# YOUNESELBOUKNIFY/Ctr_recommendation

Measured on AMD Instinct MI355X. Metric: training samples/sec (FiBiNET d=128, MicroLens-shaped synthetic, full train step), higher is better.
Workload: dtype bf16; 1 GPU; C3: FiBiNET emb_dim=128 + item_emb_d128, batch 8192/GPU, history 20, every GEMM operand bf16 (forward and backward) / fp32 accumulation + fp32 master weights, gradients and Adam; model=MM_FiBiNET, global_batch=8192, seq_len=20, item_rows=1250000, item_rows_per_gpu=1250000, emb_dim=128, parallelism=single, hipgraph=False, launch_mode=program

## Files before the change

ctr_recommendation_amd/_lib.py:

```python
from __future__ import annotations

import contextlib
import ctypes
import os
import struct
import threading
from typing import Optional

import torch

_HERE = os.path.dirname(os.path.abspath(__file__))
LIB_PATH = os.environ.get("FBN_LIB_PATH") or os.path.join(_HERE, "libfibinet_hip.so")

P = ctypes.c_void_p
I = ctypes.c_int
LL = ctypes.c_longlong
F = ctypes.c_float
D = ctypes.c_double
SZ = ctypes.c_size_t
U = ctypes.c_uint

SIGNATURES = {
    "fbn_version": (I, []),
    "fbn_last_error": (ctypes.c_char_p, []),
    "fbn_device_ok": (I, []),
    "fbn_gemm_workspace_size": (SZ, [I, I, I, I]),
    "fbn_gemm": (I, [P, P, P, P, I, I, I, I, I, I, I, I, I, I, I, I, I, I, F, I, I, I, P, P, SZ, P]),
    "fbn_gemm_split": (I, [P, P, P, P, I, I, I, I, I, I, I, I, I, I, I, F, P, P, SZ, P, I, I, P, I, I, P]),
    "fbn_gemm_bf16out": (I, [P, P, P, I, I, I, I, I, I, I, I, P]),
    "fbn_gemm_s3": (I, [P, P, P, I, I, I, I, I, I, I, I, LL, LL, F, P, SZ, P]),
    "fbn_gemm_bn_bwd_part_supported": (I, [I, I, I, I, I, I, I]),
    "fbn_gemm_bn_bwd_part": (I, [P, P, P, I, I, I, I, I, I, I, I, P, P, P, F, P, P]),
    "fbn_bn_tile_stats": (I, [P, I, I, P, P, P]),
    "fbn_bn_tile_moments": (I, [P, I, I, P, P]),
    "fbn_bn_moments_finalize": (I, [P, D, I, P, P, P, P, F, F, I, P]),
    "fbn_bn_tile_finalize": (I, [P, I, I, D, P, P, P, P, F, F, I, P]),
    "fbn_bn_colpart_size": (SZ, [I, I]),
    "fbn_row_chunks": (I, [I]),
    "fbn_bn_bwd_chunks": (I, [I, I]),
    "fbn_bn_bwd_fused": (I, [P, P, P, P, P, F, P, P, P, P, I, I, D, P, P, P, P, P, P, P, P, P]),
    "fbn_bn_bwd_fused_img": (I, [P, P, P, P, P, F, P, P, P, P, I, I, D, P, P, P, P, P, P, P, P, P]),
    "fbn_colsum_partial": (I, [P, I, I, I, P, P]),
    "fbn_sum_jobs": (I, [P, I, P]),
    "fbn_sum_jobs2": (I, [P, I, P, I, P]),
    "fbn_gemm_slabs_size": (SZ, [I, I, I]),
    "fbn_gemm_slabs": (I, [P, P, I, I, I, I, I, I, I, P, SZ, P, I, I, P, I, I, P, P]),
    "fbn_gemm_slabs_split": (I, [I, I, I]),
    "fbn_gemm_slabs_group": (I, [P, I, P]),
    "fbn_gemm_slabs_group_split": (I, [I, I, I]),
    "fbn_fields_fwd": (I, [P, P, P, P, P, P, P, F, P, I, P, LL, P, P, P, P, P, I, P, P, P, P, I, I, P, P, P, P, P, I, I, I, I,
                           P]),
    "fbn_fields_fwd_hot": (I, [P, P, P, P, P, P, P, F, P, I, P, LL, P, P, P, P, I, P, P, P, P, I, I, P, P, P, P, P,
                               I, I, I, P, P, I, P]),
    "fbn_hot_rows": (I, [P, P, I, I, LL, P, P, P, I, I, I, P]),
    "fbn_fields_bwd_partials_size": (I, [I, I, I]),
    "fbn_fields_bwd_grid": (I, [I, I]),
    "fbn_fields_bwd": (I, [P, P, P, P, P, P, P, F, P, P, P, I, I, P, P, P, P, P, P, P, P, P, P, P, P, LL, P, P, I, I,
                           I, I, P]),
    "fbn_fields_bwd_img": (I, [P, P, P, P, P, P, P, F, P, P, P, I, I, P, P, P, P, P, P, P, P, P, P, P, P, LL, P, P, I,
                               I, I, I, P]),
    "fbn_pairs_fwd": (I, [P, P, P, P, I, I, I, I, I, P]),
    "fbn_pairs_bwd": (I, [P, P, P, P, P, P, P, I, I, I, I, P]),
    "fbn_pairs_fwd_img": (I, [P, P, P, P, I, I, I, P]),
    "fbn_pairs_bwd_img": (I, [P, P, P, P, P, I, I, I, P]),
    "fbn_bn_workspace_size": (SZ, [I, I]),
    "fbn_bn_stats_pass": (I, [P, I, I, P, P, P, P]),
    "fbn_bn_mean": (I, [P, D, I, P, P]),
    "fbn_bn_finalize": (I, [P, P, D, I, P, P, P, P, F, F, I, P]),
    "fbn_bn_stats": (I, [P, I, I, P, P, P, P, F, F, I, P, P]),
    "fbn_bn_eval_params": (I, [P, P, P, P, I, F, P]),
    "fbn_bn_act_fwd": (I, [P, P, I, I, P, P, P, P, F, P, U, P, P, P, P]),
    "fbn_bn_act_fwd_img": (I, [P, P, I, I, P, P, P, P, F, P, U, P, P, P, P]),
    "fbn_bn_act_head_fwd": (I, [P, P, I, I, P, P, P, P, F, P, U, P, P, P, P, P, P, P, P, P, F, P, F, P]),
    "fbn_bn_bwd_reduce": (I, [P, P, P, P, F, P, P, I, I, P, P, P]),
    "fbn_bn_bwd_apply": (I, [P, P, P, P, F, P, P, P, P, I, I, P, D, P, P, P, P, P, P, P]),
    "fbn_convert_bf16": (I, [P, I, P]),
    "fbn_bn_bwd": (I, [P, P, P, P, F, P, P, P, P, I, I, P, P, P, P, P, P]),
    "fbn_colsum_workspace_size": (SZ, [I, I]),
    "fbn_colsum": (I, [P, I, I, I, P, F, P, P]),
    "fbn_head_fwd": (I, [P, P, P, I, I, P, P, P, P, P, F, P]),
    "fbn_sigmoid_bwd": (I, [P, P, P, I, P]),
    "fbn_outer": (I, [P, P, P, I, I, P]),
    "fbn_sum": (I, [P, I, P, F, P]),
    "fbn_sumsq": (I, [P, LL, P, I, P, P]),
    "fbn_clip_coef": (I, [P, F, P, P, P]),
    "fbn_adam_dense": (I, [P, P, P, P, LL, P, P, P, F, F, F, P, F, P, P, P]),
    "fbn_sparse_fixup": (I, [P, P, P, I, I, LL, I, P, P, P, P, I, I, P]),
    "fbn_sumsq_sparse": (I, [P, P, P, I, I, I, P, P]),
    "fbn_sparse_fixup_dup": (I, [P, I, P, P, P, I, I, P]),
    "fbn_sumsq_sparse_norms": (I, [P, P, P, P, I, I, I, P, P, P, LL, P]),
    "fbn_sparse_fold_fx": (I, [P, P, I, P, P, I, I, P, P]),
    "fbn_adam_table": (I, [P, P, P, LL, I, P, P, P, P, I, P, P, P, F, F, F, I, P]),
    "fbn_adam_touched": (I, [P, P, P, I, P, P, P, P, I, I, P, P, P, F, F, F, P, P]),
    "fbn_adam_catchup": (I, [P, P, P, LL, I, P, I, P, I, I, P, P, P, F, F, F, P, P, P, LL, I, I, P]),
    "fbn_adam_claim_catchup": (I, [P, P, I, I, LL, P, P, P, P, P, P, P, P, LL, I, I, P, P, P, F, F, F, P, P, P, LL, I,
                                   I, P]),
    "fbn_adam_claim_catchup_conv": (I, [P, P, I, I, LL, P, P, P, P, P, P, P, P, LL, I, I, P, P, P, F, F, F, P, P, P,
                                        LL, I, I, P, I, P]),
    "fbn_adam_flush": (I, [P, P, P, LL, I, P, P, P, F, F, F, P, P, P, LL, I, I, P]),
    "fbn_adam_prefetch_rows": (I, [P, I, I, LL, P, P, P, P, P, I, P, P, P, F, F, F, P, P, P, LL, I, I, P]),
    "fbn_adam_prefetch": (I, [P, P, I, I, LL, P, P, P, P, P, I, P, P, P, F, F, F, P, P, P, LL, I, I, P]),
    "fbn_adam_prefetch_binned_ws_size": (SZ, [LL]),
    "fbn_adam_prefetch_binned": (I, [P, P, I, I, LL, P, P, P, P, P, I, P, P, P, F, F, F, P, P, P, LL, I, I, P, SZ, P]),
    "fbn_adam_selftest": (I, [I, ctypes.c_uint, P, P]),
    "fbn_adam_step_tail": (I, [P, P, P, P, LL, P, F, P, P, P, P, P, I, P, P, P, P, I, I, P, P, F, F, F, P, P, P, P, I,
                               LL, I, P, P, P, P, I, P, P]),
    "fbn_adam_commit": (I, [P, P, P, I, P, P, P, P, I, I, P, P, P, F, F, F, P, P, P, P, I, I, P]),
    "fbn_claim_rows": (I, [P, P, I, I, LL, P, P, P, P, P]),
    "fbn_pack_extras": (I, [P, P, P, P]),
    "fbn_unpack_extras": (I, [P, P, P, P]),
    "fbn_unpack_sumsq": (I, [P, P, P, LL, P, P]),
    "fbn_step_end": (I, [P, P, P, P, P, I, P, P]),
    "fbn_route": (I, [P, P, I, I, LL, LL, I, P, P, P, P, P, P, P]),
# ... 345 lines not shown
```

ctr_recommendation_amd/csrc/fields.hip:

```cpp
#include <cstdlib>
#include "common.h"
#include "fields_common.h"

#ifndef FBN_HCH
#define FBN_HCH 10
#endif

struct FieldArgs {
  const int64_t* item_id;
  const int64_t* item_seq;
  const int64_t* likes;
  const int64_t* views;
  const float* hmm;
  const float* ln_g;
  const float* ln_b;
  const float* cate;
  const float* table;
  const int* pos;
  const float* w1; const float* b1; const float* w2; const float* b2;
  float* X;
  float* Vc;
  short* Vc16;
  void* c;
  float* a_out;
// ... 195 lines not shown
    const f32x4 xs[5] = {c1, c2, rit, x4, x5};
    float z[6];
    z[0] = 0.f;
#pragma unroll
    for (int f = 0; f < 5; ++f) z[f + 1] = group_sum<G>(xs[f][0] + xs[f][1] + xs[f][2] + xs[f][3]) / (float)D;
    float qv[FBN_MAXR], a[6];
    senet_excite<D>(z, p.w1, p.b1, p.w2, p.b2, p.R, qv, a);

    float* Xb = p.X + (size_t)b * 2 * D + 4 * q;
    *reinterpret_cast<f32x4*>(Xb) = rit;
    *reinterpret_cast<f32x4*>(Xb + D) = x5;
    float* Vb = p.Vc ? p.Vc + (size_t)b * 5 * D + 4 * q : nullptr;
    float* cb = (p.c && !p.c16) ? (float*)p.c + (size_t)b * p.ldc + 4 * q : nullptr;
    short* cb16 = (p.c && p.c16) ? (short*)p.c + (size_t)b * p.ldc + 4 * q : nullptr;
#pragma unroll
    for (int f = 0; f < 5; ++f) {
      const f32x4 v = xs[f] * a[f + 1];
      if (p.Vc) *reinterpret_cast<f32x4*>(Vb + f * D) = v;
      const bf16x4 v16 = (bf16x4){f2bf(v[0]), f2bf(v[1]), f2bf(v[2]), f2bf(v[3])};
      if (cb16) *reinterpret_cast<bf16x4*>(cb16 + f * D) = v16;
      else if (cb) *reinterpret_cast<f32x4*>(cb + f * D) = v;
      if (p.Vc16) *reinterpret_cast<bf16x4*>(p.Vc16 + ((size_t)b * 5 + f) * D + 4 * q) = v16;
    }
#pragma unroll
    for (int f = 0; f < 6; ++f)
      if (f % G == q) p.a_out[(size_t)b * 6 + f] = a[f];
    if (q == 0) p.cnt_out[b] = cnt;

    if (MODE == 0 && p.map) {
      for (int t = q; t <= L; t += G) {
        long long r = (t == 0) ? item : p.item_seq[(size_t)b * L + (t - 1)];
        if (r > 0 && r < p.V) map_claim(p.map, p.slot_row, (int)r, b * (L + 1) + t);
      }
    }
  }
}

struct FieldBwdArgs {
  const int64_t* item_id; const int64_t* item_seq; const int64_t* likes; const int64_t* views;
  const float* hmm; const float* ln_g;
  const float* w1; const float* b1; const float* w2;
  const float* X;
  const float* cate;
  const float* ln_b;
  const float* a;
  const float* cnt;
  const float* dV;
  float* dhmm;
  short* dhmm16;
  long long dhmm16_lo;
  float* partials;
  float* gtab; float* gvec;
  double* gnorm;
  const int* pos; void* sendbuf;
  long long V;
  int B, L, R, n_cate;
  float ln_eps;
};

template <int G>
__device__ __forceinline__ f32x4 transpose_cols(const f32x4& v, int lane) {
  const int base = lane - lane % G, q = lane % G;
  f32x4 t;
#pragma unroll
  for (int e = 0; e < 4; ++e) {
    const int src = base + e * (G / 4) + q / 4;
    const float x0 = __shfl(v[0], src, 64), x1 = __shfl(v[1], src, 64);
    const float x2 = __shfl(v[2], src, 64), x3 = __shfl(v[3], src, 64);
    const int c = q & 3;
    t[e] = c == 0 ? x0 : (c == 1 ? x1 : (c == 2 ? x2 : x3));
  }
  return t;
}
template <int G>
__device__ __forceinline__ void atomic_add_row_t(float* row, const f32x4& t, int q) {
  atomicAdd(row + q, t[0]); atomicAdd(row + G + q, t[1]); atomicAdd(row + 2 * G + q, t[2]);
  atomicAdd(row + 3 * G + q, t[3]);
}

template <int D, int MODE, int RMAX>
__global__ void __launch_bounds__(256) fields_bwd_kernel(FieldBwdArgs p) {
  FBN_MAIN_PRIO();
  constexpr int G = D / 4;
  constexpr int SPW = 64 / G;
  constexpr int NPMAX = 13 * RMAX + 6;
  constexpr int SJ = (NPMAX + G - 1) / G;
  extern __shared__ __attribute__((aligned(16))) float sp[];
  const int R = p.R;
  const int NP = 13 * R + 6;
  const int P = NP + 3 * D + p.n_cate * D;
  const int wave = threadIdx.x >> 6;
  float* ws = sp + wave * P;
  float* sv = sp + 4 * P + (wave * SPW + (threadIdx.x & 63) / G) * (12 + 2 * RMAX);
  for (int i = threadIdx.x; i < 4 * P; i += blockDim.x) sp[i] = 0.f;
  __syncthreads();
  float* w_lg = ws + NP;
  float* w_ct = w_lg + 2 * D;
  float* w_hb = w_ct + p.n_cate * D;

  const int lane = threadIdx.x & 63;
  const int q = lane % G, grp = lane / G;
  const int gw = (blockIdx.x * blockDim.x + threadIdx.x) >> 6;
  const int nwaves = (gridDim.x * blockDim.x) >> 6;
  const int L = p.L;
  f32x4 acc_lg = {0.f, 0.f, 0.f, 0.f}, acc_lb = {0.f, 0.f, 0.f, 0.f}, acc_hb = {0.f, 0.f, 0.f, 0.f};
  float acc_se[SJ];
#pragma unroll
  for (int j = 0; j < SJ; ++j) acc_se[j] = 0.f;

  for (int b0 = gw * SPW; b0 < p.B; b0 += nwaves * SPW) {
    const int b = b0 + grp;
    const bool live = b < p.B;
    f32x4 dx0 = {0.f, 0.f, 0.f, 0.f}, dx1 = {0.f, 0.f, 0.f, 0.f};
    long long lk = -1, vw = -1;
    if (live) {
      const float* Xb = p.X + (size_t)b * 2 * D + 4 * q;
      const float* dVb = p.dV + (size_t)b * 5 * D + 4 * q;
      f32x4 x[5], dv[5];
      lk = p.likes[b];
      vw = p.views[b];
      const long long lkc = (lk >= 0 && lk < p.n_cate) ? lk : 0, vwc = (vw >= 0 && vw < p.n_cate) ? vw : 0;
      x[0] = *reinterpret_cast<const f32x4*>(p.cate + lkc * D + 4 * q);
      x[1] = *reinterpret_cast<const f32x4*>(p.cate + vwc * D + 4 * q);
      x[2] = *reinterpret_cast<const f32x4*>(Xb);
      x[4] = *reinterpret_cast<const f32x4*>(Xb + D);
#pragma unroll
      for (int f = 0; f < 5; ++f) dv[f] = *reinterpret_cast<const f32x4*>(dVb + f * D);
      const f32x4 h = *reinterpret_cast<const f32x4*>(p.hmm + (size_t)b * D + 4 * q);
      x[3] = ln_relu<G>(h, p.ln_g, p.ln_b, p.ln_eps, q);
      float a[6];
#pragma unroll
      for (int f = 0; f < 6; ++f) a[f] = p.a[(size_t)b * 6 + f];
      float z[6];
      z[0] = 0.f;
#pragma unroll
      for (int f = 0; f < 5; ++f) z[f + 1] = group_sum<G>(x[f][0] + x[f][1] + x[f][2] + x[f][3]) / (float)D;
      float qv[RMAX], rj[RMAX], dq[RMAX];
#pragma unroll
      for (int j = 0; j < RMAX; ++j) {
        float s = 0.f;
        if (j < R) {
          s = p.b1[j];
#pragma unroll
          for (int f = 0; f < 6; ++f) s += p.w1[j * 6 + f] * z[f];
        }
        qv[j] = s;
        rj[j] = fmaxf(s, 0.f);
      }
      float ds[6];
      ds[0] = 0.f;
#pragma unroll
      for (int f = 0; f < 5; ++f) {
        const float da = group_sum<G>(dv[f][0] * x[f][0] + dv[f][1] * x[f][1] + dv[f][2] * x[f][2] + dv[f][3] * x[f][3]);
        ds[f + 1] = da * (1.f - a[f + 1]) * a[f + 1];
      }
      float dz[6] = {0.f, 0.f, 0.f, 0.f, 0.f, 0.f};
#pragma unroll
// ... 16 lines not shown
        for (int jj = 0; jj < RMAX; ++jj) { sv[12 + jj] = dq[jj]; sv[12 + RMAX + jj] = rj[jj]; }
      }
      __builtin_amdgcn_wave_barrier();
#pragma unroll
      for (int j = 0; j < SJ; ++j) {
        const int k = q + j * G;
        float v = 0.f;
        if (k < 6 * R) v = sv[12 + k / 6] * sv[6 + k % 6];
        else if (k < 7 * R) v = sv[12 + (k - 6 * R)];
        else if (k < 13 * R) v = sv[(k - 7 * R) / R] * sv[12 + RMAX + (k - 7 * R) % R];
        else if (k < NP) v = sv[k - 13 * R];
        acc_se[j] += v;
      }
      __builtin_amdgcn_wave_barrier();
      f32x4 dx[5];
#pragma unroll
      for (int f = 0; f < 5; ++f) dx[f] = dv[f] * a[f + 1] + dz[f + 1] / (float)D;
      dx0 = dx[0];
      dx1 = dx[1];

      {
        const float mean = group_sum<G>(h[0] + h[1] + h[2] + h[3]) / (float)D;
        const f32x4 dh = h - mean;
        const float s2 = group_sum<G>(dh[0] * dh[0] + dh[1] * dh[1] + dh[2] * dh[2] + dh[3] * dh[3]);
        const float rstd = 1.f / sqrtf(s2 / (float)D + p.ln_eps);
        const f32x4 gam = *reinterpret_cast<const f32x4*>(p.ln_g + 4 * q);
        f32x4 gl, xh, gx;
#pragma unroll
        for (int e = 0; e < 4; ++e) {
          gl[e] = x[3][e] > 0.f ? dx[3][e] : 0.f;
          xh[e] = dh[e] * rstd;
          gx[e] = gl[e] * gam[e];
          acc_lg[e] += gl[e] * xh[e];
          acc_lb[e] += gl[e];
        }
        const float m1 = group_sum<G>(gx[0] + gx[1] + gx[2] + gx[3]) / (float)D;
        const float m2 = group_sum<G>(gx[0] * xh[0] + gx[1] * xh[1] + gx[2] * xh[2] + gx[3] * xh[3]) / (float)D;
        f32x4 out;
#pragma unroll
        for (int e = 0; e < 4; ++e) out[e] = rstd * (gx[e] - m1 - xh[e] * m2);
        *reinterpret_cast<f32x4*>(p.dhmm + (size_t)b * D + 4 * q) = out;
        acc_hb += out;
        if (p.dhmm16) {
          const bf16x4 hi = (bf16x4){f2bf(out[0]), f2bf(out[1]), f2bf(out[2]), f2bf(out[3])};
          *reinterpret_cast<bf16x4*>(p.dhmm16 + (size_t)b * D + 4 * q) = hi;
          if (p.dhmm16_lo)
            *reinterpret_cast<bf16x4*>(p.dhmm16 + p.dhmm16_lo + (size_t)b * D + 4 * q) =
                (bf16x4){f2bf(out[0] - bf2f(hi[0])), f2bf(out[1] - bf2f(hi[1])), f2bf(out[2] - bf2f(hi[2])),
                         f2bf(out[3] - bf2f(hi[3]))};
        }
      }
      const f32x4 gh = dx[4] / p.cnt[b];
      if (MODE == 0 && p.gvec) {
        *reinterpret_cast<f32x4*>(p.gvec + (size_t)b * 2 * D + 4 * q) = dx[2];
        *reinterpret_cast<f32x4*>(p.gvec + ((size_t)b * 2 + 1) * D + 4 * q) = gh;
        if (p.gnorm) {
          double si = 0.0, sh = 0.0;
#pragma unroll
          for (int e = 0; e < 4; ++e) {
            si += (double)(dx[2][e] * dx[2][e]);
            sh += (double)(gh[e] * gh[e]);
          }
#pragma unroll
          for (int o = G / 2; o > 0; o >>= 1) {
            si += __shfl_xor(si, o, 64);
            sh += __shfl_xor(sh, o, 64);
          }
          if (q == 0) {
            p.gnorm[(size_t)b * 2] = si;
            p.gnorm[(size_t)b * 2 + 1] = sh;
          }
        }
      } else if (MODE == 0) {
        const f32x4 ti = transpose_cols<G>(dx[2], lane);
        const f32x4 th = transpose_cols<G>(gh, lane);
        const long long item = p.item_id[b];
        if (item > 0 && item < p.V) atomic_add_row_t<G>(p.gtab + item * D, ti, q);
        for (int t = 0; t < L; ++t) {
          const long long s = p.item_seq[(size_t)b * L + t];
          if (s > 0 && s < p.V) atomic_add_row_t<G>(p.gtab + s * D, th, q);
        }
      } else {
        const int* pb = p.pos + (size_t)b * (L + 1);
        auto put = [&](int row, const f32x4& x) {
          if constexpr (MODE == 2) {
            *reinterpret_cast<bf16x4*>(reinterpret_cast<short*>(p.sendbuf) + (size_t)row * D + 4 * q) =
                (bf16x4){f2bf(x[0]), f2bf(x[1]), f2bf(x[2]), f2bf(x[3])};
          } else {
            *reinterpret_cast<f32x4*>(reinterpret_cast<float*>(p.sendbuf) + (size_t)row * D + 4 * q) = x;
          }
        };
        if (pb[0] >= 0) put(pb[0], dx[2]);
        for (int t = 0; t < L; ++t)
          if (pb[t + 1] >= 0) put(pb[t + 1], gh);
      }
    }
#pragma unroll
    for (int gi = 0; gi < SPW; ++gi) {
      if (grp == gi && live) {
        if (lk >= 0 && lk < p.n_cate) {
          f32x4* c = reinterpret_cast<f32x4*>(w_ct + lk * D + 4 * q);
          *c = *c + dx0;
        }
        if (vw >= 0 && vw < p.n_cate) {
          f32x4* c = reinterpret_cast<f32x4*>(w_ct + vw * D + 4 * q);
          *c = *c + dx1;
        }
      }
// ... 143 lines not shown
  if (clear && i == 0) *hot_n = 0;
  if (i >= (long long)B * (L + 1)) return;
  const long long b = i / (L + 1), t = i - b * (L + 1);
  const long long id = t == 0 ? item[b] : seq[b * L + (t - 1)];
  if (id <= 0 || id >= V) return;
  if (clear) {
    cnt[id] = 0;
    return;
  }
  if (atomicAdd(cnt + id, 1) == tau - 1) {
    const int s = atomicAdd(hot_n, 1);
    if (s < H) hot[s] = (int)id;
  }
}

extern "C" int fbn_hot_rows(const int64_t* item, const int64_t* seq, int B, int L, long long V, int* cnt, int* hot,
                            int* hot_n, int H, int tau, int clear, void* stream) {
  const long long n = (long long)B * (L + 1);
  if (n <= 0) return FBN_OK;
  fbn_launch(hot_rows_kernel, dim3((unsigned)((n + 255) / 256)), dim3(256), 0, (hipStream_t)stream, item,
                     L > 0 ? seq : nullptr, B, L, V, cnt, hot, hot_n, H, tau < 1 ? 1 : tau, clear);
  FBN_CHECK_LAUNCH();
  return FBN_OK;
}

static int fields_fwd_impl(const int64_t* item_id, const int64_t* item_seq, const int64_t* likes,
                           const int64_t* views, const float* hmm, const float* ln_g, const float* ln_b,
                           float ln_eps, const float* cate, int n_cate, const float* table, long long V,
                           const int* pos, const float* w1, const float* b1, const float* w2,
                           const float* b2, int R, float* X, float* Vc, short* Vc16, void* c, int ldc, int c_bf16,
                           float* a_out, float* cnt_out, int* err, int* map, int* slot_row, int B, int L,
                           int D, int rows_bf16, const int* hot, const int* hot_n, int H, void* stream) {
  if (B <= 0) return FBN_OK;
  if (L < 0 || L > 32 || R < 1 || R > FBN_MAXR || (ldc & 3)) {
    fbn_set_error("fbn_fields_fwd: need 0 <= L <= 32, 1 <= R <= 8, ldc % 4 == 0");
    return FBN_ERR_ARG;
  }
  FieldArgs a;
  a.item_id = item_id; a.item_seq = L > 0 ? item_seq : nullptr; a.likes = likes; a.views = views;
  a.hmm = hmm; a.ln_g = ln_g; a.ln_b = ln_b; a.cate = cate; a.table = table; a.pos = pos;
  a.w1 = w1; a.b1 = b1; a.w2 = w2; a.b2 = b2;
  a.X = X; a.Vc = Vc; a.Vc16 = Vc16; a.c = c; a.a_out = a_out; a.cnt_out = cnt_out; a.err = err;
  a.map = map; a.slot_row = slot_row;
  a.V = V; a.B = B; a.L = L; a.ldc = ldc; a.R = R; a.n_cate = n_cate; a.ln_eps = ln_eps; a.c16 = c_bf16;
  a.hot = hot; a.hot_n = hot_n; a.H = H;
  if (pos && rows_bf16) return launch_fields_fwd<2>(a, D, (hipStream_t)stream);
  if (pos) return launch_fields_fwd<1>(a, D, (hipStream_t)stream);
  return launch_fields_fwd<0>(a, D, (hipStream_t)stream);
}

extern "C" int fbn_fields_bwd_partials_size(int D, int R, int n_cate) { return 13 * R + 6 + 3 * D + n_cate * D; }
extern "C" int fbn_fields_bwd_grid(int B, int D) { return fields_grid(B, D, FBN_FB_MAXBLK); }

template <int MODE, int RMAX>
static int launch_fields_bwd_r(const FieldBwdArgs& a, int D, hipStream_t st) {
  const int grid = fields_grid(a.B, D, FBN_FB_MAXBLK);
  const size_t lds = (4 * (size_t)(13 * a.R + 6 + 3 * D + a.n_cate * D) + 4 * (64 / (D / 4)) * (12 + 2 * RMAX)) *
                     sizeof(float);
  switch (D) {
    case 16: fbn_launch((fields_bwd_kernel<16, MODE, RMAX>), dim3(grid), dim3(256), lds, st, a); break;
    case 32: fbn_launch((fields_bwd_kernel<32, MODE, RMAX>), dim3(grid), dim3(256), lds, st, a); break;
    case 64: fbn_launch((fields_bwd_kernel<64, MODE, RMAX>), dim3(grid), dim3(256), lds, st, a); break;
    case 128: fbn_launch((fields_bwd_kernel<128, MODE, RMAX>), dim3(grid), dim3(256), lds, st, a); break;
    case 256: fbn_launch((fields_bwd_kernel<256, MODE, RMAX>), dim3(grid), dim3(256), lds, st, a); break;
    default: fbn_set_error("fields: embedding_dim must be one of 16,32,64,128,256"); return FBN_ERR_UNSUPPORTED;
  }
  FBN_CHECK_LAUNCH();
  return FBN_OK;
}

template <int MODE>
static int launch_fields_bwd(const FieldBwdArgs& a, int D, hipStream_t st) {
  return a.R <= 3 ? launch_fields_bwd_r<MODE, 3>(a, D, st) : launch_fields_bwd_r<MODE, FBN_MAXR>(a, D, st);
}

static int fields_bwd_impl(const int64_t* item_id, const int64_t* item_seq, const int64_t* likes,
                           const int64_t* views, const float* hmm, const float* ln_g, const float* ln_b,
                           float ln_eps, const float* w1, const float* b1, const float* w2, int R, int n_cate,
                           const float* cate, const float* X, const float* a, const float* cnt, const float* dV,
                           float* dhmm, short* dhmm16, float* partials, float* const* param_grads, float* gtab,
                           float* gvec, double* gnorm, long long V, const int* pos, void* sendbuf, int send_bf16,
                           int B, int L, int D, void* stream, long long dhmm16_lo);
extern "C" int fbn_fields_bwd(const int64_t* item_id, const int64_t* item_seq, const int64_t* likes,
                              const int64_t* views, const float* hmm, const float* ln_g, const float* ln_b,
                              float ln_eps, const float* w1, const float* b1, const float* w2, int R, int n_cate,
                              const float* cate, const float* X, const float* a, const float* cnt, const float* dV, float* dhmm,
                              short* dhmm16, float* partials, float* const* param_grads, float* gtab, float* gvec,
                              double* gnorm, long long V, const int* pos, void* sendbuf, int send_bf16, int B,
                              int L, int D, void* stream) {
  return fields_bwd_impl(item_id, item_seq, likes, views, hmm, ln_g, ln_b, ln_eps, w1, b1, w2, R, n_cate, cate, X, a,
                         cnt, dV, dhmm, dhmm16, partials, param_grads, gtab, gvec, gnorm, V, pos, sendbuf, send_bf16, B,
                         L, D, stream, 0);
}
extern "C" int fbn_fields_bwd_img(const int64_t* item_id, const int64_t* item_seq, const int64_t* likes,
                                  const int64_t* views, const float* hmm, const float* ln_g, const float* ln_b,
                                  float ln_eps, const float* w1, const float* b1, const float* w2, int R, int n_cate,
                                  const float* cate, const float* X, const float* a, const float* cnt, const float* dV,
                                  float* dhmm, void* dhmm_img, float* partials, float* const* param_grads,
                                  float* gtab, float* gvec, double* gnorm, long long V, const int* pos, void* sendbuf,
                                  int send_bf16, int B, int L, int D, void* stream) {
  if (!dhmm_img) { fbn_set_error("fbn_fields_bwd_img: dhmm_img"); return FBN_ERR_ARG; }
  return fields_bwd_impl(item_id, item_seq, likes, views, hmm, ln_g, ln_b, ln_eps, w1, b1, w2, R, n_cate, cate, X, a,
                         cnt, dV, dhmm, (short*)dhmm_img, partials, param_grads, gtab, gvec, gnorm, V, pos, sendbuf,
                         send_bf16, B, L, D, stream, (long long)B * D);
}
static int fields_bwd_impl(const int64_t* item_id, const int64_t* item_seq, const int64_t* likes,
                           const int64_t* views, const float* hmm, const float* ln_g, const float* ln_b,
                           float ln_eps, const float* w1, const float* b1, const float* w2, int R, int n_cate,
                           const float* cate, const float* X, const float* a, const float* cnt, const float* dV,
                           float* dhmm, short* dhmm16, float* partials, float* const* param_grads, float* gtab,
                           float* gvec, double* gnorm, long long V, const int* pos, void* sendbuf, int send_bf16,
                           int B, int L, int D, void* stream, long long dhmm16_lo) {
  if (B <= 0) return FBN_OK;
  if (L < 0 || L > 32 || R < 1 || R > FBN_MAXR) { fbn_set_error("fbn_fields_bwd: bad L/R"); return FBN_ERR_ARG; }
  FieldBwdArgs p;
  p.item_id = item_id; p.item_seq = L > 0 ? item_seq : nullptr; p.likes = likes; p.views = views;
  p.hmm = hmm; p.ln_g = ln_g; p.ln_b = ln_b; p.w1 = w1; p.b1 = b1; p.w2 = w2; p.cate = cate;
  p.X = X; p.a = a; p.cnt = cnt; p.dV = dV; p.dhmm = dhmm; p.dhmm16 = dhmm16; p.partials = partials;
  p.dhmm16_lo = dhmm16_lo;
  p.gtab = gtab; p.gvec = gvec; p.gnorm = gvec ? gnorm : nullptr; p.pos = pos; p.sendbuf = sendbuf;
  p.V = V; p.B = B; p.L = L; p.R = R; p.n_cate = n_cate; p.ln_eps = ln_eps;
  hipStream_t st = (hipStream_t)stream;
  int rc = !pos ? launch_fields_bwd<0>(p, D, st) : send_bf16 ? launch_fields_bwd<2>(p, D, st)
                                                               : launch_fields_bwd<1>(p, D, st);
  if (rc) return rc;
  if (!param_grads) return FBN_OK;
  const int P = 13 * R + 6 + 3 * D + n_cate * D;
  const int nblk = fields_grid(B, D, FBN_FB_MAXBLK);

  GradOuts o;
  const int sizes[8] = {6 * R, R, 6 * R, 6, D, D, n_cate * D, D};
  o.off[0] = 0;
  for (int j = 0; j < 8; ++j) {
    if (j < 7 && !param_grads[j]) {
      fbn_set_error("fbn_fields_bwd: null parameter-gradient destination");
      return FBN_ERR_ARG;
    }
    o.p[j] = param_grads[j];
    o.off[j + 1] = o.off[j] + sizes[j];
  }
  fbn_launch(reduce_partials_one16, dim3(fbn_cdiv(P, 16)), dim3(1024), 0, st, (const float*)partials, nblk, P, o);
  FBN_CHECK_LAUNCH();
  return FBN_OK;
}
```

ctr_recommendation_amd/csrc/mlp.hip:

```cpp
#include <cstdlib>
#include "common.h"
#include "convert.h"

__device__ constexpr int c_pi[10] = {0, 0, 0, 0, 1, 1, 1, 2, 2, 3};
__device__ constexpr int c_pj[10] = {1, 2, 3, 4, 2, 3, 4, 3, 4, 4};

__device__ __forceinline__ void store4(float* p, const f32x4& v) { *reinterpret_cast<f32x4*>(p) = v; }
__device__ __forceinline__ void store4(short* p, const f32x4& v) {
  *reinterpret_cast<bf16x4*>(p) = (bf16x4){f2bf(v[0]), f2bf(v[1]), f2bf(v[2]), f2bf(v[3])};
}
__device__ __forceinline__ void store_img4(short* p, long long lo_off, const f32x4& v) {
  bf16x4 h, l;
#pragma unroll
  for (int e = 0; e < 4; ++e) {
    h[e] = f2bf(v[e]);
    l[e] = f2bf(v[e] - bf2f(h[e]));
  }
  *reinterpret_cast<bf16x4*>(p) = h;
  *reinterpret_cast<bf16x4*>(p + lo_off) = l;
}
__device__ __forceinline__ void store_lo4(short* p, const f32x4& v) {
  bf16x4 l;
#pragma unroll
  for (int e = 0; e < 4; ++e) l[e] = f2bf(v[e] - bf2f(f2bf(v[e])));
// ... 753 lines not shown
                                                            const float* __restrict__ mean,
                                                            const float* __restrict__ invstd,
                                                            const float* __restrict__ g,
                                                            const float* __restrict__ coef, float* __restrict__ dX,
                                                            short* __restrict__ dX16, int B, int C,
                                                            int rows_per_chunk, float* __restrict__ colpart) {
  FBN_MAIN_PRIO();
  __shared__ f32x4 red[4][64];
  const int q = threadIdx.x & 63, rl = threadIdx.x >> 6;
  const int c = blockIdx.x * 256 + q * 4;
  const int r0 = blockIdx.y * rows_per_chunk, r1 = min(B, r0 + rows_per_chunk);
  f32x4 acc = {0.f, 0.f, 0.f, 0.f};
  if (c < C) {
    const f32x4 mu = *reinterpret_cast<const f32x4*>(mean + c);
    const f32x4 is = *reinterpret_cast<const f32x4*>(invstd + c);
    const f32x4 gg = *reinterpret_cast<const f32x4*>(g + c);
    const f32x4 c0 = *reinterpret_cast<const f32x4*>(coef + c);
    const f32x4 c1 = *reinterpret_cast<const f32x4*>(coef + C + c);
    const f32x4 ww = s.G ? (f32x4){0.f, 0.f, 0.f, 0.f} : *reinterpret_cast<const f32x4*>(s.w + c);
    for (int r = r0 + rl; r < r1; r += 4) {
      const size_t i = (size_t)r * C + c;
      const f32x4 h = bn_act4(s, i);
      const f32x4 x = *reinterpret_cast<const f32x4*>(Xpre + i);
      f32x4 d;
      if (s.G) d = *reinterpret_cast<const f32x4*>(s.G + i);
      else { const float gv = s.gvec[r]; d = (f32x4){gv * ww[0], gv * ww[1], gv * ww[2], gv * ww[3]}; }
      f32x4 v;
#pragma unroll
      for (int e = 0; e < 4; ++e) {
        const float dy = h[e] > 0.f ? d[e] * s.scale : 0.f;
        v[e] = (dy - c0[e] - (x[e] - mu[e]) * c1[e]) * is[e] * gg[e];
      }
      if (dX) *reinterpret_cast<f32x4*>(dX + i) = v;
      if (dX16) {
        if (s.dx16_lo) store_img4(dX16 + i, s.dx16_lo, v);
        else store4(dX16 + i, v);
      }
      acc += v;
    }
  }
  if (!colpart) return;
  red[rl][q] = acc;
  __syncthreads();
  if (rl == 0 && c < C)
    *reinterpret_cast<f32x4*>(colpart + (size_t)blockIdx.y * C + c) = red[0][q] + red[1][q] + red[2][q] + red[3][q];
}

struct SumJob {
  const float* part;
  float* out;
  int nch, C;
  float scale, beta;
  int ld;
  int pad_;
};
struct SlabJob {
  const float* ws;
  float* out;
  int M, N, ldc, nsplit, seg, off0, off1;
  float beta;
};
#define FBN_MAX_SUM_JOBS 16
#define FBN_SUM_WIDE 32
#define FBN_MAX_SLAB_JOBS 8
#define FBN_SLAB_GROUPS 4
struct SumJobs {
  SumJob j[FBN_MAX_SUM_JOBS];
  int col0[FBN_MAX_SUM_JOBS + 1];
  int n;
  SlabJob s[FBN_MAX_SLAB_JOBS];
  int blk0[FBN_MAX_SLAB_JOBS + 1];
  int ns;
};
#define FBN_SLAB_DIRECT 8
__device__ __forceinline__ void slab_direct(const SlabJob& sj, int lb) {
  const size_t total = (size_t)sj.M * sj.N;
  const size_t i4 = (size_t)lb * 256 + threadIdx.x;
  if (i4 >= total / 4) return;
  const float* src = sj.ws + i4 * 4;
  f32x4 x[FBN_SLAB_DIRECT];
#pragma unroll
  for (int z = 0; z < FBN_SLAB_DIRECT; ++z)
    if (z < sj.nsplit) x[z] = *reinterpret_cast<const f32x4*>(src + (size_t)z * total);
  f32x4 t = x[0];
#pragma unroll
  for (int z = 1; z < FBN_SLAB_DIRECT; ++z)
    if (z < sj.nsplit) t += x[z];
  const int m = (int)(i4 * 4 / sj.N), n = (int)(i4 * 4 - (size_t)m * sj.N);
  float* cp = sj.out + (size_t)m * sj.ldc + n + (n < sj.seg ? sj.off0 : sj.off1);
  if (sj.beta != 0.f) t += sj.beta * *reinterpret_cast<const f32x4*>(cp);
  *reinterpret_cast<f32x4*>(cp) = t;
}
__device__ __forceinline__ void slab_block(const SumJobs& J, int gb) {
  __shared__ f32x4 red[FBN_SLAB_GROUPS][64];
  int u = 0;
  while (u + 1 < J.ns && gb >= J.blk0[u + 1]) ++u;
  const SlabJob sj = J.s[u];
  if (sj.nsplit <= FBN_SLAB_DIRECT) {
    slab_direct(sj, gb - J.blk0[u]);
    return;
  }
  const int qd = threadIdx.x & 63, grp = threadIdx.x >> 6;
  const size_t total = (size_t)sj.M * sj.N;
  const size_t i4 = (size_t)(gb - J.blk0[u]) * 64 + qd;
  const bool ok = i4 < total / 4;
  f32x4 acc = {0.f, 0.f, 0.f, 0.f};
  if (ok) {
    const float* src = sj.ws + i4 * 4;
    int z = grp;
    for (; z + 3 * FBN_SLAB_GROUPS < sj.nsplit; z += 4 * FBN_SLAB_GROUPS) {
      const f32x4 a = *reinterpret_cast<const f32x4*>(src + (size_t)z * total);
      const f32x4 b = *reinterpret_cast<const f32x4*>(src + (size_t)(z + FBN_SLAB_GROUPS) * total);
      const f32x4 c = *reinterpret_cast<const f32x4*>(src + (size_t)(z + 2 * FBN_SLAB_GROUPS) * total);
      const f32x4 d = *reinterpret_cast<const f32x4*>(src + (size_t)(z + 3 * FBN_SLAB_GROUPS) * total);
      acc += a; acc += b; acc += c; acc += d;
    }
    for (; z < sj.nsplit; z += FBN_SLAB_GROUPS) acc += *reinterpret_cast<const f32x4*>(src + (size_t)z * total);
  }
  red[grp][qd] = acc;
  __syncthreads();
  if (grp == 0 && ok) {
    f32x4 t = red[0][qd];
#pragma unroll
    for (int k = 1; k < FBN_SLAB_GROUPS; ++k) t += red[k][qd];
    const int m = (int)(i4 * 4 / sj.N), n = (int)(i4 * 4 - (size_t)m * sj.N);
    float* cp = sj.out + (size_t)m * sj.ldc + n + (n < sj.seg ? sj.off0 : sj.off1);
    if (sj.beta != 0.f) t += sj.beta * *reinterpret_cast<const f32x4*>(cp);
    *reinterpret_cast<f32x4*>(cp) = t;
  }
}
__device__ __forceinline__ void sum_wide_block(const SumJob& jb, int c0) {
  __shared__ float red[16][17];
  const int col = threadIdx.x & 15, str = threadIdx.x >> 4, c = c0 + col;
  const size_t ld = jb.ld > 0 ? jb.ld : jb.C;
  float a0 = 0.f, a1 = 0.f;
  if (c < jb.C) {
    int k = str;
    for (; k + 16 < jb.nch; k += 32) {
      a0 += jb.part[(size_t)k * ld + c];
      a1 += jb.part[(size_t)(k + 16) * ld + c];
    }
    for (; k < jb.nch; k += 16) a0 += jb.part[(size_t)k * ld + c];
  }
  red[str][col] = a0 + a1;
  __syncthreads();
  if (str == 0 && c < jb.C) {
    float t = 0.f;
#pragma unroll
    for (int k = 0; k < 16; ++k) t += red[k][col];
    t *= jb.scale;
    jb.out[c] = jb.beta != 0.f ? jb.beta * jb.out[c] + t : t;
  }
}
__global__ void __launch_bounds__(256) sum_jobs_kernel(SumJobs J) {
  __shared__ float red[4];
  const int gc = blockIdx.x;
  if (gc >= J.col0[J.n]) {
    slab_block(J, gc - J.col0[J.n]);
    return;
  }
  int u = 0;
  while (u + 1 < J.n && gc >= J.col0[u + 1]) ++u;
  const SumJob jb = J.j[u];
  if (jb.C >= FBN_SUM_WIDE) {
    sum_wide_block(jb, (gc - J.col0[u]) * 16);
    return;
  }
  const int c = gc - J.col0[u];
  const size_t ld = jb.ld > 0 ? jb.ld : jb.C;
  float a0 = 0.f, a1 = 0.f, a2 = 0.f, a3 = 0.f;
  int k = threadIdx.x;
  for (; k + 768 < jb.nch; k += 1024) {
    a0 += jb.part[(size_t)k * ld + c];
    a1 += jb.part[(size_t)(k + 256) * ld + c];
    a2 += jb.part[(size_t)(k + 512) * ld + c];
    a3 += jb.part[(size_t)(k + 768) * ld + c];
  }
  for (; k < jb.nch; k += 256) a0 += jb.part[(size_t)k * ld + c];
  float v = wave_sum((a0 + a1) + (a2 + a3));
  if ((threadIdx.x & 63) == 0) red[threadIdx.x >> 6] = v;
  __syncthreads();
  if (threadIdx.x == 0) {
    const float t = jb.scale * ((red[0] + red[1]) + (red[2] + red[3]));
    jb.out[c] = jb.beta != 0.f ? jb.beta * jb.out[c] + t : t;
  }
}

__global__ void head_fwd_kernel(const float* __restrict__ H, const float* __restrict__ w, const float* __restrict__ bias,
                                int B, int C, float* __restrict__ logits, float* __restrict__ probs,
                                const float* __restrict__ labels, float* __restrict__ loss_terms,
                                float* __restrict__ gout, float denom) {
  const int lane = threadIdx.x & 63;
  const int row = (blockIdx.x * blockDim.x + threadIdx.x) >> 6;
  if (row >= B) return;
  float s = 0.f;
  for (int c = lane * 4; c < C; c += 256) {
    const f32x4 h = *reinterpret_cast<const f32x4*>(H + (size_t)row * C + c);
    const f32x4 ww = *reinterpret_cast<const f32x4*>(w + c);
    s += h[0] * ww[0] + h[1] * ww[1] + h[2] * ww[2] + h[3] * ww[3];
  }
  head_row(s, row, lane, HeadArgs{w, bias, logits, probs, labels, loss_terms, gout, denom});
}

__global__ void sigmoid_bwd_kernel(const float* gp, const float* probs, float* gout, int B) {
  const int i = blockIdx.x * blockDim.x + threadIdx.x;
  if (i < B) gout[i] = gp[i] * (1.f - probs[i]) * probs[i];
}

__global__ void outer_kernel(const float* g, const float* w, float* out, int B, int C) {
  const size_t total = (size_t)B * C;
  for (size_t i = (size_t)blockIdx.x * blockDim.x + threadIdx.x; i < total; i += (size_t)gridDim.x * blockDim.x)
    out[i] = g[i / C] * w[i % C];
}

__global__ void __launch_bounds__(1024) sum_kernel(const float* x, int n, float* out, float scale) {
  __shared__ float red[16];
  float s0 = 0.f, s1 = 0.f, s2 = 0.f, s3 = 0.f;
  int i = threadIdx.x;
  for (; i + 3 * 1024 < n; i += 4 * 1024) {
    s0 += x[i]; s1 += x[i + 1024]; s2 += x[i + 2048]; s3 += x[i + 3072];
  }
  for (; i < n; i += 1024) s0 += x[i];
  float s = wave_sum((s0 + s1) + (s2 + s3));
  if ((threadIdx.x & 63) == 0) red[threadIdx.x >> 6] = s;
  __syncthreads();
  if (threadIdx.x < 64) {
    float t = threadIdx.x < 16 ? red[threadIdx.x] : 0.f;
    t = wave_sum(t);
    if (threadIdx.x == 0) out[0] = t * scale;
  }
}

static int ew_grid(size_t n) {
  size_t g = (n + 255) / 256;
  return (int)(g < 1 ? 1 : (g > 8192 ? 8192 : g));
}
static int row_chunks(int B) {
// ... 360 lines not shown
  return bn_bwd_fused_impl(G, gvec, w, hact, hact16, scale, Xpre, mean, invstd, gamma, B, C, ntot, dXpre,
                           (short*)dXpre_img, dgamma, dbeta, dw, colpart, part_pre, ws, stream, (long long)B * C);
}
static int bn_bwd_fused_impl(const float* G, const float* gvec, const float* w, const float* hact,
                             const short* hact16, float scale, const float* Xpre, const float* mean,
                             const float* invstd, const float* gamma, int B, int C, double ntot, float* dXpre,
                             short* dXpre16, float* dgamma, float* dbeta, float* dw, float* colpart,
                             const double* part_pre, void* ws, void* stream, long long img_lo) {
  if (B <= 0) return FBN_OK;
  if (C & 3) { fbn_set_error("fbn_bn_bwd_fused: C % 4"); return FBN_ERR_ARG; }
  if (!hact && !(hact16 && G)) {
    fbn_set_error("fbn_bn_bwd_fused: the bf16 activation image stands in only for a matrix source");
    return FBN_ERR_ARG;
  }
  if (!dXpre && !dXpre16) { fbn_set_error("fbn_bn_bwd_fused: no output"); return FBN_ERR_ARG; }
  hipStream_t st = (hipStream_t)stream;
  BnBwdSrc s{G, gvec, w, hact, scale, hact16, img_lo};
  const int nch = bn_bwd_chunks(B, C), rpc = (B + nch - 1) / nch;
  double* part = (double*)ws;
  float* coef = (float*)((double*)ws + (size_t)nch * 3 * C + 3 * (size_t)C);
  if (part_pre)
    part = const_cast<double*>(part_pre);
  else
    fbn_launch(bn_bwd_partial4_kernel, dim3(fbn_cdiv(C, 256), nch), dim3(256), 0, st, s, Xpre, mean, B, C, rpc,
                       part);
  const char* nce = getenv("FBN_BN_REDUCE_NC");
  const int nc = nce ? atoi(nce) : 16;
  if (nc == 4)
    fbn_launch(bn_bwd_reduce_finalize16_kernel<4>, dim3(fbn_cdiv(C, 4)), dim3(256), 0, st, part, nch, C, ntot,
               invstd, coef, dgamma, dbeta, dw);
  else if (nc == 8)
    fbn_launch(bn_bwd_reduce_finalize16_kernel<8>, dim3(fbn_cdiv(C, 8)), dim3(512), 0, st, part, nch, C, ntot,
               invstd, coef, dgamma, dbeta, dw);
  else
    fbn_launch(bn_bwd_reduce_finalize16_kernel<16>, dim3(fbn_cdiv(C, 16)), dim3(1024), 0, st, part, nch, C, ntot,
                       invstd, coef, dgamma, dbeta, dw);
  fbn_launch(bn_bwd_apply4_kernel, dim3(fbn_cdiv(C, 256), nch), dim3(256), 0, st, s, Xpre, mean, invstd, gamma,
                     coef, dXpre, dXpre16, B, C, rpc, colpart);
  FBN_CHECK_LAUNCH();
  return FBN_OK;
}

extern "C" int fbn_colsum_partial(const float* X, int B, int C, int ldx, float* part, void* stream) {
  if (B <= 0) return FBN_OK;
  const int nch = row_chunks(B), rpc = (B + nch - 1) / nch;
  fbn_launch(colsum_partial_kernel, dim3(fbn_cdiv(C, 64), nch), dim3(256), 0, (hipStream_t)stream, X, B, C,
                     ldx, rpc, part);
  FBN_CHECK_LAUNCH();
  return FBN_OK;
}

extern "C" int fbn_row_chunks(int B) { return row_chunks(B); }

extern "C" int fbn_sum_jobs2(const SumJob* jobs, int n, const SlabJob* slabs, int ns, void* stream) {
  if (n < 0 || ns < 0 || n > FBN_MAX_SUM_JOBS || ns > FBN_MAX_SLAB_JOBS) {
    fbn_set_error("fbn_sum_jobs2: too many jobs");
    return FBN_ERR_ARG;
  }
  SumJobs J;
  J.n = n;
  J.col0[0] = 0;
  for (int i = 0; i < n; ++i) {
    J.j[i] = jobs[i];
    J.col0[i + 1] = J.col0[i] + (jobs[i].C >= FBN_SUM_WIDE ? fbn_cdiv(jobs[i].C, 16) : jobs[i].C);
  }
  J.ns = ns;
  J.blk0[0] = 0;
  for (int i = 0; i < ns; ++i) {
    const SlabJob& sj = slabs[i];
    if ((sj.N & 3) || (sj.ldc & 3) || (sj.off0 & 3) || (sj.off1 & 3) || (sj.seg != 0x7fffffff && (sj.seg & 3)) ||
        ((uintptr_t)sj.out & 15) || ((uintptr_t)sj.ws & 15) || sj.nsplit < 1) {
      fbn_set_error("fbn_sum_jobs2: slab job needs N, ldc, remap % 4, 16-B aligned buffers, nsplit >= 1");
      return FBN_ERR_ARG;
    }
    J.s[i] = sj;
    const int qpb = (sj.nsplit <= FBN_SLAB_DIRECT) ? 256 : 64;
    J.blk0[i + 1] = J.blk0[i] + (int)fbn_cdiv((long long)sj.M * sj.N / 4, qpb);
  }
  const int blocks = J.col0[n] + J.blk0[ns];
  if (blocks <= 0) return FBN_OK;
  fbn_launch(sum_jobs_kernel, dim3(blocks), dim3(256), 0, (hipStream_t)stream, J);
  FBN_CHECK_LAUNCH();
  return FBN_OK;
}

extern "C" int fbn_sum_jobs(const SumJob* jobs, int n, void* stream) {
  if (n <= 0) return FBN_OK;
  return fbn_sum_jobs2(jobs, n, nullptr, 0, stream);
}

extern "C" int fbn_bn_tile_moments(const float* part, int M, int C, double* out_d, void* stream) {
  if (M <= 0) { (void)hipMemsetAsync(out_d, 0, 2 * sizeof(double) * C, (hipStream_t)stream); return FBN_OK; }
  fbn_launch(bn_tile_moments_kernel, dim3(fbn_cdiv(C, 4)), dim3(256), 0, (hipStream_t)stream, part,
                     (M + 63) / 64, C, M, 64, out_d);
  FBN_CHECK_LAUNCH();
  return FBN_OK;
}

extern "C" int fbn_bn_moments_finalize(const double* mom_d, double ntot, int C, float* mean, float* invstd,
                                       float* run_mean, float* run_var, float momentum, float eps, int update_running,
                                       void* stream) {
  fbn_launch(bn_moments_finalize_kernel, dim3(fbn_cdiv(C, 256)), dim3(256), 0, (hipStream_t)stream, mom_d, ntot,
                     C, mean, invstd, run_mean, run_var, momentum, eps, update_running);
  FBN_CHECK_LAUNCH();
  return FBN_OK;
}
```

ctr_recommendation_amd/csrc/optim.hip:

```cpp
#include "common.h"
#include "convert.h"
#include <cstdlib>
#include <algorithm>

#pragma clang fp contract(off)

#define FBN_SUMSQ_SLOTS 64

struct AdamConsts {
  float w1;
  float nss;
  float bc2s;
  float rbc2s;
  float dmul;
  float pad0, pad1, pad2;
};

__global__ void sumsq_kernel(const float* __restrict__ x, long long n, const int* __restrict__ n_rows, int row_len,
                             double* __restrict__ out) {
  __shared__ double red[256];
  long long lim = n_rows ? (long long)(*n_rows) * row_len : n;
  double s = 0.0;
  const long long n4 = lim / 4;
  for (long long i = (long long)blockIdx.x * blockDim.x + threadIdx.x; i < n4; i += (long long)gridDim.x * blockDim.x) {
// ... 199 lines not shown
  for (long long e0 = gw * RPW; e0 < n; e0 += nw * RPW) {
    const long long e = e0 + lane / G;
    if (e >= n) continue;
    long long r;
    if (ids) {
      r = ids[e];
      if (r < 0 || (rank == 0 && r == 0)) continue;
    } else {
      const long long b = e / (L + 1), t = e - b * (L + 1);
      r = t == 0 ? item[b] : seq[b * L + (t - 1)];
      if (r <= 0 || r >= V) continue;
    }
    const int u = map[r];
    if (u == (int)e || u < 0) continue;
    const float* src = grad_base<D>(s, (int)e);
    float* dst;
    if (s.extra) {
      if (q == 0) atomicOr(&s.slot_row[u], FBN_SLOT_FLAG);
      dst = s.extra + (size_t)u * D;
    } else {
      dst = const_cast<float*>(s.vec) + (size_t)u * D;
    }
#pragma unroll
    for (int k = 0; k < 4; ++k) atomicAdd(dst + k * G + q, src[k * G + q]);
  }
}

__global__ void claim_rows_kernel(const int64_t* __restrict__ item, const int64_t* __restrict__ seq, int B, int L,
                                  long long V, int* __restrict__ map, int* __restrict__ slot_row, int* __restrict__ dup,
                                  int* __restrict__ hasdup) {
  const long long n = (long long)B * (L + 1);
  for (long long e = (long long)blockIdx.x * blockDim.x + threadIdx.x; e < n; e += (long long)gridDim.x * blockDim.x) {
    const long long b = e / (L + 1), t = e - b * (L + 1);
    const long long r = t == 0 ? item[b] : seq[b * L + (t - 1)];
    int owner = -1;
    if (r > 0 && r < V) {
      owner = __hip_atomic_load(map + r, __ATOMIC_RELAXED, __HIP_MEMORY_SCOPE_AGENT);
      if (owner == -1) {
        int expected = -1;
        if (__hip_atomic_compare_exchange_strong(map + r, &expected, (int)e, __ATOMIC_RELAXED, __ATOMIC_RELAXED,
                                                 __HIP_MEMORY_SCOPE_AGENT))
          slot_row[e] = (int)r;
        else
          owner = expected;
      }
    }
    if (dup) dup[e] = owner;
    if (hasdup && owner >= 0) hasdup[owner] = 1;
  }
}

template <int D>
__global__ void __launch_bounds__(FBN_FOLD_THREADS) sparse_fixup_dup_kernel(const int* __restrict__ dup, int n, GradSrc s) {
  constexpr int NPL = D / 64 > 0 ? D / 64 : 1;
  constexpr int MAXV = 16;
  constexpr int CPW = FBN_FOLD_CHUNKS;
  constexpr int NS = D >= 256 ? 32 : 64;
  __shared__ int skey[NS];
  __shared__ float sacc[NS * D];
  const int tid = threadIdx.x, lane = tid & 63, wave = tid >> 6;
  for (int i = tid; i < NS; i += blockDim.x) skey[i] = -1;
  for (int i = tid; i < NS * D; i += blockDim.x) sacc[i] = 0.f;
  __syncthreads();
  const int Lp1 = s.Lp1;
  const long long base = (long long)blockIdx.x * blockDim.x * CPW;
  int uu[CPW];
#pragma unroll
  for (int c = 0; c < CPW; ++c) {
    const long long e = base + ((long long)(wave * CPW + c) << 6) + lane;
    uu[c] = e < n ? dup[e] : -1;
  }
  auto add_row = [&](int ue, const float (&acc)[NPL], bool hot) {
    int slot = -1;
    if (hot && lane == 0) {
      for (int k = 0, h = (int)(((unsigned)ue * 2654435761u) >> 20) & (NS - 1); k < 4; ++k, h = (h + 1) & (NS - 1)) {
        int cur = __hip_atomic_load(skey + h, __ATOMIC_RELAXED, __HIP_MEMORY_SCOPE_WORKGROUP);
        if (cur == -1) {
          int expected = -1;
          if (__hip_atomic_compare_exchange_strong(skey + h, &expected, ue, __ATOMIC_RELAXED, __ATOMIC_RELAXED,
                                                   __HIP_MEMORY_SCOPE_WORKGROUP)) {
            slot = h;
            break;
          }
          cur = expected;
        }
        if (cur == ue) {
          slot = h;
          break;
        }
      }
    }
    slot = __shfl(slot, 0, 64);
    if (slot >= 0) {
#pragma unroll
      for (int k = 0; k < NPL; ++k)
        if (D >= 64 || lane < D) atomicAdd(sacc + slot * D + (D >= 64 ? k * 64 : 0) + lane, acc[k]);
    } else {
      float* dst = s.extra + (size_t)ue * D;
      if (lane == 0) atomicOr(&s.slot_row[ue], FBN_SLOT_FLAG);
#pragma unroll
      for (int k = 0; k < NPL; ++k)
        if (D >= 64 || lane < D) atomicAdd(dst + (D >= 64 ? k * 64 : 0) + lane, acc[k]);
    }
  };
#pragma unroll 1
  for (int c = 0; c < CPW; ++c) {
// ... 14 lines not shown
      unsigned long long vm[MAXV];
#pragma unroll
      for (int v = 0; v < MAXV; ++v) {
        vm[v] = __ballot(vid == v);
        const float* src = s.vec + ((size_t)bs * 2 + (v < nv ? v : 0)) * D;
#pragma unroll
        for (int k = 0; k < NPL; ++k)
          vec[v][k] = (D >= 64 || lane < D) ? src[(D >= 64 ? k * 64 : 0) + (lane & (D - 1))] : 0.f;
      }
      while (act) {
        const int l = __ffsll((long long)act) - 1;
        const int ue = __shfl(u, l, 64);
        const unsigned long long m = __ballot(u == ue) & act;
        act &= ~m;
        float acc[NPL];
#pragma unroll
        for (int k = 0; k < NPL; ++k) acc[k] = 0.f;
#pragma unroll
        for (int v = 0; v < MAXV; ++v) {
          const float cnt = (float)__popcll(m & vm[v]);
#pragma unroll
          for (int k = 0; k < NPL; ++k) acc[k] = __builtin_fmaf(cnt, vec[v][k], acc[k]);
        }
        add_row(ue, acc, __popcll(m) > 1);
      }
    } else {
      while (act) {
        const int l = __ffsll((long long)act) - 1;
        act &= act - 1;
        const int ue = __shfl(u, l, 64);
        const float* src = grad_base<D>(s, (int)(e0 + l));
        float acc[NPL];
#pragma unroll
        for (int k = 0; k < NPL; ++k) acc[k] = (D >= 64 || lane < D) ? src[(D >= 64 ? k * 64 : 0) + (lane & (D - 1))] : 0.f;
        add_row(ue, acc, false);
      }
    }
  }
  __syncthreads();
  for (int slot = wave; slot < NS; slot += blockDim.x >> 6) {
    const int ue = skey[slot];
    if (ue < 0) continue;
    if (lane == 0) atomicOr(&s.slot_row[ue], FBN_SLOT_FLAG);
    float* dst = s.extra + (size_t)ue * D;
    for (int k = lane; k < D; k += 64) atomicAdd(dst + k, sacc[slot * D + k]);
  }
}

#define FBN_FX_SHIFT 40
__device__ __forceinline__ long long to_fx(float x) { return __double2ll_rn((double)x * 1099511627776.0); }
template <int D>
__global__ void __launch_bounds__(256) sparse_fold_fx_kernel(const int* __restrict__ dup, int* __restrict__ hasdup,
                                                             int n, GradSrc s, unsigned long long* __restrict__ acc) {
  const int lane = threadIdx.x & 63;
  for (long long e0 = ((long long)blockIdx.x * blockDim.x + threadIdx.x) - lane; e0 < n;
       e0 += (long long)gridDim.x * blockDim.x) {
    const long long e = e0 + lane;
    int u = -1;
    if (e < n) {
      u = dup[e];
      if (u < 0 && hasdup[e]) {
        u = (int)e;
        hasdup[e] = 0;
        s.slot_row[e] |= FBN_SLOT_FLAG;
      }
    }
    unsigned long long mask = __ballot(u >= 0);
    while (mask) {
      const int l = __ffsll((long long)mask) - 1;
      mask &= mask - 1;
      const int ue = __shfl(u, l, 64);
      const float* src = grad_base<D>(s, (int)(e0 + l));
      unsigned long long* dst = acc + (size_t)ue * D;
      for (int k = lane; k < D; k += 64) atomicAdd(dst + k, (unsigned long long)to_fx(src[k]));
    }
  }
}

template <int D>
__global__ void __launch_bounds__(256) sumsq_norms_kernel(GradSrc s, const double* __restrict__ gnorm, int n,
                                                          double* __restrict__ out, unsigned long long* __restrict__ fx,
                                                          const float* __restrict__ dense, long long n_dense) {
  __shared__ double red[4];
  const int lane = threadIdx.x & 63;
  double acc = 0.0;
  for (long long i = (long long)blockIdx.x * blockDim.x + threadIdx.x; i < n_dense / 4;
       i += (long long)gridDim.x * blockDim.x) {
    const f32x4 v = *reinterpret_cast<const f32x4*>(dense + 4 * i);
    acc += (double)(v[0] * v[0]) + (double)(v[1] * v[1]) + (double)(v[2] * v[2]) + (double)(v[3] * v[3]);
  }
  for (long long e0 = ((long long)blockIdx.x * blockDim.x + threadIdx.x) - lane; e0 < n;
       e0 += (long long)gridDim.x * blockDim.x) {
    const long long e = e0 + lane;
    const int sr = e < n ? s.slot_row[e] : -1;
    const bool flag = sr != -1 && (sr & FBN_SLOT_FLAG);
    if (sr != -1 && !flag) {
      const int b = (int)(e / s.Lp1), t = (int)(e - (long long)b * s.Lp1);
      acc += gnorm[(size_t)b * 2 + (t ? 1 : 0)];
    }
    unsigned long long mask = __ballot(flag);
    if (fx) {
      while (mask) {
        const int l = __ffsll((long long)mask) - 1;
        mask &= mask - 1;
        float* x = s.extra + (size_t)(e0 + l) * D;
        unsigned long long* a = fx + (size_t)(e0 + l) * D;
        for (int k = lane; k < D; k += 64) {
          const float y = (float)((double)(long long)a[k] * (1.0 / 1099511627776.0));
          x[k] = y;
          a[k] = 0ull;
          acc += (double)(y * y);
        }
      }
    } else {
      constexpr int LPR = D / 8, RPR = 64 / LPR;
      while (mask) {
        int mine = -1;
#pragma unroll
        for (int gi = 0; gi < RPR; ++gi) {
          if (!mask) break;
          const int l = __ffsll((long long)mask) - 1;
          mask &= mask - 1;
          if (lane / LPR == gi) mine = l;
        }
        if (mine < 0) continue;
        const int c = (lane % LPR) * 8;
        const float* v = grad_base<D>(s, (int)(e0 + mine)) + c;
        const float* x = s.extra + (size_t)(e0 + mine) * D + c;
        const f32x4 v0 = *reinterpret_cast<const f32x4*>(v), v1 = *reinterpret_cast<const f32x4*>(v + 4);
        const f32x4 x0 = *reinterpret_cast<const f32x4*>(x), x1 = *reinterpret_cast<const f32x4*>(x + 4);
        const f32x4 y0 = v0 + x0, y1 = v1 + x1;
#pragma unroll
        for (int k = 0; k < 4; ++k) acc += (double)(y0[k] * y0[k]) + (double)(y1[k] * y1[k]);
      }
    }
// ... 1176 lines not shown
      if (ps.pend) ps.pend[(size_t)(r) * FBN_RS_I] = -1;
    }
  }
}

template <int D>
__global__ void __launch_bounds__(256) adam_touched_kernel(float* __restrict__ p, float* __restrict__ m,
                                                           float* __restrict__ v, int* __restrict__ map, GradSrc gs,
                                                           int n, const float* __restrict__ coef_ptr,
                                                           const AdamConsts* __restrict__ table,
                                                           const int* __restrict__ step_ptr, float wd, float b2,
                                                           float omb2, float eps, int* __restrict__ last) {
  resolve_src(gs);
  constexpr int G = D / 4, RPW = 64 / G;
  const AdamConsts k = table[*step_ptr];
  const float coef = coef_ptr ? *coef_ptr : 1.f;
  const int lane = threadIdx.x & 63, q = lane % G;
  const long long gw = ((long long)blockIdx.x * blockDim.x + threadIdx.x) >> 6;
  const long long nw = ((long long)gridDim.x * blockDim.x) >> 6;
  for (long long e0 = gw * RPW; e0 < n; e0 += nw * RPW) {
    const long long e = e0 + lane / G;
    if (e >= n) continue;
    const int sr = gs.slot_row[e];
    if (sr == -1) continue;
    const long long r = sr & ~FBN_SLOT_FLAG;
    f32x4 gg = grad4<D>(gs, (int)e, 4 * q);
    if (sr & FBN_SLOT_FLAG) {
      float* ex = gs.extra + (size_t)e * D + 4 * q;
      gg = gs.full ? *reinterpret_cast<const f32x4*>(ex) : gg + *reinterpret_cast<const f32x4*>(ex);
      *reinterpret_cast<f32x4*>(ex) = (f32x4){0.f, 0.f, 0.f, 0.f};
    }
    const size_t off = (size_t)r * D + 4 * q;
    f32x4 pp = *reinterpret_cast<f32x4*>(p + off);
    f32x4 mm = *reinterpret_cast<f32x4*>(m + off);
    f32x4 vv = *reinterpret_cast<f32x4*>(v + off);
    adam_tab4<true>(pp, mm, vv, gg * coef, wd, b2, omb2, eps, k);
    *reinterpret_cast<f32x4*>(p + off) = pp;
    *reinterpret_cast<f32x4*>(m + off) = mm;
    *reinterpret_cast<f32x4*>(v + off) = vv;
    if (q == 0) {
      map[r] = -1;
      if (last) last[(size_t)(r) * FBN_RS_I] = *step_ptr + 1;
    }
  }
}

template <int D>
__device__ __forceinline__ void adam_commit_body(float* __restrict__ p, float* __restrict__ m, float* __restrict__ v,
                                                 int* __restrict__ map, const GradSrc& gs, int n, float coef,
                                                 const AdamConsts& k, int t, float wd, float b2, float omb2, float eps,
                                                 int* __restrict__ last, const PendSrc& ps, int B, long long bid,
                                                 long long nblk) {
  constexpr int G = D / 4, RPW = 64 / G;
  if (gs.Lp1 > 1) {
    float* dst = const_cast<float*>(ps.ring) + (size_t)(t % ps.ring_n) * ps.ring_stride;
    const long long n4 = (long long)B * 2 * D / 4, st = nblk * blockDim.x;
    for (long long i0 = bid * blockDim.x + threadIdx.x; i0 < n4; i0 += 8 * st) {
      f32x4 x[8];
#pragma unroll
      for (int u = 0; u < 8; ++u)
        x[u] = reinterpret_cast<const f32x4*>(gs.vec)[i0 + u * st < n4 ? i0 + u * st : i0];
#pragma unroll
      for (int u = 0; u < 8; ++u)
        if (i0 + u * st < n4) reinterpret_cast<f32x4*>(dst)[i0 + u * st] = x[u];
    }
  }
  const int lane = threadIdx.x & 63, q = lane % G;
  for (long long e0 = (bid * blockDim.x + threadIdx.x) - lane; e0 < n; e0 += nblk * blockDim.x) {
    const long long e = e0 + lane;
    const int sr = e < n ? gs.slot_row[e] : -1;
    const bool flag = sr != -1 && (sr & FBN_SLOT_FLAG);
    bool imm = flag;
    if (sr != -1 && !flag) {
      if (last && (unsigned)row_state(last, sr).y == (unsigned)(t + 1)) {
        imm = true;
      } else {
        if (gs.Lp1 == 1) {
          ps.pend[(size_t)(sr) * FBN_RS_I] = (int)e;
        } else {
          const int b = (int)(e / gs.Lp1), tt = (int)(e - (long long)b * gs.Lp1);
          ps.pend[(size_t)(sr) * FBN_RS_I] = b * 2 + (tt ? 1 : 0);
        }
        map[sr] = -1;
        gs.slot_row[e] = -1;
      }
    }
    unsigned long long mask = __ballot(imm);
    constexpr int G8 = D / 8 > 0 ? D / 8 : 1, RPW8 = 64 / G8;
    const int q8 = lane % G8;
    while (mask) {
      int mine = -1;
#pragma unroll
      for (int gi = 0; gi < RPW8; ++gi) {
        if (!mask) break;
        const int l = __ffsll((long long)mask) - 1;
        mask &= mask - 1;
        if (lane / G8 == gi) mine = l;
      }
      const int sr_l = __shfl(sr, mine < 0 ? 0 : mine, 64);
      if (mine < 0) continue;
      const long long ee = e0 + mine;
      const long long r = sr_l & ~FBN_SLOT_FLAG;
#pragma unroll
      for (int h = 0; h < 2; ++h) {
        const int c = 8 * q8 + 4 * h;
        if (D < 8 && c >= D) break;
        f32x4 gg = grad4<D>(gs, (int)ee, c);
        if (sr_l & FBN_SLOT_FLAG) {
// ... 1028 lines not shown
```

ctr_recommendation_amd/csrc/plan_thunks.inc:

```

static int th_fbn_adam_catchup(const uint64_t* i, const double* f) {
  return fbn_adam_catchup(reinterpret_cast<float*>(static_cast<uintptr_t>(i[0])),
      reinterpret_cast<float*>(static_cast<uintptr_t>(i[1])),
      reinterpret_cast<float*>(static_cast<uintptr_t>(i[2])),
      static_cast<long long>(i[3]),
      static_cast<int>(i[4]),
      reinterpret_cast<const int*>(static_cast<uintptr_t>(i[5])),
      static_cast<int>(i[6]),
      reinterpret_cast<const int*>(static_cast<uintptr_t>(i[7])),
      static_cast<int>(i[8]),
      static_cast<int>(i[9]),
      reinterpret_cast<int*>(static_cast<uintptr_t>(i[10])),
      reinterpret_cast<const void*>(static_cast<uintptr_t>(i[11])),
      reinterpret_cast<const int*>(static_cast<uintptr_t>(i[12])),
      plan_f32(f[0]),
      plan_f32(f[1]),
      plan_f32(f[2]),
      reinterpret_cast<int*>(static_cast<uintptr_t>(i[13])),
      reinterpret_cast<const float*>(static_cast<uintptr_t>(i[14])),
      reinterpret_cast<const float*>(static_cast<uintptr_t>(i[15])),
      static_cast<long long>(i[16]),
      static_cast<int>(i[17]),
      static_cast<int>(i[18]),
      reinterpret_cast<void*>(static_cast<uintptr_t>(i[19])));
// ... 814 lines not shown
      reinterpret_cast<void*>(static_cast<uintptr_t>(i[26])),
      static_cast<int>(i[27]),
      static_cast<int>(i[28]),
      static_cast<int>(i[29]),
      static_cast<int>(i[30]),
      reinterpret_cast<void*>(static_cast<uintptr_t>(i[31])));
}
static int th_fbn_fields_bwd_grid(const uint64_t* i, const double* f) {
  (void)f;
  return fbn_fields_bwd_grid(static_cast<int>(i[0]),
      static_cast<int>(i[1]));
}
static int th_fbn_fields_bwd_img(const uint64_t* i, const double* f) {
  return fbn_fields_bwd_img(reinterpret_cast<const int64_t*>(static_cast<uintptr_t>(i[0])),
      reinterpret_cast<const int64_t*>(static_cast<uintptr_t>(i[1])),
      reinterpret_cast<const int64_t*>(static_cast<uintptr_t>(i[2])),
      reinterpret_cast<const int64_t*>(static_cast<uintptr_t>(i[3])),
      reinterpret_cast<const float*>(static_cast<uintptr_t>(i[4])),
      reinterpret_cast<const float*>(static_cast<uintptr_t>(i[5])),
      reinterpret_cast<const float*>(static_cast<uintptr_t>(i[6])),
      plan_f32(f[0]),
      reinterpret_cast<const float*>(static_cast<uintptr_t>(i[7])),
      reinterpret_cast<const float*>(static_cast<uintptr_t>(i[8])),
      reinterpret_cast<const float*>(static_cast<uintptr_t>(i[9])),
      static_cast<int>(i[10]),
      static_cast<int>(i[11]),
      reinterpret_cast<const float*>(static_cast<uintptr_t>(i[12])),
      reinterpret_cast<const float*>(static_cast<uintptr_t>(i[13])),
      reinterpret_cast<const float*>(static_cast<uintptr_t>(i[14])),
      reinterpret_cast<const float*>(static_cast<uintptr_t>(i[15])),
      reinterpret_cast<const float*>(static_cast<uintptr_t>(i[16])),
      reinterpret_cast<float*>(static_cast<uintptr_t>(i[17])),
      reinterpret_cast<void*>(static_cast<uintptr_t>(i[18])),
      reinterpret_cast<float*>(static_cast<uintptr_t>(i[19])),
      reinterpret_cast<float* const*>(static_cast<uintptr_t>(i[20])),
      reinterpret_cast<float*>(static_cast<uintptr_t>(i[21])),
      reinterpret_cast<float*>(static_cast<uintptr_t>(i[22])),
      reinterpret_cast<double*>(static_cast<uintptr_t>(i[23])),
      static_cast<long long>(i[24]),
      reinterpret_cast<const int*>(static_cast<uintptr_t>(i[25])),
      reinterpret_cast<void*>(static_cast<uintptr_t>(i[26])),
      static_cast<int>(i[27]),
      static_cast<int>(i[28]),
      static_cast<int>(i[29]),
      static_cast<int>(i[30]),
      reinterpret_cast<void*>(static_cast<uintptr_t>(i[31])));
}
static int th_fbn_fields_bwd_partials_size(const uint64_t* i, const double* f) {
  (void)f;
  return fbn_fields_bwd_partials_size(static_cast<int>(i[0]),
      static_cast<int>(i[1]),
      static_cast<int>(i[2]));
}
static int th_fbn_fields_fwd(const uint64_t* i, const double* f) {
  return fbn_fields_fwd(reinterpret_cast<const int64_t*>(static_cast<uintptr_t>(i[0])),
      reinterpret_cast<const int64_t*>(static_cast<uintptr_t>(i[1])),
      reinterpret_cast<const int64_t*>(static_cast<uintptr_t>(i[2])),
      reinterpret_cast<const int64_t*>(static_cast<uintptr_t>(i[3])),
      reinterpret_cast<const float*>(static_cast<uintptr_t>(i[4])),
      reinterpret_cast<const float*>(static_cast<uintptr_t>(i[5])),
      reinterpret_cast<const float*>(static_cast<uintptr_t>(i[6])),
      plan_f32(f[0]),
      reinterpret_cast<const float*>(static_cast<uintptr_t>(i[7])),
      static_cast<int>(i[8]),
      reinterpret_cast<const float*>(static_cast<uintptr_t>(i[9])),
      static_cast<long long>(i[10]),
      reinterpret_cast<const int*>(static_cast<uintptr_t>(i[11])),
      reinterpret_cast<const float*>(static_cast<uintptr_t>(i[12])),
      reinterpret_cast<const float*>(static_cast<uintptr_t>(i[13])),
      reinterpret_cast<const float*>(static_cast<uintptr_t>(i[14])),
      reinterpret_cast<const float*>(static_cast<uintptr_t>(i[15])),
      static_cast<int>(i[16]),
      reinterpret_cast<float*>(static_cast<uintptr_t>(i[17])),
      reinterpret_cast<float*>(static_cast<uintptr_t>(i[18])),
      reinterpret_cast<short*>(static_cast<uintptr_t>(i[19])),
      reinterpret_cast<void*>(static_cast<uintptr_t>(i[20])),
      static_cast<int>(i[21]),
      static_cast<int>(i[22]),
      reinterpret_cast<float*>(static_cast<uintptr_t>(i[23])),
      reinterpret_cast<float*>(static_cast<uintptr_t>(i[24])),
      reinterpret_cast<int*>(static_cast<uintptr_t>(i[25])),
      reinterpret_cast<int*>(static_cast<uintptr_t>(i[26])),
      reinterpret_cast<int*>(static_cast<uintptr_t>(i[27])),
      static_cast<int>(i[28]),
      static_cast<int>(i[29]),
      static_cast<int>(i[30]),
      static_cast<int>(i[31]),
      reinterpret_cast<void*>(static_cast<uintptr_t>(i[32])));
}
static int th_fbn_fields_fwd_hot(const uint64_t* i, const double* f) {
  return fbn_fields_fwd_hot(reinterpret_cast<const int64_t*>(static_cast<uintptr_t>(i[0])),
      reinterpret_cast<const int64_t*>(static_cast<uintptr_t>(i[1])),
      reinterpret_cast<const int64_t*>(static_cast<uintptr_t>(i[2])),
      reinterpret_cast<const int64_t*>(static_cast<uintptr_t>(i[3])),
      reinterpret_cast<const float*>(static_cast<uintptr_t>(i[4])),
      reinterpret_cast<const float*>(static_cast<uintptr_t>(i[5])),
      reinterpret_cast<const float*>(static_cast<uintptr_t>(i[6])),
      plan_f32(f[0]),
      reinterpret_cast<const float*>(static_cast<uintptr_t>(i[7])),
      static_cast<int>(i[8]),
      reinterpret_cast<const float*>(static_cast<uintptr_t>(i[9])),
      static_cast<long long>(i[10]),
      reinterpret_cast<const float*>(static_cast<uintptr_t>(i[11])),
      reinterpret_cast<const float*>(static_cast<uintptr_t>(i[12])),
      reinterpret_cast<const float*>(static_cast<uintptr_t>(i[13])),
      reinterpret_cast<const float*>(static_cast<uintptr_t>(i[14])),
// ... 522 lines not shown
  (void)f;
  return fbn_sparse_fixup_dup(reinterpret_cast<const int*>(static_cast<uintptr_t>(i[0])),
      static_cast<int>(i[1]),
      reinterpret_cast<const float*>(static_cast<uintptr_t>(i[2])),
      reinterpret_cast<float*>(static_cast<uintptr_t>(i[3])),
      reinterpret_cast<int*>(static_cast<uintptr_t>(i[4])),
      static_cast<int>(i[5]),
      static_cast<int>(i[6]),
      reinterpret_cast<void*>(static_cast<uintptr_t>(i[7])));
}
static int th_fbn_sparse_fold_fx(const uint64_t* i, const double* f) {
  (void)f;
  return fbn_sparse_fold_fx(reinterpret_cast<const int*>(static_cast<uintptr_t>(i[0])),
      reinterpret_cast<int*>(static_cast<uintptr_t>(i[1])),
      static_cast<int>(i[2]),
      reinterpret_cast<const float*>(static_cast<uintptr_t>(i[3])),
      reinterpret_cast<int*>(static_cast<uintptr_t>(i[4])),
      static_cast<int>(i[5]),
      static_cast<int>(i[6]),
      reinterpret_cast<unsigned long long*>(static_cast<uintptr_t>(i[7])),
      reinterpret_cast<void*>(static_cast<uintptr_t>(i[8])));
}
static int th_fbn_step_end(const uint64_t* i, const double* f) {
  (void)f;
  return fbn_step_end(reinterpret_cast<int*>(static_cast<uintptr_t>(i[0])),
      reinterpret_cast<unsigned long long*>(static_cast<uintptr_t>(i[1])),
      reinterpret_cast<double*>(static_cast<uintptr_t>(i[2])),
      reinterpret_cast<long long*>(static_cast<uintptr_t>(i[3])),
      reinterpret_cast<long long*>(static_cast<uintptr_t>(i[4])),
      static_cast<int>(i[5]),
      reinterpret_cast<int*>(static_cast<uintptr_t>(i[6])),
      reinterpret_cast<void*>(static_cast<uintptr_t>(i[7])));
}
static int th_fbn_sum(const uint64_t* i, const double* f) {
  return fbn_sum(reinterpret_cast<const float*>(static_cast<uintptr_t>(i[0])),
      static_cast<int>(i[1]),
      reinterpret_cast<float*>(static_cast<uintptr_t>(i[2])),
      plan_f32(f[0]),
      reinterpret_cast<void*>(static_cast<uintptr_t>(i[3])));
}
static int th_fbn_sum_jobs(const uint64_t* i, const double* f) {
  (void)f;
  return fbn_sum_jobs(reinterpret_cast<const void*>(static_cast<uintptr_t>(i[0])),
      static_cast<int>(i[1]),
      reinterpret_cast<void*>(static_cast<uintptr_t>(i[2])));
}
static int th_fbn_sum_jobs2(const uint64_t* i, const double* f) {
  (void)f;
  return fbn_sum_jobs2(reinterpret_cast<const void*>(static_cast<uintptr_t>(i[0])),
      static_cast<int>(i[1]),
      reinterpret_cast<const void*>(static_cast<uintptr_t>(i[2])),
      static_cast<int>(i[3]),
      reinterpret_cast<void*>(static_cast<uintptr_t>(i[4])));
}
static int th_fbn_sum_slices(const uint64_t* i, const double* f) {
  (void)f;
  return fbn_sum_slices(reinterpret_cast<const void*>(static_cast<uintptr_t>(i[0])),
      static_cast<int>(i[1]),
      static_cast<long long>(i[2]),
      static_cast<int>(i[3]),
      reinterpret_cast<void*>(static_cast<uintptr_t>(i[4])),
      reinterpret_cast<void*>(static_cast<uintptr_t>(i[5])));
}
static int th_fbn_sumsq(const uint64_t* i, const double* f) {
  (void)f;
  return fbn_sumsq(reinterpret_cast<const float*>(static_cast<uintptr_t>(i[0])),
      static_cast<long long>(i[1]),
      reinterpret_cast<const int*>(static_cast<uintptr_t>(i[2])),
      static_cast<int>(i[3]),
      reinterpret_cast<double*>(static_cast<uintptr_t>(i[4])),
      reinterpret_cast<void*>(static_cast<uintptr_t>(i[5])));
}
static int th_fbn_sumsq_flagged(const uint64_t* i, const double* f) {
  (void)f;
  return fbn_sumsq_flagged(reinterpret_cast<const int*>(static_cast<uintptr_t>(i[0])),
      static_cast<int>(i[1]),
      reinterpret_cast<const void*>(static_cast<uintptr_t>(i[2])),
      reinterpret_cast<float*>(static_cast<uintptr_t>(i[3])),
      static_cast<int>(i[4]),
      reinterpret_cast<const double*>(static_cast<uintptr_t>(i[5])),
      reinterpret_cast<double*>(static_cast<uintptr_t>(i[6])),
      reinterpret_cast<unsigned long long*>(static_cast<uintptr_t>(i[7])),
      static_cast<int>(i[8]),
      reinterpret_cast<void*>(static_cast<uintptr_t>(i[9])));
}
static int th_fbn_sumsq_sparse(const uint64_t* i, const double* f) {
  (void)f;
  return fbn_sumsq_sparse(reinterpret_cast<const float*>(static_cast<uintptr_t>(i[0])),
      reinterpret_cast<float*>(static_cast<uintptr_t>(i[1])),
      reinterpret_cast<int*>(static_cast<uintptr_t>(i[2])),
      static_cast<int>(i[3]),
      static_cast<int>(i[4]),
      static_cast<int>(i[5]),
      reinterpret_cast<double*>(static_cast<uintptr_t>(i[6])),
      reinterpret_cast<void*>(static_cast<uintptr_t>(i[7])));
}
static int th_fbn_sumsq_sparse_norms(const uint64_t* i, const double* f) {
  (void)f;
  return fbn_sumsq_sparse_norms(reinterpret_cast<const double*>(static_cast<uintptr_t>(i[0])),
      reinterpret_cast<const float*>(static_cast<uintptr_t>(i[1])),
      reinterpret_cast<float*>(static_cast<uintptr_t>(i[2])),
      reinterpret_cast<int*>(static_cast<uintptr_t>(i[3])),
      static_cast<int>(i[4]),
      static_cast<int>(i[5]),
      static_cast<int>(i[6]),
      reinterpret_cast<double*>(static_cast<uintptr_t>(i[7])),
// ... 40 lines not shown
    {"fbn_adam_flush", th_fbn_adam_flush, 15, 3},
    {"fbn_adam_owner_claim_catchup", th_fbn_adam_owner_claim_catchup, 22, 3},
    {"fbn_adam_prefetch", th_fbn_adam_prefetch, 21, 3},
    {"fbn_adam_prefetch_binned", th_fbn_adam_prefetch_binned, 23, 3},
    {"fbn_adam_prefetch_rows", th_fbn_adam_prefetch_rows, 20, 3},
    {"fbn_adam_selftest", th_fbn_adam_selftest, 4, 0},
    {"fbn_adam_step_tail", th_fbn_adam_step_tail, 34, 4},
    {"fbn_adam_table", th_fbn_adam_table, 15, 3},
    {"fbn_adam_touched", th_fbn_adam_touched, 15, 3},
    {"fbn_bilinear_bwd", th_fbn_bilinear_bwd, 11, 0},
    {"fbn_bilinear_fwd", th_fbn_bilinear_fwd, 7, 0},
    {"fbn_bilinear_supported", th_fbn_bilinear_supported, 1, 0},
    {"fbn_bn_act_fwd", th_fbn_bn_act_fwd, 14, 1},
    {"fbn_bn_act_fwd_img", th_fbn_bn_act_fwd_img, 14, 1},
    {"fbn_bn_act_head_fwd", th_fbn_bn_act_head_fwd, 21, 3},
    {"fbn_bn_bwd", th_fbn_bn_bwd, 16, 1},
    {"fbn_bn_bwd_apply", th_fbn_bn_bwd_apply, 18, 2},
    {"fbn_bn_bwd_chunks", th_fbn_bn_bwd_chunks, 2, 0},
    {"fbn_bn_bwd_fused", th_fbn_bn_bwd_fused, 20, 2},
    {"fbn_bn_bwd_fused_img", th_fbn_bn_bwd_fused_img, 20, 2},
    {"fbn_bn_bwd_reduce", th_fbn_bn_bwd_reduce, 11, 1},
    {"fbn_bn_eval_params", th_fbn_bn_eval_params, 6, 1},
    {"fbn_bn_finalize", th_fbn_bn_finalize, 9, 3},
    {"fbn_bn_mean", th_fbn_bn_mean, 4, 1},
    {"fbn_bn_moments_finalize", th_fbn_bn_moments_finalize, 8, 3},
    {"fbn_bn_stats", th_fbn_bn_stats, 10, 2},
    {"fbn_bn_stats_pass", th_fbn_bn_stats_pass, 7, 0},
    {"fbn_bn_tile_finalize", th_fbn_bn_tile_finalize, 9, 3},
    {"fbn_bn_tile_moments", th_fbn_bn_tile_moments, 5, 0},
    {"fbn_bn_tile_stats", th_fbn_bn_tile_stats, 6, 0},
    {"fbn_claim_rows", th_fbn_claim_rows, 10, 0},
    {"fbn_clip_coef", th_fbn_clip_coef, 4, 1},
    {"fbn_collate", th_fbn_collate, 24, 0},
    {"fbn_collate_zero_if", th_fbn_collate_zero_if, 4, 0},
    {"fbn_colsum", th_fbn_colsum, 7, 1},
    {"fbn_colsum_partial", th_fbn_colsum_partial, 6, 0},
    {"fbn_comm_allgather", th_fbn_comm_allgather, 5, 0},
    {"fbn_comm_allreduce", th_fbn_comm_allreduce, 5, 0},
    {"fbn_comm_alltoall", th_fbn_comm_alltoall, 5, 0},
    {"fbn_comm_alltoall_peers", th_fbn_comm_alltoall_peers, 5, 0},
    {"fbn_comm_alltoallv", th_fbn_comm_alltoallv, 7, 0},
    {"fbn_comm_heartbeat", th_fbn_comm_heartbeat, 1, 0},
    {"fbn_comm_id_bytes", th_fbn_comm_id_bytes, 0, 0},
    {"fbn_compact_routes", th_fbn_compact_routes, 6, 0},
    {"fbn_convert_bf16", th_fbn_convert_bf16, 3, 0},
    {"fbn_copy_jobs", th_fbn_copy_jobs, 5, 0},
    {"fbn_device_ok", th_fbn_device_ok, 0, 0},
    {"fbn_eval_pack", th_fbn_eval_pack, 6, 0},
    {"fbn_eval_reduce", th_fbn_eval_reduce, 7, 0},
    {"fbn_fields_bwd", th_fbn_fields_bwd, 32, 1},
    {"fbn_fields_bwd_grid", th_fbn_fields_bwd_grid, 2, 0},
    {"fbn_fields_bwd_img", th_fbn_fields_bwd_img, 32, 1},
    {"fbn_fields_bwd_partials_size", th_fbn_fields_bwd_partials_size, 3, 0},
    {"fbn_fields_fwd", th_fbn_fields_fwd, 33, 1},
    {"fbn_fields_fwd_hot", th_fbn_fields_fwd_hot, 34, 1},
    {"fbn_gemm", th_fbn_gemm, 25, 1},
    {"fbn_gemm_bf16out", th_fbn_gemm_bf16out, 12, 0},
    {"fbn_gemm_bn_bwd_part", th_fbn_gemm_bn_bwd_part, 16, 1},
    {"fbn_gemm_bn_bwd_part_supported", th_fbn_gemm_bn_bwd_part_supported, 7, 0},
    {"fbn_gemm_s3", th_fbn_gemm_s3, 16, 1},
    {"fbn_gemm_slabs", th_fbn_gemm_slabs, 19, 0},
    {"fbn_gemm_slabs_group", th_fbn_gemm_slabs_group, 3, 0},
    {"fbn_gemm_slabs_group_split", th_fbn_gemm_slabs_group_split, 3, 0},
    {"fbn_gemm_slabs_split", th_fbn_gemm_slabs_split, 3, 0},
    {"fbn_gemm_split", th_fbn_gemm_split, 25, 1},
    {"fbn_head_fwd", th_fbn_head_fwd, 11, 1},
    {"fbn_hot_rows", th_fbn_hot_rows, 12, 0},
    {"fbn_outer", th_fbn_outer, 6, 0},
    {"fbn_owner_claim", th_fbn_owner_claim, 6, 0},
    {"fbn_owner_fold", th_fbn_owner_fold, 20, 0},
    {"fbn_owner_gather", th_fbn_owner_gather, 10, 0},
    {"fbn_owner_gather_self", th_fbn_owner_gather_self, 13, 0},
    {"fbn_pack_extras", th_fbn_pack_extras, 4, 0},
    {"fbn_pad_routes", th_fbn_pad_routes, 7, 0},
    {"fbn_pairs_bwd", th_fbn_pairs_bwd, 12, 0},
    {"fbn_pairs_bwd_img", th_fbn_pairs_bwd_img, 9, 0},
    {"fbn_pairs_fwd", th_fbn_pairs_fwd, 10, 0},
    {"fbn_pairs_fwd_img", th_fbn_pairs_fwd_img, 8, 0},
    {"fbn_probe_arm", th_fbn_probe_arm, 1, 0},
    {"fbn_probe_disarm", th_fbn_probe_disarm, 0, 0},
    {"fbn_rec_fields", th_fbn_rec_fields, 26, 0},
    {"fbn_rec_hist_pool", th_fbn_rec_hist_pool, 9, 0},
    {"fbn_rec_item_cache", th_fbn_rec_item_cache, 13, 1},
    {"fbn_rec_topk", th_fbn_rec_topk, 18, 0},
    {"fbn_ring_slot", th_fbn_ring_slot, 12, 0},
    {"fbn_route", th_fbn_route, 14, 0},
    {"fbn_route_fc", th_fbn_route_fc, 13, 0},
    {"fbn_route_fc_status", th_fbn_route_fc_status, 8, 0},
    {"fbn_row_chunks", th_fbn_row_chunks, 1, 0},
    {"fbn_sigmoid_bwd", th_fbn_sigmoid_bwd, 5, 0},
    {"fbn_sparse_fixup", th_fbn_sparse_fixup, 14, 0},
    {"fbn_sparse_fixup_dup", th_fbn_sparse_fixup_dup, 8, 0},
    {"fbn_sparse_fold_fx", th_fbn_sparse_fold_fx, 9, 0},
    {"fbn_step_end", th_fbn_step_end, 8, 0},
    {"fbn_sum", th_fbn_sum, 4, 1},
    {"fbn_sum_jobs", th_fbn_sum_jobs, 3, 0},
    {"fbn_sum_jobs2", th_fbn_sum_jobs2, 5, 0},
    {"fbn_sum_slices", th_fbn_sum_slices, 6, 0},
    {"fbn_sumsq", th_fbn_sumsq, 6, 0},
    {"fbn_sumsq_flagged", th_fbn_sumsq_flagged, 10, 0},
    {"fbn_sumsq_sparse", th_fbn_sumsq_sparse, 8, 0},
    {"fbn_sumsq_sparse_norms", th_fbn_sumsq_sparse_norms, 12, 0},
    {"fbn_unpack_extras", th_fbn_unpack_extras, 4, 0},
    {"fbn_unpack_sumsq", th_fbn_unpack_sumsq, 6, 0},
    {"fbn_version", th_fbn_version, 0, 0},
    {"fbn_widen_bf16", th_fbn_widen_bf16, 4, 0},
};
```

ctr_recommendation_amd/ops.py:

```python
from __future__ import annotations

import os

import ctypes
from dataclasses import dataclass
from typing import Callable, Dict, Optional

import torch

from . import _lib
from ._lib import call, ptr

INT_MAX = 0x7FFFFFFF
NO_REMAP = (INT_MAX, 0, 0)
H1, H2 = 512, 256
LN_EPS = 1e-5
BN_EPS = 1e-5
BN_MOMENTUM = 0.1


_BN2_BWD_IN_FWD = os.environ.get("FBN_BN2_BWD_IN_FWD", "1") == "1"
_SPLIT_BWD = os.environ.get("FBN_SPLIT_BWD", "0") == "1"
_SPLIT3 = os.environ.get("FBN_SPLIT3", "1") != "0"
_BN1_BWD_IN_GEMM = os.environ.get("FBN_BN1_BWD_IN_GEMM", "1") == "1"
# ... 86 lines not shown
                 x: Optional[torch.Tensor] = None, images: bool = False) -> Dict[str, torch.Tensor]:
    jobs, n, out = bf16_weight_jobs(p, d, a, x, images)
    call("fbn_convert_bf16", ctypes.cast(jobs, ctypes.c_void_p).value, n, stream)
    return out


def bf16_weight_jobs(p: Dict[str, torch.Tensor], d: int, a: Dict[str, torch.Tensor],
                     x: Optional[torch.Tensor] = None, images: bool = False):
    dev = p["mlp.0.weight"].device
    KC = 15 * d
    spec = [("Wa", p["mlp.0.weight"], H1, KC, 21 * d, 0, wa_remap(d)),
            ("WaT", p["mlp.0.weight"], KC, H1, 21 * d, 1, wa_remap(d)),
            ("Wb", p["mlp.4.weight"], H2, H1, H1, 0, NO_REMAP),
            ("WbT", p["mlp.4.weight"], H1, H2, H1, 1, NO_REMAP),
            ("Wp", p["mm_proj.0.weight"], d, 128, 128, 0, NO_REMAP)]
    if "bilinear.W" in p:
        spec += [("W", p["bilinear.W"], d, d, d, 0, NO_REMAP), ("WT", p["bilinear.W"], d, d, d, 1, NO_REMAP)]
    if x is not None:
        spec.append(("x", x, x.shape[0], x.shape[1], x.shape[1], 0, NO_REMAP))
    jobs = (_ConvJob * CONV_MAX)()
    a["_conv_jobs"] = jobs
    _lib.keep(jobs)
    out = {}
    for i, (name, src, rows, cols, ld, trans, rm) in enumerate(spec):
        img = images and name in ("WaT", "WbT", "W", "x")
        key = ("s3w_" if img else "w16_") + name
        dld = wa_ld(d) if name == "Wa" else cols
        shape = (2, rows, cols) if img else (rows, dld)
        t = a.get(key)
        if t is None or tuple(t.shape) != shape:
            t = _lib.persistent(lambda: torch.zeros(shape, dtype=torch.bfloat16, device=dev))
            a[key] = t
        out[name] = t[0] if img else (t[:, :cols] if dld != cols else t)
        if name == "Wa":
            out["Wa_full"] = t
        jobs[i] = _ConvJob(src.data_ptr(), t.data_ptr(), rows, cols, ld, trans, rm[0], rm[1], rm[2],
                           2 if img else 0, dld if dld != cols else 0, rows * cols if img else 0)
    return jobs, len(spec), out


class _SumJob(ctypes.Structure):
    _fields_ = [("part", ctypes.c_void_p), ("out", ctypes.c_void_p), ("nch", ctypes.c_int), ("C", ctypes.c_int),
                ("scale", ctypes.c_float), ("beta", ctypes.c_float), ("ld", ctypes.c_int), ("pad", ctypes.c_int)]


class _SlabJob(ctypes.Structure):
    _fields_ = [("ws", ctypes.c_void_p), ("out", ctypes.c_void_p), ("M", ctypes.c_int), ("N", ctypes.c_int),
                ("ldc", ctypes.c_int), ("nsplit", ctypes.c_int), ("seg", ctypes.c_int), ("off0", ctypes.c_int),
                ("off1", ctypes.c_int), ("beta", ctypes.c_float)]


_DEFER_REDUCE = os.environ.get("FBN_DEFER_REDUCE", "1") != "0"
_WGRAD_GROUP = os.environ.get("FBN_WGRAD_GROUP", "1") != "0"


class _SlabGemm(ctypes.Structure):
    _fields_ = [("A", ctypes.c_void_p), ("B", ctypes.c_void_p), ("ws", ctypes.c_void_p), ("ws_bytes", ctypes.c_size_t),
                ("A2", ctypes.c_void_p), ("B2", ctypes.c_void_p), ("M", ctypes.c_int), ("N", ctypes.c_int),
                ("K", ctypes.c_int), ("lda", ctypes.c_int), ("ldb", ctypes.c_int), ("transA", ctypes.c_int),
                ("transB", ctypes.c_int), ("lda2", ctypes.c_int), ("kseg", ctypes.c_int), ("ldb2", ctypes.c_int),
                ("nseg", ctypes.c_int), ("s3k0", ctypes.c_int), ("lo_a", ctypes.c_longlong),
                ("lo_b", ctypes.c_longlong)]
_nsplit = ctypes.c_int(0)
_GATHER_HOT = int(os.environ.get("FBN_GATHER_HOT", "0"))


class DeferredSums:

    def __init__(self, cache: Optional[Dict[str, torch.Tensor]] = None):
        self.jobs = []
        self.slabs = []
        self.keep = []
        self.cache = cache
        self.used = set()
        self.group = []

    def add(self, part, nch, C, out, scale=1.0, beta=0.0, ld=0):
        self.jobs.append((part.data_ptr(), out.data_ptr(), int(nch), int(C), float(scale), float(beta), int(ld), 0))
        self.keep.append(part)

    def gemm_slabs(self, A, B, out, M, N, K, lda, ldb, ldc, transA, transB, rC=NO_REMAP, beta=0.0, stream=None,
                   A2=None, lda2=0, kseg=INT_MAX, B2=None, ldb2=0, nseg=INT_MAX, s3=False) -> bool:
        grouped = _WGRAD_GROUP and transA and not transB and A2 is None and M % 8 == 0 and N % 8 == 0
        if s3 and not (grouped and B2 is None and K % 64 == 0):
            return False
        lo_a, lo_b = (A[0].numel(), B[0].numel()) if s3 else (0, 0)
        K0, K = (K, 3 * K) if s3 else (0, K)
        if not (_DEFER_REDUCE and A.dtype == torch.bfloat16 and B.dtype == torch.bfloat16 and K % 64 == 0
                and lda % 8 == 0 and ldb % 8 == 0 and (not transA or M % 8 == 0) and (transB or N % 8 == 0)
                and N % 4 == 0 and ldc % 4 == 0 and all(x % 4 == 0 for x in rC[1:])
                and (rC[0] == INT_MAX or rC[0] % 4 == 0)):
            return False
        nbytes = _lib.lib().fbn_gemm_slabs_size(M, N, K)
        key = f"slab_ws_{M}_{N}_{K}"
        while key in self.used:
            key += "'"
        self.used.add(key)
        ws = self.cache.get(key) if self.cache is not None else None
        if ws is None or ws.numel() * 8 < nbytes:
            if self.cache is not None:
                ws = self.cache[key] = _lib.persistent(lambda: _ws(nbytes, out.device))
            else:
                ws = _ws(nbytes, out.device)
        st = stream if stream is not None else _lib.stream_handle()
        if grouped:
            nsplit = _lib.lib().fbn_gemm_slabs_group_split(M, N, K)
            self.group.append((A.data_ptr(), B.data_ptr(), ws.data_ptr(), nbytes, 0, ptr(B2) or 0, M, N, K, lda,
                               ldb, 1, 0, 0, 0, ldb2, nseg if B2 is not None else INT_MAX, K0, lo_a, lo_b))
            self.keep += [A, B] + ([B2] if B2 is not None else [])
        else:
            call("fbn_gemm_slabs", ptr(A), ptr(B), M, N, K, lda, ldb, int(transA), int(transB), ptr(ws), nbytes,
                 ptr(A2), lda2, kseg, ptr(B2), ldb2, nseg, ctypes.addressof(_nsplit), st)
            nsplit = _nsplit.value
        self.slabs.append((ws.data_ptr(), out.data_ptr(), M, N, ldc, nsplit, rC[0], rC[1], rC[2], float(beta)))
        self.keep.append(ws)
        return True

    def colsum(self, X, B, C, ldx, out, stream):
        nch = _lib.lib().fbn_row_chunks(B)
        part = torch.empty((nch, C), dtype=torch.float32, device=X.device)
        call("fbn_colsum_partial", ptr(X), B, C, ldx, ptr(part), stream)
        self.add(part, nch, C, out)

    def launch_group(self, stream, probe: Optional[Dict[str, list]] = None, tstream=None) -> None:
        group = [x for x in self.group if x[-3]] + [x for x in self.group if not x[-3]]
        ev = _probe_start(probe, "wgrad_group") if group else None
        while group:
            n = 0
            while n < min(6, len(group)) and bool(group[n][-3]) == bool(group[0][-3]):
                n += 1
            gc, group = group[:n], group[n:]
            garr = (_SlabGemm * len(gc))(*[_SlabGemm(*x) for x in gc])
            _lib.keep(garr)
            call("fbn_gemm_slabs_group", ctypes.addressof(garr), len(gc), stream)
        if ev is not None:
            _probe_end(ev)
            self.timed_group = True
        self.group = []

    timed_group = False

    def flush(self, stream, probe: Optional[Dict[str, list]] = None):
        self.launch_group(stream, None if self.timed_group else probe)
        jobs, slabs = self.jobs, self.slabs
        while jobs or slabs:
            jc, sc = jobs[:16], slabs[:8]
            jobs, slabs = jobs[16:], slabs[8:]
            arr = (_SumJob * max(1, len(jc)))(*[_SumJob(*j) for j in jc])
            sarr = (_SlabJob * max(1, len(sc)))(*[_SlabJob(*j) for j in sc])
            _lib.keep((arr, sarr))
            call("fbn_sum_jobs2", ctypes.addressof(arr), len(jc), ctypes.addressof(sarr), len(sc), stream)
        self.jobs, self.slabs, self.keep = [], [], []
        self.used = set()


def colsum(X, B, C, ldx, out, beta=0.0, stream=None):
    ws = _ws(_lib.lib().fbn_colsum_workspace_size(B, C), X.device)
    call("fbn_colsum", ptr(X), B, C, ldx, ptr(out), float(beta), ptr(ws),
         stream if stream is not None else _lib.stream_handle())


@dataclass
class FwdConfig:
    d: int
    L: int
    training: bool
    p_drop: float
    bf16: bool = False
    fwd16: bool = False
    bilinear_each: bool = False
    R: int = 3


class Collective:

    world = 1

    def allreduce_(self, t: torch.Tensor) -> None:
        return None


NO_COLLECTIVE = Collective()


@dataclass
class FieldsStage:
    rows: int
    device: torch.device
    fill: Callable


def bn_train_stats(h, B, C, mean, invstd, run_mean, run_var, ntot, coll: Collective, stream, tiles=None):
    dev = h.device
    if tiles is not None and coll.world <= 1:
        call("fbn_bn_tile_finalize", ptr(tiles), B, C, float(ntot), ptr(mean), ptr(invstd), ptr(run_mean),
             ptr(run_var), BN_MOMENTUM, BN_EPS, 1 if run_mean is not None else 0, stream)
        return
    s = torch.empty(C, dtype=torch.float64, device=dev)
    mean_d = torch.empty(C, dtype=torch.float64, device=dev)
    if tiles is not None:
        mom = torch.empty(2 * C, dtype=torch.float64, device=dev)
        call("fbn_bn_tile_moments", ptr(tiles), B, C, ptr(mom), stream)
        coll.allreduce_(mom)
        call("fbn_bn_moments_finalize", ptr(mom), float(ntot), C, ptr(mean), ptr(invstd), ptr(run_mean),
             ptr(run_var), BN_MOMENTUM, BN_EPS, 1 if run_mean is not None else 0, stream)
        return
# ... 251 lines not shown
             stats=t2)
    else:
        gemm(h1, p["mlp.4.weight"], h2pre, B, H2, H1, H1, H1, H2, False, True, bias=p["mlp.4.bias"], stream=st,
             stats=t2)
    if cfg.training:
        bn_train_stats(h2pre, B, H2, mean2, inv2, p["mlp.5.running_mean"], p["mlp.5.running_var"], ntot, coll, st,
                       tiles=t2)
    else:
        call("fbn_bn_eval_params", ptr(p["mlp.5.running_mean"]), ptr(p["mlp.5.running_var"]), ptr(mean2), ptr(inv2),
             H2, BN_EPS, st)
    logits, probs = buf("logits", (B,)), buf("probs", (B,))
    lt = buf("loss_terms", (B,)) if labels is not None else None
    go = buf("gout", (B,)) if labels is not None else None
    bpart = None
    if labels is not None and cfg.training and coll.world <= 1 and _BN2_BWD_IN_FWD:
        bpart = buf("bn2_bwd_part", (_lib.lib().fbn_bn_bwd_chunks(B, H2) * 3 * H2,), torch.float64)
    a["bn2_bwd_part"] = bpart
    bscale = 1.0 / (1.0 - cfg.p_drop) if (cfg.training and cfg.p_drop > 0) else 1.0
    call("fbn_bn_act_head_fwd", ptr(h2pre), ptr(h2), B, H2, ptr(mean2), ptr(inv2), ptr(p["mlp.5.weight"]),
         ptr(p["mlp.5.bias"]), float(p_drop), ptr(rng), 2, ptr(m2), ptr(mi2), ptr(p["mlp.8.weight"]),
         ptr(p["mlp.8.bias"]), ptr(logits), ptr(probs), ptr(labels), ptr(lt), ptr(go),
         float(loss_denom if loss_denom is not None else ntot), ptr(bpart), float(bscale), st)
    if cfg.training and count_batches and "mlp.1.num_batches_tracked" in p:
        p["mlp.1.num_batches_tracked"].add_(1)
        p["mlp.5.num_batches_tracked"].add_(1)
    a["err"] = err
    a["B"] = B
    return a


class _SideWork:

    def __init__(self, side: Optional["torch.cuda.Stream"], dev):
        self.side = side
        self.dev = dev
        self.main = torch.cuda.current_stream(dev) if side is not None else None

    def run(self, fn):
        if self.side is None:
            fn(_lib.stream_handle(self.dev))
            return
        _lib.wait_stream(self.side, self.main)
        with torch.cuda.stream(self.side):
            fn(self.side.cuda_stream)

    def join(self):
        if self.side is not None:
            _lib.wait_stream(self.main, self.side)


def backward(p: Dict[str, torch.Tensor], batch: Dict[str, torch.Tensor], a: Dict[str, torch.Tensor],
             gout: torch.Tensor, g: Dict[str, torch.Tensor], cfg: FwdConfig, *,
             table_grad: Optional[torch.Tensor] = None, gvec: Optional[torch.Tensor] = None,
             gnorm: Optional[torch.Tensor] = None,
             pos: Optional[torch.Tensor] = None,
             sendbuf: Optional[torch.Tensor] = None, coll: Collective = NO_COLLECTIVE,
             ntot: Optional[int] = None, extra_sums=(), side: Optional["torch.cuda.Stream"] = None,
             probe: Optional[Dict[str, list]] = None, hooks: Optional[Dict[str, object]] = None) -> None:
    d, L = cfg.d, cfg.L
    B = a["B"]
    dev = gout.device
    st = _lib.stream_handle(dev)
    ntot = B if ntot is None else ntot
    KC = 15 * d
    scale = 1.0 / (1.0 - cfg.p_drop) if (cfg.training and cfg.p_drop > 0) else 1.0
    f32 = dict(dtype=torch.float32, device=dev)
    bf = cfg.bf16
    w16 = a.get("w16")
    bf16_ = dict(dtype=torch.bfloat16, device=dev)
    lean = bf and coll.world <= 1

    def tmp(name, shape, dtype=torch.float32):
        t = a.get("bwd_" + name)
        if t is None or tuple(t.shape) != tuple(shape) or t.dtype != dtype:
            t = _lib.persistent(lambda: torch.empty(shape, dtype=dtype, device=dev))
            a["bwd_" + name] = t
        return t

    sb = 2 if (cfg.fwd16 and _SPLIT_BWD) else False
    s3 = cfg.fwd16 and _SPLIT3 and not bf and not cfg.bilinear_each
    s3img = s3 and bool(a.get("s3img"))
    im = {}

    def img(name, rows, cols):
        return tmp("s3_" + name, (2, rows, cols), torch.bfloat16)

    if s3:
        jobs = []
        for name, src, rows, cols, ld, trans, rm in (("WbT", p["mlp.4.weight"], H1, H2, H1, 1, NO_REMAP),
                                                     ("WaT", p["mlp.0.weight"], KC, H1, 21 * d, 1, wa_remap(d)),
                                                     ("W", p["bilinear.W"], d, d, d, 0, NO_REMAP),
                                                     ("x", batch["item_emb_d128"], B, 128, 128, 0, NO_REMAP)):
            t = a.get("s3w_" + name) if a.get("s3w") else None
            if t is not None and tuple(t.shape) == (2, rows, cols):
                im[name] = t
            else:
                im[name] = img(name, rows, cols)
                jobs.append((src, im[name], rows, cols, ld, trans, rm))
        if s3img:
            im["h1"] = a["s3_h1"]
        else:
            im["h1"] = img("h1", B, H1)
            jobs.append((a["h1"], im["h1"], B, H1, H1, 0, NO_REMAP))
        if a.get("s3img"):
            im["Vc"] = a["s3_vc"]
        else:
            im["Vc"] = img("Vc", 5 * B, d)
            jobs.append((a["Vc"], im["Vc"], 5 * B, d, d, 0, NO_REMAP))
        if a.get("s3_c") is not None and tuple(a["s3_c"].shape) == (2, B, KC):
            im["c"] = a["s3_c"]
        else:
# ... 108 lines not shown
    elif not cfg.bilinear_each:
        if bf:
            if not sums.gemm_slabs(a["Vc16"], dU16, g["bilinear.W"], d, d, 5 * B, d, d, d, True, False, stream=st):
                wg.run(lambda s: gemm(a["Vc16"], dU16, g["bilinear.W"], d, d, 5 * B, d, d, d, True, False, stream=s))
            gemm(dU16, w16["W"], dV, 5 * B, d, d, d, d, d, False, True, beta=1.0, stream=st)
        elif s3:
            if dU is not None:
                dU2 = img("dU", 5 * B, d)
                split_images([(dU, dU2, 5 * B, d, d, 0, NO_REMAP)], st)
            if not sums.gemm_slabs(im["Vc"], dU2, g["bilinear.W"], d, d, 5 * B, d, d, d, True, False, stream=st,
                                   s3=True):
                wg.run(lambda s: gemm(a["Vc"], dU, g["bilinear.W"], d, d, 5 * B, d, d, d, True, False, stream=s))
            if s3_ok(5 * B, d, d, d, d, False, True):
                gemm_s3(dU2, im["W"], dV, 5 * B, d, d, d, d, d, False, True, beta=1.0, stream=st)
            else:
                gemm(dU, p["bilinear.W"], dV, 5 * B, d, d, d, d, d, False, True, beta=1.0, stream=st)
        else:
            wg.run(lambda s: gemm(a["Vc"], dU, g["bilinear.W"], d, d, 5 * B, d, d, d, True, False, bf16=sb,
                                  stream=s))
            gemm(dU, p["bilinear.W"], dV, 5 * B, d, d, d, d, d, False, True, beta=1.0, bf16=sb, stream=st)
    else:
        g["bilinear.W_list.0"].zero_()
        for f in range(1, 5):
            gemm(dU[:, f - 1], p[f"bilinear.W_list.{f}"], dV[:, f - 1], B, d, d, 5 * d, d, 5 * d, False, True,
                 beta=1.0, bf16=cfg.bf16, stream=st)
            gemm(a["Vc"][:, f - 1], dU[:, f - 1], g[f"bilinear.W_list.{f}"], d, d, B, 5 * d, 5 * d, d, True, False,
                 bf16=cfg.bf16, stream=st)
    if hooks and "after_bilinear_bwd" in hooks:
        hooks["after_bilinear_bwd"](sums)
    R = cfg.R
    ncate = p["cate_emb.weight"].shape[0]
    P = _lib.lib().fbn_fields_bwd_partials_size(d, R, ncate)
    nblk = _lib.lib().fbn_fields_bwd_grid(B, d)
    partials = tmp("partials", (nblk, P))
    dhmm = tmp("dhmm", (B, d))
    dhmm16 = tmp("dhmm16", (B, d), torch.bfloat16) if bf else None
    dhs = img("dhmm", B, d) if s3 else None
    seq = batch.get("item_seq", None)
    Lr = 0 if seq is None else L
    V = p["item_emb.weight"].shape[0] if pos is None else 0
    keys = ("senet.excitation.0.weight", "senet.excitation.0.bias", "senet.excitation.2.weight",
            "senet.excitation.2.bias", "mm_proj.1.weight", "mm_proj.1.bias", "cate_emb.weight", "mm_proj.0.bias")
    if _DEFER_REDUCE:
        outs = None
        o = 0
        for k, n in zip(keys, (6 * R, R, 6 * R, 6, d, d, ncate * d, d)):
            sums.add(partials[:, o:], nblk, n, g[k], ld=P)
            o += n
    else:
        outs_arr = (ctypes.c_void_p * 8)(*[g[k].data_ptr() for k in keys])
        _lib.keep(outs_arr)
        outs = ctypes.cast(outs_arr, ctypes.c_void_p).value
    evb = _probe_start(probe, "fields_bwd")
    call("fbn_fields_bwd_img" if s3img else "fbn_fields_bwd", ptr(batch["item_id"]), ptr(seq) if Lr else None,
         ptr(batch["likes_level"]),
         ptr(batch["views_level"]), ptr(a["hmm"]), ptr(p["mm_proj.1.weight"]), ptr(p["mm_proj.1.bias"]), LN_EPS,
         ptr(p["senet.excitation.0.weight"]), ptr(p["senet.excitation.0.bias"]), ptr(p["senet.excitation.2.weight"]),
         R, ncate, ptr(p["cate_emb.weight"]), ptr(a["X"]), ptr(a["a"]), ptr(a["cnt"]), ptr(dV), ptr(dhmm),
         ptr(dhs if s3img else dhmm16), ptr(partials), outs,
         ptr(table_grad), ptr(gvec), ptr(gnorm), V, ptr(pos), ptr(sendbuf),
         int(sendbuf is not None and sendbuf.dtype == torch.bfloat16), B, Lr, d, st)
    _probe_end(evb)
    if hooks and "after_fields_bwd" in hooks:
        hooks["after_fields_bwd"]()
    if bf:
        if not sums.gemm_slabs(dhmm16, w16["x"], g["mm_proj.0.weight"], d, 128, B, d, 128, 128, True, False,
                               stream=st):
            wg.run(lambda s: gemm(dhmm16, w16["x"], g["mm_proj.0.weight"], d, 128, B, d, 128, 128, True, False,
                                  stream=s))
    elif s3:
        if not s3img:
            split_images([(dhmm, dhs, B, d, d, 0, NO_REMAP)], st)
        if not sums.gemm_slabs(dhs, im["x"], g["mm_proj.0.weight"], d, 128, B, d, 128, 128, True, False,
                               stream=st, s3=True):
            wg.run(lambda s: gemm(dhmm, batch["item_emb_d128"], g["mm_proj.0.weight"], d, 128, B, d, 128, 128, True,
                                  False, stream=s))
    else:
        wg.run(lambda s: gemm(dhmm, batch["item_emb_d128"], g["mm_proj.0.weight"], d, 128, B, d, 128, 128, True,
                              False, bf16=sb, stream=s))
    for job in extra_sums:
        sums.add(*job)
    if hooks and "before_flush" in hooks:
        hooks["before_flush"]()
    sums.flush(st, probe)
    wg.join()
```

ctr_recommendation_amd/trainer.py:

```python
from __future__ import annotations

import ctypes
import os
from typing import Dict, List, Optional

import numpy as np
import torch
import torch.distributed as dist

from . import _lib, ops
from ._lib import call, ptr
from .exchange import DistCollective, NativeComm, RowExchange, native_comm_wanted
from .model_fibinet import build_model

_W16_MODE = os.environ.get("FBN_W16", "main")
_SIDE_AFTER_MLP0 = os.environ.get("FBN_SIDE_AFTER_MLP0", "0") == "1"
_SIDE_AFTER_MMPROJ = os.environ.get("FBN_SIDE_AFTER_MMPROJ", "0") == "1"
_CLAIM_ON_SIDE = os.environ.get("FBN_CLAIM_ON_SIDE", "0") == "1"
_HEAD_CONV = os.environ.get("FBN_HEAD_CONV", "1") != "0"
_SIDE_SERIAL = os.environ.get("FBN_SIDE_SERIAL", "auto")
_SIDE_ORDER = os.environ.get("FBN_SIDE_ORDER", "wp")
_FIXUP_ON_SIDE = os.environ.get("FBN_FIXUP_ON_SIDE", "auto")
_JOIN_ONCE = True
_SIDE_AFTER_GATHER = os.environ.get("FBN_SIDE_AFTER_GATHER", "0") == "1"
_ROUTE_AFTER_COMPUTE = os.environ.get("FBN_ROUTE_AFTER_COMPUTE", "1") == "1"
_DENSE_SUMSQ_FOLD = os.environ.get("FBN_DENSE_SUMSQ_FOLD", "1") == "1"
_EARLY_GRAD_XCHG = os.environ.get("FBN_EARLY_GRAD_XCHG")
_WGRAD_EARLY = os.environ.get("FBN_WGRAD_EARLY", "0") == "1"
_PF_BINNED = os.environ.get("FBN_PF_BINNED", "0") == "1"
_FC = os.environ.get("FBN_FC", "1") != "0"
_FC_CAP = int(os.environ.get("FBN_FC_CAP", "0"))
_FC_MARGIN = float(os.environ.get("FBN_FC_MARGIN", "1.25"))
FC_CALIB_STEPS = 2
FBN_GRAD_CELL = 0x20000
FBN_GRAD_BF16 = 0x40000
FBN_RING_BF16 = 0x40000000
_RING_BF16 = os.environ.get("FBN_RING_BF16", "0") == "1"
_OWNER_PF2 = os.environ.get("FBN_OWNER_PF2", "1") != "0"
_OWNER_CLAIM_FUSED = os.environ.get("FBN_OWNER_CLAIM_FUSED", "1") != "0"
_SHARD_W16_SIDE = os.environ.get("FBN_SHARD_W16_SIDE", "1") != "0"
_OWNER_FOLD = os.environ.get("FBN_OWNER_FOLD", "1") != "0"
_CHECK_POOL = os.environ.get("FBN_CHECK_POOL", "0") == "1"
from .schedule import OneCycle, adam_table

TABLE = "item_emb.weight"
FBN_GRAD_FULL = 0x10000
FROZEN = ("user_emb.weight",)
BUFFERS = ("mlp.1.running_mean", "mlp.1.running_var", "mlp.1.num_batches_tracked",
           "mlp.5.running_mean", "mlp.5.running_var", "mlp.5.num_batches_tracked")


def _events(probe, name, stream=None):
    if probe is None:
        return None
    kp = _lib.KernelProbe()
    probe.setdefault(name, []).append((kp, None))
    return kp


def _events_end(kp, stream=None):
    if kp is not None:
        kp.done()


def default_lazy_window(d: int) -> int:
    return 128 if d >= 128 else 32


def _side_stream(dev):
    mask = os.environ.get("FBN_SIDE_CU_MASK")
    if not mask:
        return torch.cuda.Stream(device=dev)
    words = [int(w, 16) for w in mask.split(",")]
    ncu = torch.cuda.get_device_properties(dev).multi_processor_count
    n = (ncu + 31) // 32
    arr = (ctypes.c_uint32 * n)(*[words[i % len(words)] for i in range(n)])
    hip = ctypes.CDLL("libamdhip64.so")
    s = ctypes.c_void_p()
    with torch.cuda.device(dev):
        rc = hip.hipExtStreamCreateWithCUMask(ctypes.byref(s), n, arr)
    if rc != 0:
        raise RuntimeError(f"hipExtStreamCreateWithCUMask failed ({rc})")
    return torch.cuda.ExternalStream(s.value, device=dev)


class _Segments:

    def __init__(self, base, pool):
        self.base, self.world, self.pool = base, base.world, pool
        self.prog: list = []
        self.cur = None

    def begin(self) -> None:
        self.cur = torch.cuda.CUDAGraph()
# ... 161 lines not shown
                                   decoupled_wd=self.wd if self.decoupled else 0.0)
        self.sched = torch.from_numpy(tab).to(dev)
        self.step_dev = torch.zeros(1, **i32)
        seed_d = dropout_seed if dropout_seed is not None else (seed * 1000003 + 17)
        seed_d += rank * 0x9E3779B9
        self.rng = torch.tensor([seed_d & 0x7FFFFFFFFFFF, 0], dtype=torch.int64, device=dev)
        self.sumsq = torch.zeros(64, dtype=torch.float64, device=dev)
        self.sumsq_tab = torch.zeros(64, dtype=torch.float64, device=dev)
        self.coef = torch.ones(1, dtype=torch.float32, device=dev)
        self.norm = torch.zeros(1, dtype=torch.float32, device=dev)
        self.err = torch.zeros(1, **i32)
        self.loss = torch.zeros(1, dtype=torch.float32, device=dev)
        self.host_step = 0
        self.acts: Dict[str, torch.Tensor] = {}
        self.native_comm = NativeComm(world, rank, group, dev) \
            if (sharded or world > 1) and native_comm_wanted(dev, group, stage_on_cpu, force=native_comm) else None
        self.coll = DistCollective(world, group, stage_on_cpu, comm=self.native_comm, det=self.deterministic)
        self.sync_bn = bool(model_cfg.get("sync_bn", True) if sync_bn is None else sync_bn)
        self.bn_coll = self.coll if self.sync_bn else ops.NO_COLLECTIVE
        self.side = _side_stream(dev)
        self.xchg = RowExchange(rank, world, self.V, d, self.B, max_len, dev, group, stage_on_cpu=stage_on_cpu,
                                rows_bf16=self.fcfg.bf16, side=self.side, comm=self.native_comm) if sharded else None
        self.stage_on_cpu = stage_on_cpu
        self._eval_metrics = None
        self.early_grad_xchg = _EARLY_GRAD_XCHG == "1"
        self.table_adam = os.environ.get("FBN_TABLE_ADAM", table_adam)
        if self.table_adam not in ("lazy", "eager", "sparse"):
            raise ValueError(f"table_adam must be 'lazy', 'eager' or 'sparse', not {self.table_adam!r}")
        self.lazy_window = int(lazy_window) if lazy_window is not None else default_lazy_window(d)
        self.side_serial = _SIDE_SERIAL == "1" or (_SIDE_SERIAL == "auto" and d < 128)
        self.last = self.row_state[:, 2]
        self.deferred = self.table_adam == "lazy" and defer_table_grads
        self.pend = self.ring = self.coef_hist = None
        self.ring_n = self.lazy_window + 1
        self.ring_cap = self.B * (max_len + 1) if sharded else 0
        self.ring_bf16 = bool(sharded and self.fcfg.bf16 and _RING_BF16 and self.deferred)
        if self.deferred:
            self.pend = self.row_state[:, 3]
            shape = (self.ring_n, self.B, 2, d) if not sharded else (self.ring_n, self.ring_cap, d)
            self.ring = self._new_ring(shape)
            self.coef_hist = torch.ones(total_steps + 1, dtype=torch.float32, device=dev)
            self.ticket = torch.zeros(17, dtype=torch.int32, device=dev)
        self.shard_graph = self.sharded and os.environ.get("FBN_SHARD_GRAPH", "1") != "0"
        self._late_side = None
        self._sg = None
        self._sg_eager = 0
        self._bn_synced_at = -1
        self._used_pre = False
        self._recording = False
        self.fc_wanted = self.sharded and _FC and self.device.type == "cuda"
        self._fc_seen = 0
        self._fc_steps = 0
        self.ring_cell = torch.zeros(2, dtype=torch.int64, device=dev)
        self._fc_grad = None
        self._fc_extra = None
        self._fc_part = None

    def step(self, batch: Dict[str, torch.Tensor], labels: torch.Tensor,
             masks_out: Optional[Dict[str, torch.Tensor]] = None, probe: Optional[Dict[str, list]] = None,
             next_batch: Optional[Dict[str, torch.Tensor]] = None) -> torch.Tensor:
        if self.host_step >= self.total_steps:
            raise ValueError(f"Tried to step {self.host_step + 1} times. The specified number of total steps is "
                             f"{self.total_steps}")
        st = _lib.stream_handle(self.device)
        B = batch["item_id"].shape[0]
        if B > self.B:
            raise ValueError(f"batch of {B} rows exceeds the trainer's batch_size {self.B}")
        ntot = B * self.world
        d = self.d
        cfg = self.fcfg
        seq = batch.get("item_seq")
        L = cfg.L = seq.shape[1] if seq is not None else 0
        if L > self.L:
            raise ValueError(f"history length {L} exceeds max_len {self.L}")
        rows = pos = None
        main = torch.cuda.current_stream(self.device)

        lazy = self.table_adam == "lazy"

        side_hooks = {}

        def catch_up(n_ent, claim=False, before_side=None, on_side=None):
            if on_side is not None:
                _lib.wait_event(self.side, on_side)
                ev = _events(probe, "adam_catchup", self.side)
                key = _batch_key(batch["item_id"], seq if L else None)
                pre = self.preclaim if (self.preclaim is not None and key == self._pre_key) else None
                self._used_pre = pre is not None
                self._pre_key = None
                call("fbn_adam_claim_catchup", ptr(batch["item_id"]), ptr(seq) if L else None, B, L, self.V,
                     ptr(self.map), ptr(self.slot_row), ptr(self.dup), ptr(self.hasdup), ptr(pre), ptr(self.E),
                     ptr(self.Em), ptr(self.Ev), self.rows_local, d, self.lazy_window, ptr(self.last),
                     ptr(self.sched), ptr(self.step_dev), self.wd_g, self.beta2, self.eps, *self._pend_args(),
                     int(self.decoupled), self.side.cuda_stream)
                _events_end(ev, self.side)
                claim_ev = torch.cuda.Event()
                _lib.record_event(claim_ev, self.side)
                side_hooks["before_gather"] = lambda: _lib.wait_event(main, claim_ev)
                side_pass(wait_main=False)
                return
            ev = _events(probe, "adam_catchup")
            if claim:
                key = _batch_key(batch["item_id"], seq if L else None)
                pre = self.preclaim if (self.preclaim is not None and key == self._pre_key) else None
                self._used_pre = pre is not None
                self._pre_key = None
# ... 121 lines not shown
            if lazy and _OWNER_CLAIM_FUSED:
                def owner_claim_catchup(ids, n):
                    ev = _events(probe, "adam_catchup")
                    pre = self.row_state.view(torch.int64)[:, 0] if (self.prefetch_owner and _OWNER_PF2) else None
                    call("fbn_adam_owner_claim_catchup", ptr(ids), n, int(self.rank == 0), ptr(self.map),
                         ptr(self.slot_row), ptr(pre), ptr(self.E), ptr(self.Em), ptr(self.Ev), self.rows_local, d,
                         self.lazy_window, ptr(self.last), ptr(self.sched), ptr(self.step_dev), self.wd_g,
                         self.beta2, self.eps, *self._pend_args(), int(self.decoupled), st)
                    _events_end(ev)
                    side_pass()
                sparse["claim_catchup"] = owner_claim_catchup
            rows = self.xchg.forward(batch["item_id"], seq, self.E, sparse, self.err,
                                     before_gather=catch_up if lazy else None)
            pos = self.xchg.cur_pos
            fwd_ev = torch.cuda.Event()
            _lib.record_event(fwd_ev, main)
        route_ahead = None
        if self.xchg is not None and next_batch is not None:
            def route_ahead():
                own = self.prefetch_owner and lazy
                self.xchg.prepare(next_batch["item_id"], next_batch.get("item_seq"), self.err, send_rows=own,
                                  after=fwd_ev)
                if own and self.xchg.next_lids is not None:
                    _lib.wait_stream(self.side, self.xchg.side)
                    ev = _events(probe, "adam_prefetch", self.side)
                    call("fbn_adam_prefetch_rows", ptr(self.xchg.next_lids), self.xchg.next_lids.numel(),
                         int(self.rank == 0), self.rows_local, ptr(self.map),
                         ptr(self.row_state.view(torch.int64)[:, 0]) if _OWNER_PF2 else None, ptr(self.E), ptr(self.Em),
                         ptr(self.Ev), d, ptr(self.last), ptr(self.sched), ptr(self.step_dev), self.wd_g, self.beta2,
                         self.eps, *self._pend_args(), int(self.decoupled), self.side.cuda_stream)
                    _events_end(ev, self.side)
                    self.xchg.next_lids.record_stream(self.side)
            if not _ROUTE_AFTER_COMPUTE:
                route_ahead()
                route_ahead = None
        elif self.xchg is None and lazy:
            if w16_late:
                step_start = torch.cuda.Event()
                _lib.record_event(step_start, main)
                catch_up(B * (L + 1), claim=True, before_side=step_start)
                w16_ev = self._w16_ev
            else:
                catch_up(B * (L + 1), claim=True, on_side=claim_side)
        elif self.xchg is None:
            call("fbn_claim_rows", ptr(batch["item_id"]), ptr(seq) if L else None, B, L, self.V, ptr(self.map),
                 ptr(self.slot_row), ptr(self.dup), ptr(self.hasdup), st)
        if w16_ev is not None:
            _lib.wait_event(main, w16_ev)
        graphed = False
        fixup_side = (self.xchg is None and (_FIXUP_ON_SIDE == "1" or (_FIXUP_ON_SIDE == "auto" and not self.side_serial
                                                                        and not torch.cuda.is_current_stream_capturing()))
                      and not self.deterministic and L > 0
                      and not self._early_grad_xchg())
        if (self.xchg is not None and self.shard_graph and probe is None and masks_out is None
                and self.table_adam != "eager" and not self._recording):
            sendbuf = self.xchg.make_sendbuf()
            graphed = self._sharded_compute(batch, labels, pos, cfg, ntot, B, L)
        if not graphed:
            a = ops.forward(self.p, batch, cfg, self.rng, table_rows=rows, pos=pos, err=self.err, labels=labels,
                            w16_ready=w16_ev is not None or w16_main,
                            loss_denom=float(ntot), coll=self.bn_coll, ntot=self._bn_n(ntot, B), acts=self.acts,
                            masks_out=masks_out,
                            probe=probe, count_batches=False,
                            after_gather=start_untouched_adam if self.table_adam == "eager" else None,
                            hooks=side_hooks)
            if self._late_side is not None:
                self._late_side()
                self._late_side = None
            sendbuf = self.xchg.make_sendbuf() if self.xchg is not None else None
            bhooks = {"after_fields_bwd": self._grad_xchg_start} if self._early_grad_xchg() else None
            if fixup_side:
                def fork_fixup():
                    _lib.wait_stream(self.side, main)
                    call("fbn_sparse_fixup_dup", ptr(self.dup), B * (L + 1), ptr(self.gvec), ptr(self.extra),
                         ptr(self.slot_row), L + 1, d, self.side.cuda_stream)
                bhooks = {"after_fields_bwd": fork_fixup}
                if _WGRAD_EARLY and cfg.bf16:
                    def early_wgrad(sums):
                        _lib.wait_stream(self.side, main)
                        sums.launch_group(self.side.cuda_stream, probe, tstream=self.side)
                    bhooks["after_bilinear_bwd"] = early_wgrad
                    bhooks["before_flush"] = lambda: _lib.wait_stream(main, self.side)
            ops.backward(self.p, batch, a, a["gout"], self.g, cfg, gvec=self.gvec if self.xchg is None else None,
                         gnorm=self.gnorm if self.xchg is None else None,
                         pos=pos, sendbuf=sendbuf, coll=self.bn_coll, ntot=self._bn_n(ntot, B),
                         extra_sums=[(a["loss_terms"], B, 1, self.loss, 1.0 / ntot)], probe=probe,
                         hooks=bhooks)
        dense_work = None
        if self.sharded and self._early_grad_xchg() and self.native_comm is None and not self.coll.det:
            dense_work = dist.all_reduce(self.flat_g, group=self.coll.group, async_op=True)
        if route_ahead is not None:
            route_ahead()
        joined = False
        fold_done = False
        if self.xchg is None:
            n_ent = B * (L + 1)
            if self.deterministic:
                if L == 0:
                    raise ValueError("deterministic mode needs the item_seq history (L > 0)")
                gsrc = (self.gvec, self.extra, (L + 1) | FBN_GRAD_FULL)
                call("fbn_sparse_fold_fx", ptr(self.dup), ptr(self.hasdup), n_ent, ptr(self.gvec), ptr(self.slot_row),
                     gsrc[2], d, ptr(self.fx), st)
            else:
                gsrc = (self.gvec, self.extra, L + 1)
                if fixup_side:
                    _lib.wait_stream(main, self.side)
                    joined = True
                else:
                    call("fbn_sparse_fixup_dup", ptr(self.dup), n_ent, ptr(self.gvec), ptr(self.extra),
                         ptr(self.slot_row), L + 1, d, st)
        else:
            x = self.xchg
            n_ent = x.n_recv
            fold_done = False
            if x.fc_active:
                wire = x.backward_finish() if x._pending is not None else x.backward(sendbuf)
                defer_now = self.deferred and n_ent <= self.ring_cap
                lo, cnt = x.fc_self_rows
                if self._fc_extra is None or self._fc_extra.shape[0] < n_ent:
                    self._fc_extra = _lib.persistent(
                        lambda: torch.zeros((n_ent, d), dtype=torch.float32, device=self.device))
                if defer_now:
                    ring, ring_n, stride = self.ring, self._ring_n_arg(), self._ring_stride()
                else:
                    if self._fc_grad is None or self._fc_grad.shape[0] < n_ent:
                        self._fc_grad = _lib.persistent(
                            lambda: torch.empty((n_ent, d), dtype=torch.float32, device=self.device))
                    ring, ring_n, stride = self._fc_grad, 1, n_ent * d
                rb = FBN_GRAD_BF16 if (defer_now and self.ring_bf16) else 0
                if _OWNER_FOLD or self.deterministic or rb:
                    fx = self._fold_bufs(n_ent)
                    call("fbn_owner_fold", ptr(x.recv_ids), n_ent, self.rank, ptr(self.map), ptr(self.slot_row),
                         ptr(wire), int(wire.dtype == torch.bfloat16), ptr(x.fc_send) if cnt else None, lo, cnt,
                         ptr(ring), ring_n, stride, ptr(self.step_dev), ptr(self.ring_cell), ptr(self._fc_extra), d,
                         ptr(self._fc_part), ptr(fx), st)
                    gsrc = (self.ring_cell, self._fc_extra,
                            1 | FBN_GRAD_CELL | rb | (FBN_GRAD_FULL if fx is not None else 0))
                    fold_done = True
                else:
                    call("fbn_ring_slot", ptr(ring), ring_n, stride, ptr(self.step_dev), ptr(self.ring_cell),
                         ptr(wire), int(wire.dtype == torch.bfloat16), n_ent * d, ptr(x.fc_send) if cnt else None,
                         lo * d, cnt * d, st)
                    gsrc = (self.ring_cell, None, 1 | FBN_GRAD_CELL)
            else:
                slot = self._grad_slot()
                defer_now = slot is not None
                if x._pending is not None:
                    grows = x.backward_finish()
                else:
                    grows = x.backward(sendbuf, out=slot)
                gsrc = (grows, None, 1)
                g16 = grows.dtype == torch.bfloat16
                if (self.deterministic or g16) and n_ent > 0:
                    fx = self._fold_bufs(n_ent)
                    call("fbn_owner_fold", ptr(x.recv_ids), n_ent, self.rank, ptr(self.map), ptr(self.slot_row),
                         ptr(grows), int(g16), None, 0, 0, ptr(grows), 1 | (FBN_RING_BF16 if g16 else 0), n_ent * d,
                         ptr(self.step_dev), ptr(self.ring_cell), ptr(self._fc_extra), d, ptr(self._fc_part), ptr(fx),
                         st)
                    gsrc = (self.ring_cell, self._fc_extra, 1 | FBN_GRAD_CELL | (FBN_GRAD_BF16 if g16 else 0) |
                            (FBN_GRAD_FULL if fx is not None else 0))
                    fold_done = True
            if not fold_done:
                call("fbn_sparse_fixup", None, None, ptr(x.recv_ids), n_ent, 0, self.V, self.rank, ptr(self.map),
                     ptr(gsrc[0]), None, ptr(self.slot_row), gsrc[2], d, st)
        tab_acc = self.sumsq_tab if self.sharded else self.sumsq
        dense_done = False
        if self.xchg is None and L > 0:
            fold = not self.sharded and _DENSE_SUMSQ_FOLD
            call("fbn_sumsq_sparse_norms", ptr(self.gnorm), ptr(gsrc[0]), ptr(gsrc[1]), ptr(self.slot_row), gsrc[2],
                 n_ent, d, ptr(tab_acc), ptr(self.fx), ptr(self.flat_g) if fold else None,
                 self.n_dense if fold else 0, st)
            dense_done = fold
        elif fold_done:
            call("fbn_sumsq_flagged", ptr(self.slot_row), n_ent, ptr(self.ring_cell), ptr(self._fc_extra), d,
                 ptr(self._fc_part), ptr(tab_acc), ptr(self._fx_sh) if self.deterministic else None,
                 int(bool(gsrc[2] & FBN_GRAD_BF16)), st)
        else:
            call("fbn_sumsq_sparse", ptr(gsrc[0]), ptr(gsrc[1]), ptr(self.slot_row), gsrc[2], n_ent, d, ptr(tab_acc),
                 st)
        if self.sharded:
            o = self.n_dense
            call("fbn_pack_extras", ptr(self.loss), ptr(self.sumsq_tab), ptr(self.flat_g_ext[o:]), st)
            if dense_work is not None:
                dist.all_reduce(self.flat_g_ext[o:o + 2], group=self.coll.group)
                dense_work.wait()
            else:
                self.coll.allreduce_(self.flat_g_ext[:o + 2])
            if not dense_done:
                call("fbn_unpack_sumsq", ptr(self.flat_g_ext[o:]), ptr(self.loss), ptr(self.flat_g), self.n_dense,
                     ptr(self.sumsq), st)
                dense_done = True
            else:
                call("fbn_unpack_extras", ptr(self.flat_g_ext[o:]), ptr(self.loss), ptr(self.sumsq), st)
        if not dense_done:
            call("fbn_sumsq", ptr(self.flat_g), self.n_dense, None, 0, ptr(self.sumsq), st)
        if not (joined and _JOIN_ONCE):
            _lib.wait_stream(main, self.side)
        if self.xchg is None:
            defer_now = self.deferred
        if defer_now:
            ev = _events(probe, "adam_tail")
            call("fbn_adam_step_tail", ptr(self.flat_p), ptr(self.flat_g), ptr(self.flat_m), ptr(self.flat_v),
                 self.n_dense, ptr(self.sumsq), self.max_norm, ptr(self.coef), ptr(self.norm), ptr(self.E),
                 ptr(self.Em), ptr(self.Ev), d, ptr(self.map), ptr(gsrc[0]), ptr(gsrc[1]), ptr(self.slot_row), gsrc[2],
                 n_ent, ptr(self.sched), ptr(self.step_dev), self.wd_g, self.beta2, self.eps, ptr(self.last),
                 ptr(self.pend), ptr(self.ring), ptr(self.coef_hist), self._ring_n_arg(), self._ring_stride(), self.B,
                 ptr(self.rng),
                 ptr(self.p["mlp.1.num_batches_tracked"]), ptr(self.p["mlp.5.num_batches_tracked"]), ptr(self.ticket),
                 self.total_steps, ptr(self.err), st)
            _events_end(ev)
        else:
            call("fbn_adam_dense", ptr(self.flat_p), ptr(self.flat_g), ptr(self.flat_m), ptr(self.flat_v),
                 self.n_dense, None, ptr(self.sched), ptr(self.step_dev), self.wd_g, self.beta2, self.eps,
                 ptr(self.sumsq), self.max_norm, ptr(self.coef), ptr(self.norm), st)
            ev = _events(probe, "adam_touched")
            call("fbn_adam_touched", ptr(self.E), ptr(self.Em), ptr(self.Ev), d, ptr(self.map), ptr(gsrc[0]),
                 ptr(gsrc[1]), ptr(self.slot_row), gsrc[2], n_ent, ptr(self.coef), ptr(self.sched),
                 ptr(self.step_dev), self.wd_g, self.beta2, self.eps, ptr(self.last) if lazy else None, st)
            _events_end(ev)
            self.slot_row[:n_ent].fill_(-1)
# ... 381 lines not shown
```

include/fibinet.h:

```cpp
#ifndef FIBINET_H
#define FIBINET_H

#include <stddef.h>
#include <stdint.h>

#ifdef __cplusplus
extern "C" {
#endif

#define FBN_OK 0
#define FBN_ERR_ARG 1
#define FBN_ERR_LAUNCH 2
#define FBN_ERR_UNSUPPORTED 3

const char* fbn_last_error(void);
int fbn_probe_arm(int slot);
int fbn_probe_disarm(void);
float fbn_probe_elapsed(int slot);
int fbn_version(void);
int fbn_device_ok(void);

size_t fbn_gemm_workspace_size(int M, int N, int K, int bf16);
int fbn_gemm(const void* A, const void* B, float* C, const float* bias, int M, int N, int K, int lda, int ldb,
             int ldc, int transA, int transB, int rB_seg, int rB_off0, int rB_off1, int rC_seg, int rC_off0,
             int rC_off1, float beta, int bf16, int a16, int b16, float* stats, float* ws, size_t ws_bytes,
             void* stream);
size_t fbn_gemm_slabs_size(int M, int N, int K);
int fbn_gemm_slabs(const void* A, const void* B, int M, int N, int K, int lda, int ldb, int transA, int transB,
                   float* ws, size_t ws_bytes, const void* A2, int lda2, int kseg, const void* B2, int ldb2, int nseg,
                   int* nsplit, void* stream);
int fbn_gemm_slabs_split(int M, int N, int K);
int fbn_gemm_slabs_group(const void* descs, int n, void* stream);
int fbn_gemm_slabs_group_split(int M, int N, int K);
int fbn_gemm_bf16out(const void* A, const void* B, void* C, int M, int N, int K, int lda, int ldb, int ldc,
                     int transA, int transB, void* stream);
int fbn_gemm_s3(const void* A, const void* B, float* C, int M, int N, int K0, int lda, int ldb, int ldc, int transA,
                int transB, long long lo_a, long long lo_b, float beta, float* ws, size_t ws_bytes, void* stream);
int fbn_gemm_bn_bwd_part_supported(int M, int N, int K, int lda, int ldb, int transA, int transB);
int fbn_gemm_bn_bwd_part(const void* A, const void* B, float* C, int M, int N, int K, int lda, int ldb, int ldc,
                         int transA, int transB, const short* hact16, const float* xpre, const float* mean, float scale,
                         double* part, void* stream);
int fbn_gemm_split(const void* A, const void* B, float* C, const float* bias, int M, int N, int K, int lda, int ldb,
                   int ldc, int transA, int transB, int rC_seg, int rC_off0, int rC_off1, float beta, float* stats,
                   float* ws, size_t ws_bytes, const void* A2, int lda2, int kseg, const void* B2, int ldb2, int nseg,
                   void* stream);

int fbn_fields_fwd(const int64_t* item_id, const int64_t* item_seq, const int64_t* likes, const int64_t* views,
                   const float* hmm, const float* ln_g, const float* ln_b, float ln_eps, const float* cate, int n_cate,
                   const float* table, long long V, const int* pos, const float* w1, const float* b1, const float* w2,
                   const float* b2, int R, float* X, float* Vc, short* Vc16, void* c, int ldc, int c_bf16, float* a_out,
                   float* cnt_out,
                   int* err, int* map, int* slot_row, int B, int L, int D, int rows_bf16, void* stream);
int fbn_hot_rows(const int64_t* item, const int64_t* seq, int B, int L, long long V, int* cnt, int* hot, int* hot_n,
                 int H, int tau, int clear, void* stream);
int fbn_fields_fwd_hot(const int64_t* item_id, const int64_t* item_seq, const int64_t* likes, const int64_t* views,
                       const float* hmm, const float* ln_g, const float* ln_b, float ln_eps, const float* cate,
                       int n_cate, const float* table, long long V, const float* w1, const float* b1, const float* w2,
                       const float* b2, int R, float* X, float* Vc, short* Vc16, void* c, int ldc, int c_bf16,
                       float* a_out, float* cnt_out, int* err, int* map, int* slot_row, int B, int L, int D,
                       const int* hot, const int* hot_n, int H, void* stream);

int fbn_fields_bwd_partials_size(int D, int R, int n_cate);
int fbn_fields_bwd_grid(int B, int D);
int fbn_fields_bwd(const int64_t* item_id, const int64_t* item_seq, const int64_t* likes, const int64_t* views,
                   const float* hmm, const float* ln_g, const float* ln_b, float ln_eps, const float* w1,
                   const float* b1, const float* w2, int R, int n_cate, const float* cate, const float* X, const float* a, const float* cnt, const float* dV, float* dhmm,
                   short* dhmm16, float* partials, float* const* param_grads, float* gtab, float* gvec,
                   double* gnorm, long long V, const int* pos, void* sendbuf, int send_bf16, int B, int L, int D,
                   void* stream);
int fbn_fields_bwd_img(const int64_t* item_id, const int64_t* item_seq, const int64_t* likes, const int64_t* views,
                       const float* hmm, const float* ln_g, const float* ln_b, float ln_eps, const float* w1,
                       const float* b1, const float* w2, int R, int n_cate, const float* cate, const float* X,
                       const float* a, const float* cnt, const float* dV, float* dhmm, void* dhmm_img,
                       float* partials, float* const* param_grads, float* gtab, float* gvec, double* gnorm,
                       long long V, const int* pos, void* sendbuf, int send_bf16, int B, int L, int D, void* stream);

int fbn_pairs_fwd(const float* Vc, const short* Vc16, const float* U, void* c, int B, int D, int ldc, int mode,
                  int c_bf16, void* stream);
int fbn_pairs_fwd_img(const float* Vc, const float* U, void* c_img, void* vc_img, int B, int D, int ldc, void* stream);
int fbn_pairs_bwd_img(const float* dc, const float* Vc, const float* U, float* dV, void* dU_img, int B, int D, int ldc,
                      void* stream);
int fbn_pairs_bwd(const float* dc, const float* Vc, const short* Vc16, const float* U, float* dV, float* dU,
                  short* dU16, int B, int D, int ldc, int mode, void* stream);

size_t fbn_bn_workspace_size(int B, int C);
int fbn_bn_stats_pass(const float* X, int B, int C, const double* mean_d, double* out_d, void* ws, void* stream);
int fbn_bn_mean(const double* sum_d, double ntot, int C, double* mean_d, void* stream);
int fbn_bn_finalize(const double* m2_d, const double* mean_d, double ntot, int C, float* mean, float* invstd,
                    float* run_mean, float* run_var, float momentum, float eps, int update_running, void* stream);
int fbn_bn_stats(const float* X, int B, int C, float* mean, float* invstd, float* run_mean, float* run_var,
                 float momentum, float eps, int update_running, void* ws, void* stream);
int fbn_bn_tile_stats(const float* part, int M, int C, const double* mean_d, double* out_d, void* stream);
int fbn_bn_tile_moments(const float* part, int M, int C, double* out_d, void* stream);
int fbn_bn_moments_finalize(const double* mom_d, double ntot, int C, float* mean, float* invstd, float* run_mean,
                            float* run_var, float momentum, float eps, int update_running, void* stream);
int fbn_bn_tile_finalize(const float* part, int M, int C, double ntot, float* mean, float* invstd, float* run_mean,
                         float* run_var, float momentum, float eps, int update_running, void* stream);
int fbn_bn_eval_params(const float* run_mean, const float* run_var, float* mean, float* invstd, int C, float eps,
                       void* stream);
int fbn_bn_act_fwd(const float* X, float* Y, int B, int C, const float* mean, const float* invstd, const float* g,
                   const float* b, float p_drop, const unsigned long long* rng, unsigned stream_id,
                   unsigned char* mask_out, const unsigned char* mask_in, short* Y16, void* stream);
int fbn_bn_act_fwd_img(const float* X, float* Y, int B, int C, const float* mean, const float* invstd, const float* g,
                       const float* b, float p_drop, const unsigned long long* rng, unsigned stream_id,
                       unsigned char* mask_out, const unsigned char* mask_in, void* Y_img, void* stream);
int fbn_bn_act_head_fwd(const float* X, float* Y, int B, int C, const float* mean, const float* invstd, const float* g,
                        const float* b, float p_drop, const unsigned long long* rng, unsigned stream_id,
                        unsigned char* mask_out, const unsigned char* mask_in, const float* hw, const float* hbias,
                        float* logits, float* probs, const float* labels, float* loss_terms, float* gout, float denom,
                        double* bwd_part, float bwd_scale, void* stream);
int fbn_bn_bwd_reduce(const float* G, const float* gvec, const float* w, const float* hact, float scale,
                      const float* Xpre, const float* mean, int B, int C, double* red_d, void* ws, void* stream);
int fbn_bn_bwd_apply(const float* G, const float* gvec, const float* w, const float* hact, float scale,
                     const float* Xpre, const float* mean, const float* invstd, const float* gamma, int B, int C,
                     const double* red_d, double ntot, float* dXpre, short* dXpre16, float* dgamma, float* dbeta,
                     float* dw, void* ws, void* stream);
int fbn_bn_bwd(const float* G, const float* gvec, const float* w, const float* hact, float scale, const float* Xpre,
               const float* mean, const float* invstd, const float* gamma, int B, int C, float* dXpre, float* dgamma,
               float* dbeta, float* dw, void* ws, void* stream);
size_t fbn_bn_colpart_size(int B, int C);
int fbn_row_chunks(int B);
int fbn_bn_bwd_chunks(int B, int C);
int fbn_bn_bwd_fused(const float* G, const float* gvec, const float* w, const float* hact, const short* hact16,
                     float scale, const float* Xpre, const float* mean, const float* invstd, const float* gamma, int B,
                     int C, double ntot, float* dXpre, short* dXpre16, float* dgamma, float* dbeta, float* dw,
                     float* colpart, const double* part_pre, void* ws, void* stream);
int fbn_bn_bwd_fused_img(const float* G, const float* gvec, const float* w, const float* hact, const short* hact16,
                         float scale, const float* Xpre, const float* mean, const float* invstd, const float* gamma,
                         int B, int C, double ntot, float* dXpre, void* dXpre_img, float* dgamma, float* dbeta,
                         float* dw, float* colpart, const double* part_pre, void* ws, void* stream);
int fbn_convert_bf16(const void* jobs, int n, void* stream);
size_t fbn_colsum_workspace_size(int B, int C);
int fbn_colsum(const float* X, int B, int C, int ldx, float* out, float beta, void* ws, void* stream);
int fbn_colsum_partial(const float* X, int B, int C, int ldx, float* part, void* stream);
int fbn_sum_jobs(const void* jobs, int n, void* stream);
int fbn_sum_jobs2(const void* jobs, int n, const void* slabs, int ns, void* stream);

int fbn_head_fwd(const float* H, const float* w, const float* bias, int B, int C, float* logits, float* probs,
                 const float* labels, float* loss_terms, float* gout, float denom, void* stream);
int fbn_sigmoid_bwd(const float* gp, const float* probs, float* gout, int B, void* stream);
int fbn_outer(const float* g, const float* w, float* out, int B, int C, void* stream);
int fbn_sum(const float* x, int n, float* out, float scale, void* stream);

int fbn_sumsq(const float* x, long long n, const int* n_rows, int row_len, double* out, void* stream);
int fbn_clip_coef(const double* sumsq, float max_norm, float* coef, float* norm, void* stream);
int fbn_adam_dense(float* p, const float* g, float* m, float* v, long long n, const float* coef,
                   const void* consts_table, const int* step, float wd, float beta2, float eps, const double* sumsq,
                   float max_norm, float* coef_out, float* norm_out, void* stream);
int fbn_sparse_fixup(const int64_t* item, const int64_t* seq, const int* ids, int n, int L, long long V, int rank,
                     const int* map, const float* gvec, float* extra, int* slot_row, int Lp1, int D, void* stream);
int fbn_sumsq_sparse(const float* gvec, float* extra, int* slot_row, int Lp1, int n, int D, double* out,
                     void* stream);
int fbn_sparse_fixup_dup(const int* dup, int n, const float* gvec, float* extra, int* slot_row, int Lp1, int D,
                         void* stream);
int fbn_sumsq_sparse_norms(const double* gnorm, const float* gvec, float* extra, int* slot_row, int Lp1, int n, int D,
                           double* out, unsigned long long* fx, const float* dense, long long n_dense, void* stream);
#define FBN_GRAD_FULL 0x10000
#define FBN_GRAD_CELL 0x20000
#define FBN_GRAD_BF16 0x40000
#define FBN_RING_BF16 0x40000000
int fbn_sparse_fold_fx(const int* dup, int* hasdup, int n, const float* gvec, int* slot_row, int Lp1, int D,
                       unsigned long long* acc, void* stream);
int fbn_adam_table(float* p, float* m, float* v, long long nrows, int D, int* map, const float* gvec, float* extra,
                   int* slot_row, int Lp1, const float* coef, const void* consts_table, const int* step, float wd,
                   float beta2, float eps, int mode, void* stream);
int fbn_adam_touched(float* p, float* m, float* v, int D, int* map, const float* gvec, float* extra, int* slot_row,
                     int Lp1, int n, const float* coef, const void* consts_table, const int* step, float wd,
                     float beta2, float eps, int* last, void* stream);
#define FBN_ROW_STATE_BYTES 16
int fbn_adam_catchup(float* p, float* m, float* v, long long nrows, int D, const int* slot_row, int n_ent,
                     const int* map, int F, int parts, int* last, const void* consts_table, const int* step, float wd,
                     float beta2, float eps, int* pend, const float* ring, const float* coef_hist,
                     long long ring_stride, int ring_n, int decoupled, void* stream);
int fbn_adam_owner_claim_catchup(const int* lids, int n, int skip0, int* map, int* slot_row,
                                 unsigned long long* preclaim, float* p, float* m, float* v, long long nrows, int D,
                                 int F, int* last, const void* consts_table, const int* step, float wd, float beta2,
                                 float eps, int* pend, const float* ring, const float* coef_hist, long long ring_stride,
                                 int ring_n, int decoupled, void* stream);
int fbn_adam_claim_catchup(const int64_t* item, const int64_t* seq, int B, int L, long long V, int* map, int* slot_row,
                           int* dup, int* hasdup, unsigned long long* preclaim, float* p, float* m, float* v,
                           long long nrows, int D, int F, int* last,
                           const void* consts_table, const int* step, float wd, float beta2, float eps, int* pend,
                           const float* ring, const float* coef_hist, long long ring_stride, int ring_n, int decoupled,
                           void* stream);
int fbn_adam_claim_catchup_conv(const int64_t* item, const int64_t* seq, int B, int L, long long V, int* map,
                                int* slot_row, int* dup, int* hasdup, unsigned long long* preclaim, float* p,
                                float* m, float* v, long long nrows, int D, int F, int* last,
                                const void* consts_table, const int* step, float wd, float beta2, float eps,
                                int* pend, const float* ring, const float* coef_hist, long long ring_stride,
// ... 135 lines not shown
```

Baseline: 20.47 million samples/s.

## Write table grads into ring slot and fold dense grad norm into sum jobs

The fields backward kernel can now write the sparse-table gradient vector straight into a ring-buffer slot picked on the device from the step counter, and it publishes the slot pointer through a cell. This removes a separate gvec buffer and the copy that would otherwise follow. Separately, the dense-gradient sum-of-squares for clipping is fused into the final sum/slab reduction kernel, with extra blocks covering other gradient ranges, so a standalone norm pass is skipped. The cost is more complex kernels, double atomics spread over 64 slots, and a one-time check that unwritten gradient columns are zero.

```diff
diff --git a/ctr_recommendation_amd/_lib.py b/ctr_recommendation_amd/_lib.py
--- a/ctr_recommendation_amd/_lib.py
+++ b/ctr_recommendation_amd/_lib.py
@@ -43,6 +43,7 @@
     "fbn_colsum_partial": (I, [P, I, I, I, P, P]),
     "fbn_sum_jobs": (I, [P, I, P]),
     "fbn_sum_jobs2": (I, [P, I, P, I, P]),
+    "fbn_sum_jobs_sq": (I, [P, I, P, I, P, I, P, P]),
     "fbn_gemm_slabs_size": (SZ, [I, I, I]),
     "fbn_gemm_slabs": (I, [P, P, I, I, I, I, I, I, I, P, SZ, P, I, I, P, I, I, P, P]),
     "fbn_gemm_slabs_split": (I, [I, I, I]),
@@ -59,6 +60,8 @@
                            I, I, P]),
     "fbn_fields_bwd_img": (I, [P, P, P, P, P, P, P, F, P, P, P, I, I, P, P, P, P, P, P, P, P, P, P, P, P, LL, P, P, I,
                                I, I, I, P]),
+    "fbn_fields_bwd_slot": (I, [P, P, P, P, P, P, P, F, P, P, P, I, I, P, P, P, P, P, P, P, I, P, P, P, I, LL, P, P, P,
+                                LL, I, I, I, P]),
     "fbn_pairs_fwd": (I, [P, P, P, P, I, I, I, I, I, P]),
     "fbn_pairs_bwd": (I, [P, P, P, P, P, P, P, I, I, I, I, P]),
     "fbn_pairs_fwd_img": (I, [P, P, P, P, I, I, I, P]),
diff --git a/ctr_recommendation_amd/csrc/fields.hip b/ctr_recommendation_amd/csrc/fields.hip
--- a/ctr_recommendation_amd/csrc/fields.hip
+++ b/ctr_recommendation_amd/csrc/fields.hip
@@ -271,6 +271,7 @@
   float* partials;
   float* gtab; float* gvec;
   double* gnorm;
+  const int* slot_step; float** slot_cell; long long ring_stride; int ring_n;
   const int* pos; void* sendbuf;
   long long V;
   int B, L, R, n_cate;
@@ -297,7 +298,7 @@
   atomicAdd(row + 3 * G + q, t[3]);
 }
 
-template <int D, int MODE, int RMAX>
+template <int D, int MODE, int RMAX, bool SLOT = false>
 __global__ void __launch_bounds__(256) fields_bwd_kernel(FieldBwdArgs p) {
   FBN_MAIN_PRIO();
   constexpr int G = D / 4;
@@ -322,6 +323,11 @@
   const int gw = (blockIdx.x * blockDim.x + threadIdx.x) >> 6;
   const int nwaves = (gridDim.x * blockDim.x) >> 6;
   const int L = p.L;
+  float* gvec = p.gvec;
+  if constexpr (SLOT) {
+    gvec += (size_t)(__builtin_amdgcn_readfirstlane(*p.slot_step) % p.ring_n) * p.ring_stride;
+    if (blockIdx.x == 0 && threadIdx.x == 0) *p.slot_cell = gvec;
+  }
   f32x4 acc_lg = {0.f, 0.f, 0.f, 0.f}, acc_lb = {0.f, 0.f, 0.f, 0.f}, acc_hb = {0.f, 0.f, 0.f, 0.f};
   float acc_se[SJ];
 #pragma unroll
@@ -444,8 +450,8 @@
       }
       const f32x4 gh = dx[4] / p.cnt[b];
       if (MODE == 0 && p.gvec) {
-        *reinterpret_cast<f32x4*>(p.gvec + (size_t)b * 2 * D + 4 * q) = dx[2];
-        *reinterpret_cast<f32x4*>(p.gvec + ((size_t)b * 2 + 1) * D + 4 * q) = gh;
+        *reinterpret_cast<f32x4*>(gvec + (size_t)b * 2 * D + 4 * q) = dx[2];
+        *reinterpret_cast<f32x4*>(gvec + ((size_t)b * 2 + 1) * D + 4 * q) = gh;
         if (p.gnorm) {
           double si = 0.0, sh = 0.0;
 #pragma unroll
@@ -695,17 +701,17 @@
 extern "C" int fbn_fields_bwd_partials_size(int D, int R, int n_cate) { return 13 * R + 6 + 3 * D + n_cate * D; }
 extern "C" int fbn_fields_bwd_grid(int B, int D) { return fields_grid(B, D, FBN_FB_MAXBLK); }
 
-template <int MODE, int RMAX>
+template <int MODE, int RMAX, bool SLOT = false>
 static int launch_fields_bwd_r(const FieldBwdArgs& a, int D, hipStream_t st) {
   const int grid = fields_grid(a.B, D, FBN_FB_MAXBLK);
   const size_t lds = (4 * (size_t)(13 * a.R + 6 + 3 * D + a.n_cate * D) + 4 * (64 / (D / 4)) * (12 + 2 * RMAX)) *
                      sizeof(float);
   switch (D) {
-    case 16: fbn_launch((fields_bwd_kernel<16, MODE, RMAX>), dim3(grid), dim3(256), lds, st, a); break;
-    case 32: fbn_launch((fields_bwd_kernel<32, MODE, RMAX>), dim3(grid), dim3(256), lds, st, a); break;
-    case 64: fbn_launch((fields_bwd_kernel<64, MODE, RMAX>), dim3(grid), dim3(256), lds, st, a); break;
-    case 128: fbn_launch((fields_bwd_kernel<128, MODE, RMAX>), dim3(grid), dim3(256), lds, st, a); break;
-    case 256: fbn_launch((fields_bwd_kernel<256, MODE, RMAX>), dim3(grid), dim3(256), lds, st, a); break;
+    case 16: fbn_launch((fields_bwd_kernel<16, MODE, RMAX, SLOT>), dim3(grid), dim3(256), lds, st, a); break;
+    case 32: fbn_launch((fields_bwd_kernel<32, MODE, RMAX, SLOT>), dim3(grid), dim3(256), lds, st, a); break;
+    case 64: fbn_launch((fields_bwd_kernel<64, MODE, RMAX, SLOT>), dim3(grid), dim3(256), lds, st, a); break;
+    case 128: fbn_launch((fields_bwd_kernel<128, MODE, RMAX, SLOT>), dim3(grid), dim3(256), lds, st, a); break;
+    case 256: fbn_launch((fields_bwd_kernel<256, MODE, RMAX, SLOT>), dim3(grid), dim3(256), lds, st, a); break;
     default: fbn_set_error("fields: embedding_dim must be one of 16,32,64,128,256"); return FBN_ERR_UNSUPPORTED;
   }
   FBN_CHECK_LAUNCH();
@@ -714,6 +720,9 @@
 
 template <int MODE>
 static int launch_fields_bwd(const FieldBwdArgs& a, int D, hipStream_t st) {
+  if constexpr (MODE == 0)
+    if (a.slot_step)
+      return a.R <= 3 ? launch_fields_bwd_r<0, 3, true>(a, D, st) : launch_fields_bwd_r<0, FBN_MAXR, true>(a, D, st);
   return a.R <= 3 ? launch_fields_bwd_r<MODE, 3>(a, D, st) : launch_fields_bwd_r<MODE, FBN_MAXR>(a, D, st);
 }
 
@@ -723,7 +732,8 @@
                            const float* cate, const float* X, const float* a, const float* cnt, const float* dV,
                            float* dhmm, short* dhmm16, float* partials, float* const* param_grads, float* gtab,
                            float* gvec, double* gnorm, long long V, const int* pos, void* sendbuf, int send_bf16,
-                           int B, int L, int D, void* stream, long long dhmm16_lo);
+                           int B, int L, int D, void* stream, long long dhmm16_lo, const int* slot_step = nullptr,
+                           void* slot_cell = nullptr, int ring_n = 0, long long ring_stride = 0);
 extern "C" int fbn_fields_bwd(const int64_t* item_id, const int64_t* item_seq, const int64_t* likes,
                               const int64_t* views, const float* hmm, const float* ln_g, const float* ln_b,
                               float ln_eps, const float* w1, const float* b1, const float* w2, int R, int n_cate,
@@ -747,13 +757,31 @@
                          cnt, dV, dhmm, (short*)dhmm_img, partials, param_grads, gtab, gvec, gnorm, V, pos, sendbuf,
                          send_bf16, B, L, D, stream, (long long)B * D);
 }
+extern "C" int fbn_fields_bwd_slot(const int64_t* item_id, const int64_t* item_seq, const int64_t* likes,
+                                   const int64_t* views, const float* hmm, const float* ln_g, const float* ln_b,
+                                   float ln_eps, const float* w1, const float* b1, const float* w2, int R, int n_cate,
+                                   const float* cate, const float* X, const float* a, const float* cnt, const float* dV,
+                                   float* dhmm, void* dhmm16, int dhmm_is_img, float* partials,
+                                   float* const* param_grads, float* ring, int ring_n, long long ring_stride,
+                                   const int* step, void* cell, double* gnorm, long long V, int B, int L, int D,
+                                   void* stream) {
+  if (!ring || !step || !cell || ring_n < 1 || ring_stride < (long long)B * 2 * D || (ring_stride & 3) ||
+      ((uintptr_t)ring & 15) || (dhmm_is_img && !dhmm16)) {
+    fbn_set_error("fbn_fields_bwd_slot: ring (16-B aligned), step, cell; ring_n >= 1, ring_stride >= B*2*D, % 4 == 0");
+    return FBN_ERR_ARG;
+  }
+  return fields_bwd_impl(item_id, item_seq, likes, views, hmm, ln_g, ln_b, ln_eps, w1, b1, w2, R, n_cate, cate, X, a,
+                         cnt, dV, dhmm, (short*)dhmm16, partials, param_grads, nullptr, ring, gnorm, V, nullptr, nullptr,
+                         0, B, L, D, stream, dhmm_is_img ? (long long)B * D : 0, step, cell, ring_n, ring_stride);
+}
 static int fields_bwd_impl(const int64_t* item_id, const int64_t* item_seq, const int64_t* likes,
                            const int64_t* views, const float* hmm, const float* ln_g, const float* ln_b,
                            float ln_eps, const float* w1, const float* b1, const float* w2, int R, int n_cate,
                            const float* cate, const float* X, const float* a, const float* cnt, const float* dV,
                            float* dhmm, short* dhmm16, float* partials, float* const* param_grads, float* gtab,
                            float* gvec, double* gnorm, long long V, const int* pos, void* sendbuf, int send_bf16,
-                           int B, int L, int D, void* stream, long long dhmm16_lo) {
+                           int B, int L, int D, void* stream, long long dhmm16_lo, const int* slot_step,
+                           void* slot_cell, int ring_n, long long ring_stride) {
   if (B <= 0) return FBN_OK;
   if (L < 0 || L > 32 || R < 1 || R > FBN_MAXR) { fbn_set_error("fbn_fields_bwd: bad L/R"); return FBN_ERR_ARG; }
   FieldBwdArgs p;
@@ -761,6 +789,7 @@
   p.hmm = hmm; p.ln_g = ln_g; p.ln_b = ln_b; p.w1 = w1; p.b1 = b1; p.w2 = w2; p.cate = cate;
   p.X = X; p.a = a; p.cnt = cnt; p.dV = dV; p.dhmm = dhmm; p.dhmm16 = dhmm16; p.partials = partials;
   p.dhmm16_lo = dhmm16_lo;
+  p.slot_step = slot_step; p.slot_cell = (float**)slot_cell; p.ring_n = ring_n; p.ring_stride = ring_stride;
   p.gtab = gtab; p.gvec = gvec; p.gnorm = gvec ? gnorm : nullptr; p.pos = pos; p.sendbuf = sendbuf;
   p.V = V; p.B = B; p.L = L; p.R = R; p.n_cate = n_cate; p.ln_eps = ln_eps;
   hipStream_t st = (hipStream_t)stream;
diff --git a/ctr_recommendation_amd/csrc/mlp.hip b/ctr_recommendation_amd/csrc/mlp.hip
--- a/ctr_recommendation_amd/csrc/mlp.hip
+++ b/ctr_recommendation_amd/csrc/mlp.hip
@@ -829,7 +829,7 @@
   int nch, C;
   float scale, beta;
   int ld;
-  int pad_;
+  int sq;
 };
 struct SlabJob {
   const float* ws;
@@ -841,6 +841,13 @@
 #define FBN_SUM_WIDE 32
 #define FBN_MAX_SLAB_JOBS 8
 #define FBN_SLAB_GROUPS 4
+#define FBN_SUMSQ_SLOTS 64
+#define FBN_MAX_SQ_RANGES 24
+#define FBN_SQ_RANGE_BLOCK 1024
+struct SqRange {
+  const float* x;
+  long long n;
+};
 struct SumJobs {
   SumJob j[FBN_MAX_SUM_JOBS];
   int col0[FBN_MAX_SUM_JOBS + 1];
@@ -849,11 +856,20 @@
   int blk0[FBN_MAX_SLAB_JOBS + 1];
   int ns;
 };
+struct SumSq {
+  double* out;
+  SqRange r[FBN_MAX_SQ_RANGES];
+  int rblk0[FBN_MAX_SQ_RANGES + 1];
+  int nr;
+};
+__device__ __forceinline__ double sq4(const f32x4& t) {
+  return ((double)(t[0] * t[0]) + (double)(t[1] * t[1])) + ((double)(t[2] * t[2]) + (double)(t[3] * t[3]));
+}
 #define FBN_SLAB_DIRECT 8
-__device__ __forceinline__ void slab_direct(const SlabJob& sj, int lb) {
+__device__ __forceinline__ double slab_direct(const SlabJob& sj, int lb) {
   const size_t total = (size_t)sj.M * sj.N;
   const size_t i4 = (size_t)lb * 256 + threadIdx.x;
-  if (i4 >= total / 4) return;
+  if (i4 >= total / 4) return 0.0;
   const float* src = sj.ws + i4 * 4;
   f32x4 x[FBN_SLAB_DIRECT];
 #pragma unroll
@@ -867,16 +883,14 @@
   float* cp = sj.out + (size_t)m * sj.ldc + n + (n < sj.seg ? sj.off0 : sj.off1);
   if (sj.beta != 0.f) t += sj.beta * *reinterpret_cast<const f32x4*>(cp);
   *reinterpret_cast<f32x4*>(cp) = t;
-}
-__device__ __forceinline__ void slab_block(const SumJobs& J, int gb) {
+  return sq4(t);
+}
+__device__ __forceinline__ double slab_block(const SumJobs& J, int gb) {
   __shared__ f32x4 red[FBN_SLAB_GROUPS][64];
   int u = 0;
   while (u + 1 < J.ns && gb >= J.blk0[u + 1]) ++u;
   const SlabJob sj = J.s[u];
-  if (sj.nsplit <= FBN_SLAB_DIRECT) {
-    slab_direct(sj, gb - J.blk0[u]);
-    return;
-  }
+  if (sj.nsplit <= FBN_SLAB_DIRECT) return slab_direct(sj, gb - J.blk0[u]);
   const int qd = threadIdx.x & 63, grp = threadIdx.x >> 6;
   const size_t total = (size_t)sj.M * sj.N;
   const size_t i4 = (size_t)(gb - J.blk0[u]) * 64 + qd;
@@ -904,9 +918,11 @@
     float* cp = sj.out + (size_t)m * sj.ldc + n + (n < sj.seg ? sj.off0 : sj.off1);
     if (sj.beta != 0.f) t += sj.beta * *reinterpret_cast<const f32x4*>(cp);
     *reinterpret_cast<f32x4*>(cp) = t;
-  }
-}
-__device__ __forceinline__ void sum_wide_block(const SumJob& jb, int c0) {
+    return sq4(t);
+  }
+  return 0.0;
+}
+__device__ __forceinline__ double sum_wide_block(const SumJob& jb, int c0) {
   __shared__ float red[16][17];
   const int col = threadIdx.x & 15, str = threadIdx.x >> 4, c = c0 + col;
   const size_t ld = jb.ld > 0 ? jb.ld : jb.C;
@@ -926,23 +942,20 @@
 #pragma unroll
     for (int k = 0; k < 16; ++k) t += red[k][col];
     t *= jb.scale;
-    jb.out[c] = jb.beta != 0.f ? jb.beta * jb.out[c] + t : t;
-  }
-}
-__global__ void __launch_bounds__(256) sum_jobs_kernel(SumJobs J) {
+    t = jb.beta != 0.f ? jb.beta * jb.out[c] + t : t;
+    jb.out[c] = t;
+    return jb.sq ? (double)(t * t) : 0.0;
+  }
+  return 0.0;
+}
+__device__ __forceinline__ double sum_jobs_block(const SumJobs& J) {
   __shared__ float red[4];
   const int gc = blockIdx.x;
-  if (gc >= J.col0[J.n]) {
-    slab_block(J, gc - J.col0[J.n]);
-    return;
-  }
+  if (gc >= J.col0[J.n]) return slab_block(J, gc - J.col0[J.n]);
   int u = 0;
   while (u + 1 < J.n && gc >= J.col0[u + 1]) ++u;
   const SumJob jb = J.j[u];
-  if (jb.C >= FBN_SUM_WIDE) {
-    sum_wide_block(jb, (gc - J.col0[u]) * 16);
-    return;
-  }
+  if (jb.C >= FBN_SUM_WIDE) return sum_wide_block(jb, (gc - J.col0[u]) * 16);
   const int c = gc - J.col0[u];
   const size_t ld = jb.ld > 0 ? jb.ld : jb.C;
   float a0 = 0.f, a1 = 0.f, a2 = 0.f, a3 = 0.f;
@@ -958,8 +971,39 @@
   if ((threadIdx.x & 63) == 0) red[threadIdx.x >> 6] = v;
   __syncthreads();
   if (threadIdx.x == 0) {
-    const float t = jb.scale * ((red[0] + red[1]) + (red[2] + red[3]));
-    jb.out[c] = jb.beta != 0.f ? jb.beta * jb.out[c] + t : t;
+    float t = jb.scale * ((red[0] + red[1]) + (red[2] + red[3]));
+    t = jb.beta != 0.f ? jb.beta * jb.out[c] + t : t;
+    jb.out[c] = t;
+    return jb.sq ? (double)(t * t) : 0.0;
+  }
+  return 0.0;
+}
+__global__ void __launch_bounds__(256) sum_jobs_kernel(SumJobs J) { (void)sum_jobs_block(J); }
+__global__ void __launch_bounds__(256) sum_jobs_sq_kernel(SumJobs J, SumSq Q) {
+  __shared__ double sred[4];
+  const int nsum = J.col0[J.n] + J.blk0[J.ns];
+  double acc = 0.0;
+  if ((int)blockIdx.x < nsum) {
+    acc = sum_jobs_block(J);
+  } else {
+    const int rb = blockIdx.x - nsum;
+    int u = 0;
+    while (u + 1 < Q.nr && rb >= Q.rblk0[u + 1]) ++u;
+    const SqRange r = Q.r[u];
+    const long long i0 = (long long)(rb - Q.rblk0[u]) * FBN_SQ_RANGE_BLOCK + threadIdx.x;
+#pragma unroll
+    for (int k = 0; k < FBN_SQ_RANGE_BLOCK / 256; ++k) {
+      const long long i = i0 + k * 256;
+      const float v = i < r.n ? r.x[i] : 0.f;
+      acc += (double)(v * v);
+    }
+  }
+  for (int o = 32; o > 0; o >>= 1) acc += __shfl_xor(acc, o, 64);
+  if ((threadIdx.x & 63) == 0) sred[threadIdx.x >> 6] = acc;
+  __syncthreads();
+  if (threadIdx.x == 0) {
+    const double t = (sred[0] + sred[1]) + (sred[2] + sred[3]);
+    if (t != 0.0) atomicAdd(Q.out + (blockIdx.x & (FBN_SUMSQ_SLOTS - 1)), t);
   }
 }
 
@@ -1426,7 +1470,21 @@
 
 extern "C" int fbn_row_chunks(int B) { return row_chunks(B); }
 
+static int sum_jobs_impl(const SumJob* jobs, int n, const SlabJob* slabs, int ns, const SqRange* ranges, int nr,
+                         double* sumsq, void* stream);
 extern "C" int fbn_sum_jobs2(const SumJob* jobs, int n, const SlabJob* slabs, int ns, void* stream) {
+  return sum_jobs_impl(jobs, n, slabs, ns, nullptr, 0, nullptr, stream);
+}
+extern "C" int fbn_sum_jobs_sq(const SumJob* jobs, int n, const SlabJob* slabs, int ns, const SqRange* ranges, int nr,
+                               double* sumsq, void* stream) {
+  if (!sumsq || nr < 0 || nr > FBN_MAX_SQ_RANGES || (nr > 0 && !ranges)) {
+    fbn_set_error("fbn_sum_jobs_sq: sumsq and at most 24 ranges");
+    return FBN_ERR_ARG;
+  }
+  return sum_jobs_impl(jobs, n, slabs, ns, ranges, nr, sumsq, stream);
+}
+static int sum_jobs_impl(const SumJob* jobs, int n, const SlabJob* slabs, int ns, const SqRange* ranges, int nr,
+                         double* sumsq, void* stream) {
   if (n < 0 || ns < 0 || n > FBN_MAX_SUM_JOBS || ns > FBN_MAX_SLAB_JOBS) {
     fbn_set_error("fbn_sum_jobs2: too many jobs");
     return FBN_ERR_ARG;
@@ -1452,6 +1510,24 @@
     J.blk0[i + 1] = J.blk0[i] + (int)fbn_cdiv((long long)sj.M * sj.N / 4, qpb);
   }
   const int blocks = J.col0[n] + J.blk0[ns];
+  if (sumsq) {
+    SumSq Q;
+    Q.out = sumsq;
+    Q.nr = nr;
+    Q.rblk0[0] = 0;
+    for (int i = 0; i < nr; ++i) {
+      if (!ranges[i].x || ranges[i].n < 0) {
+        fbn_set_error("fbn_sum_jobs_sq: null range");
+        return FBN_ERR_ARG;
+      }
+      Q.r[i] = ranges[i];
+      Q.rblk0[i + 1] = Q.rblk0[i] + (int)fbn_cdiv(ranges[i].n, (long long)FBN_SQ_RANGE_BLOCK);
+    }
+    if (blocks + Q.rblk0[nr] <= 0) return FBN_OK;
+    fbn_launch(sum_jobs_sq_kernel, dim3(blocks + Q.rblk0[nr]), dim3(256), 0, (hipStream_t)stream, J, Q);
+    FBN_CHECK_LAUNCH();
+    return FBN_OK;
+  }
   if (blocks <= 0) return FBN_OK;
   fbn_launch(sum_jobs_kernel, dim3(blocks), dim3(256), 0, (hipStream_t)stream, J);
   FBN_CHECK_LAUNCH();
diff --git a/ctr_recommendation_amd/csrc/optim.hip b/ctr_recommendation_amd/csrc/optim.hip
--- a/ctr_recommendation_amd/csrc/optim.hip
+++ b/ctr_recommendation_amd/csrc/optim.hip
@@ -275,6 +275,7 @@
 
 template <int D>
 __global__ void __launch_bounds__(FBN_FOLD_THREADS) sparse_fixup_dup_kernel(const int* __restrict__ dup, int n, GradSrc s) {
+  resolve_src(s);
   constexpr int NPL = D / 64 > 0 ? D / 64 : 1;
   constexpr int MAXV = 16;
   constexpr int CPW = FBN_FOLD_CHUNKS;
@@ -395,6 +396,7 @@
 template <int D>
 __global__ void __launch_bounds__(256) sparse_fold_fx_kernel(const int* __restrict__ dup, int* __restrict__ hasdup,
                                                              int n, GradSrc s, unsigned long long* __restrict__ acc) {
+  resolve_src(s);
   const int lane = threadIdx.x & 63;
   for (long long e0 = ((long long)blockIdx.x * blockDim.x + threadIdx.x) - lane; e0 < n;
        e0 += (long long)gridDim.x * blockDim.x) {
@@ -424,6 +426,7 @@
 __global__ void __launch_bounds__(256) sumsq_norms_kernel(GradSrc s, const double* __restrict__ gnorm, int n,
                                                           double* __restrict__ out, unsigned long long* __restrict__ fx,
                                                           const float* __restrict__ dense, long long n_dense) {
+  resolve_src(s);
   __shared__ double red[4];
   const int lane = threadIdx.x & 63;
   double acc = 0.0;
@@ -1706,8 +1709,8 @@
                                                  int* __restrict__ last, const PendSrc& ps, int B, long long bid,
                                                  long long nblk) {
   constexpr int G = D / 4, RPW = 64 / G;
-  if (gs.Lp1 > 1) {
-    float* dst = const_cast<float*>(ps.ring) + (size_t)(t % ps.ring_n) * ps.ring_stride;
+  float* dst = const_cast<float*>(ps.ring) + (size_t)(t % ps.ring_n) * ps.ring_stride;
+  if (gs.Lp1 > 1 && gs.vec != dst) {
     const long long n4 = (long long)B * 2 * D / 4, st = nblk * blockDim.x;
     for (long long i0 = bid * blockDim.x + threadIdx.x; i0 < n4; i0 += 8 * st) {
       f32x4 x[8];
diff --git a/ctr_recommendation_amd/csrc/plan_thunks.inc b/ctr_recommendation_amd/csrc/plan_thunks.inc
--- a/ctr_recommendation_amd/csrc/plan_thunks.inc
+++ b/ctr_recommendation_amd/csrc/plan_thunks.inc
@@ -890,6 +890,42 @@
       static_cast<int>(i[1]),
       static_cast<int>(i[2]));
 }
+static int th_fbn_fields_bwd_slot(const uint64_t* i, const double* f) {
+  return fbn_fields_bwd_slot(reinterpret_cast<const int64_t*>(static_cast<uintptr_t>(i[0])),
+      reinterpret_cast<const int64_t*>(static_cast<uintptr_t>(i[1])),
+      reinterpret_cast<const int64_t*>(static_cast<uintptr_t>(i[2])),
+      reinterpret_cast<const int64_t*>(static_cast<uintptr_t>(i[3])),
+      reinterpret_cast<const float*>(static_cast<uintptr_t>(i[4])),
+      reinterpret_cast<const float*>(static_cast<uintptr_t>(i[5])),
+      reinterpret_cast<const float*>(static_cast<uintptr_t>(i[6])),
+      plan_f32(f[0]),
+      reinterpret_cast<const float*>(static_cast<uintptr_t>(i[7])),
+      reinterpret_cast<const float*>(static_cast<uintptr_t>(i[8])),
+      reinterpret_cast<const float*>(static_cast<uintptr_t>(i[9])),
+      static_cast<int>(i[10]),
+      static_cast<int>(i[11]),
+      reinterpret_cast<const float*>(static_cast<uintptr_t>(i[12])),
+      reinterpret_cast<const float*>(static_cast<uintptr_t>(i[13])),
+      reinterpret_cast<const float*>(static_cast<uintptr_t>(i[14])),
+      reinterpret_cast<const float*>(static_cast<uintptr_t>(i[15])),
+      reinterpret_cast<const float*>(static_cast<uintptr_t>(i[16])),
+      reinterpret_cast<float*>(static_cast<uintptr_t>(i[17])),
+      reinterpret_cast<void*>(static_cast<uintptr_t>(i[18])),
+      static_cast<int>(i[19]),
+      reinterpret_cast<float*>(static_cast<uintptr_t>(i[20])),
+      reinterpret_cast<float* const*>(static_cast<uintptr_t>(i[21])),
+      reinterpret_cast<float*>(static_cast<uintptr_t>(i[22])),
+      static_cast<int>(i[23]),
+      static_cast<long long>(i[24]),
+      reinterpret_cast<const int*>(static_cast<uintptr_t>(i[25])),
+      reinterpret_cast<void*>(static_cast<uintptr_t>(i[26])),
+      reinterpret_cast<double*>(static_cast<uintptr_t>(i[27])),
+      static_cast<long long>(i[28]),
+      static_cast<int>(i[29]),
+      static_cast<int>(i[30]),
+      static_cast<int>(i[31]),
+      reinterpret_cast<void*>(static_cast<uintptr_t>(i[32])));
+}
 static int th_fbn_fields_fwd(const uint64_t* i, const double* f) {
   return fbn_fields_fwd(reinterpret_cast<const int64_t*>(static_cast<uintptr_t>(i[0])),
       reinterpret_cast<const int64_t*>(static_cast<uintptr_t>(i[1])),
@@ -1518,6 +1554,17 @@
       reinterpret_cast<const void*>(static_cast<uintptr_t>(i[2])),
       static_cast<int>(i[3]),
       reinterpret_cast<void*>(static_cast<uintptr_t>(i[4])));
+}
+static int th_fbn_sum_jobs_sq(const uint64_t* i, const double* f) {
+  (void)f;
+  return fbn_sum_jobs_sq(reinterpret_cast<const void*>(static_cast<uintptr_t>(i[0])),
+      static_cast<int>(i[1]),
+      reinterpret_cast<const void*>(static_cast<uintptr_t>(i[2])),
+      static_cast<int>(i[3]),
+      reinterpret_cast<const void*>(static_cast<uintptr_t>(i[4])),
+      static_cast<int>(i[5]),
+      reinterpret_cast<double*>(static_cast<uintptr_t>(i[6])),
+      reinterpret_cast<void*>(static_cast<uintptr_t>(i[7])));
 }
 static int th_fbn_sum_slices(const uint64_t* i, const double* f) {
   (void)f;
@@ -1664,6 +1711,7 @@
     {"fbn_fields_bwd_grid", th_fbn_fields_bwd_grid, 2, 0},
     {"fbn_fields_bwd_img", th_fbn_fields_bwd_img, 32, 1},
     {"fbn_fields_bwd_partials_size", th_fbn_fields_bwd_partials_size, 3, 0},
+    {"fbn_fields_bwd_slot", th_fbn_fields_bwd_slot, 33, 1},
     {"fbn_fields_fwd", th_fbn_fields_fwd, 33, 1},
     {"fbn_fields_fwd_hot", th_fbn_fields_fwd_hot, 34, 1},
     {"fbn_gemm", th_fbn_gemm, 25, 1},
@@ -1708,6 +1756,7 @@
     {"fbn_sum", th_fbn_sum, 4, 1},
     {"fbn_sum_jobs", th_fbn_sum_jobs, 3, 0},
     {"fbn_sum_jobs2", th_fbn_sum_jobs2, 5, 0},
+    {"fbn_sum_jobs_sq", th_fbn_sum_jobs_sq, 8, 0},
     {"fbn_sum_slices", th_fbn_sum_slices, 6, 0},
     {"fbn_sumsq", th_fbn_sumsq, 6, 0},
     {"fbn_sumsq_flagged", th_fbn_sumsq_flagged, 10, 0},
diff --git a/ctr_recommendation_amd/ops.py b/ctr_recommendation_amd/ops.py
--- a/ctr_recommendation_amd/ops.py
+++ b/ctr_recommendation_amd/ops.py
@@ -162,6 +162,10 @@
 
 _DEFER_REDUCE = os.environ.get("FBN_DEFER_REDUCE", "1") != "0"
 _WGRAD_GROUP = os.environ.get("FBN_WGRAD_GROUP", "1") != "0"
+
+
+class _SqRange(ctypes.Structure):
+    _fields_ = [("x", ctypes.c_void_p), ("n", ctypes.c_longlong)]
 
 
 class _SlabGemm(ctypes.Structure):
@@ -250,18 +254,59 @@
 
     timed_group = False
 
-    def flush(self, stream, probe: Optional[Dict[str, list]] = None):
+    def classify(self, grads: Dict[str, torch.Tensor]):
+        by_ptr = {t.data_ptr(): (k, t) for k, t in grads.items()}
+        covered, partial = set(), []
+        for i, j in enumerate(self.jobs):
+            hit = by_ptr.get(j[1])
+            if hit is None:
+                continue
+            if j[3] != hit[1].numel() or j[5] != 0.0 or hit[0] in covered:
+                raise RuntimeError("clip norm in the sum launch: a sum job must write one whole dense gradient, once")
+            covered.add(hit[0])
+            self.jobs[i] = j[:7] + (1,)
+        for sj in self.slabs:
+            hit = by_ptr.get(sj[1])
+            if hit is None or hit[0] in covered:
+                raise RuntimeError("clip norm in the sum launch: a slab job's output is not one dense gradient")
+            covered.add(hit[0])
+            if sj[2] * sj[3] != hit[1].numel():
+                partial.append((hit[0], sj[3], (sj[6], sj[7], sj[8])))
+        ranges = [(t.data_ptr(), t.numel()) for k, t in grads.items() if k not in covered]
+        return ranges, partial
+
+    def flush(self, stream, probe: Optional[Dict[str, list]] = None, sumsq: Optional[torch.Tensor] = None,
+              grads: Optional[Dict[str, torch.Tensor]] = None):
         self.launch_group(stream, None if self.timed_group else probe)
+        ranges, partial = self.classify(grads) if sumsq is not None else (None, None)
         jobs, slabs = self.jobs, self.slabs
-        while jobs or slabs:
+        while jobs or slabs or ranges:
             jc, sc = jobs[:16], slabs[:8]
             jobs, slabs = jobs[16:], slabs[8:]
             arr = (_SumJob * max(1, len(jc)))(*[_SumJob(*j) for j in jc])
             sarr = (_SlabJob * max(1, len(sc)))(*[_SlabJob(*j) for j in sc])
+            if sumsq is not None:
+                rc, ranges = ranges[:24], ranges[24:]
+                rarr = (_SqRange * max(1, len(rc)))(*[_SqRange(*r) for r in rc])
+                _lib.keep((arr, sarr, rarr))
+                call("fbn_sum_jobs_sq", ctypes.addressof(arr), len(jc), ctypes.addressof(sarr), len(sc),
+                     ctypes.addressof(rarr), len(rc), ptr(sumsq), stream)
+                continue
             _lib.keep((arr, sarr))
             call("fbn_sum_jobs2", ctypes.addressof(arr), len(jc), ctypes.addressof(sarr), len(sc), stream)
         self.jobs, self.slabs, self.keep = [], [], []
         self.used = set()
+        return partial
+
+
+def check_unwritten_columns_zero(gt: torch.Tensor, N: int, remap) -> None:
+    seg, off0, off1 = remap
+    cols = torch.arange(N, device=gt.device)
+    keep = torch.ones(gt.shape[1], dtype=torch.bool, device=gt.device)
+    keep[cols + torch.where(cols < seg, off0, off1)] = False
+    worst = gt[:, keep].abs().max().item() if bool(keep.any()) else 0.0
+    if worst != 0.0:
+        raise RuntimeError(f"dense gradient columns outside the slab job's image are not zero (max {worst})")
 
 
 def colsum(X, B, C, ldx, out, beta=0.0, stream=None):
@@ -619,11 +664,11 @@
 def backward(p: Dict[str, torch.Tensor], batch: Dict[str, torch.Tensor], a: Dict[str, torch.Tensor],
              gout: torch.Tensor, g: Dict[str, torch.Tensor], cfg: FwdConfig, *,
              table_grad: Optional[torch.Tensor] = None, gvec: Optional[torch.Tensor] = None,
-             gnorm: Optional[torch.Tensor] = None,
+             gnorm: Optional[torch.Tensor] = None, gslot=None, dense_sumsq: Optional[torch.Tensor] = None,
              pos: Optional[torch.Tensor] = None,
              sendbuf: Optional[torch.Tensor] = None, coll: Collective = NO_COLLECTIVE,
              ntot: Optional[int] = None, extra_sums=(), side: Optional["torch.cuda.Stream"] = None,
-             probe: Optional[Dict[str, list]] = None, hooks: Optional[Dict[str, object]] = None) -> None:
+             probe: Optional[Dict[str, list]] = None, hooks: Optional[Dict[str, object]] = None):
     d, L = cfg.d, cfg.L
     B = a["B"]
     dev = gout.device
@@ -838,14 +883,24 @@
         _lib.keep(outs_arr)
         outs = ctypes.cast(outs_arr, ctypes.c_void_p).value
     evb = _probe_start(probe, "fields_bwd")
-    call("fbn_fields_bwd_img" if s3img else "fbn_fields_bwd", ptr(batch["item_id"]), ptr(seq) if Lr else None,
-         ptr(batch["likes_level"]),
-         ptr(batch["views_level"]), ptr(a["hmm"]), ptr(p["mm_proj.1.weight"]), ptr(p["mm_proj.1.bias"]), LN_EPS,
-         ptr(p["senet.excitation.0.weight"]), ptr(p["senet.excitation.0.bias"]), ptr(p["senet.excitation.2.weight"]),
-         R, ncate, ptr(p["cate_emb.weight"]), ptr(a["X"]), ptr(a["a"]), ptr(a["cnt"]), ptr(dV), ptr(dhmm),
-         ptr(dhs if s3img else dhmm16), ptr(partials), outs,
-         ptr(table_grad), ptr(gvec), ptr(gnorm), V, ptr(pos), ptr(sendbuf),
-         int(sendbuf is not None and sendbuf.dtype == torch.bfloat16), B, Lr, d, st)
+    if gslot is not None:
+        ring, ring_n, ring_stride, step, cell = gslot
+        call("fbn_fields_bwd_slot", ptr(batch["item_id"]), ptr(seq) if Lr else None, ptr(batch["likes_level"]),
+             ptr(batch["views_level"]), ptr(a["hmm"]), ptr(p["mm_proj.1.weight"]), ptr(p["mm_proj.1.bias"]), LN_EPS,
+             ptr(p["senet.excitation.0.weight"]), ptr(p["senet.excitation.0.bias"]),
+             ptr(p["senet.excitation.2.weight"]), R, ncate, ptr(p["cate_emb.weight"]), ptr(a["X"]), ptr(a["a"]),
+             ptr(a["cnt"]), ptr(dV), ptr(dhmm), ptr(dhs if s3img else dhmm16), int(bool(s3img)), ptr(partials), outs,
+             ptr(ring), ring_n, ring_stride, ptr(step), ptr(cell), ptr(gnorm), V, B, Lr, d, st)
+    else:
+        call("fbn_fields_bwd_img" if s3img else "fbn_fields_bwd", ptr(batch["item_id"]), ptr(seq) if Lr else None,
+             ptr(batch["likes_level"]),
+             ptr(batch["views_level"]), ptr(a["hmm"]), ptr(p["mm_proj.1.weight"]), ptr(p["mm_proj.1.bias"]), LN_EPS,
+             ptr(p["senet.excitation.0.weight"]), ptr(p["senet.excitation.0.bias"]),
+             ptr(p["senet.excitation.2.weight"]),
+             R, ncate, ptr(p["cate_emb.weight"]), ptr(a["X"]), ptr(a["a"]), ptr(a["cnt"]), ptr(dV), ptr(dhmm),
+             ptr(dhs if s3img else dhmm16), ptr(partials), outs,
+             ptr(table_grad), ptr(gvec), ptr(gnorm), V, ptr(pos), ptr(sendbuf),
+             int(sendbuf is not None and sendbuf.dtype == torch.bfloat16), B, Lr, d, st)
     _probe_end(evb)
     if hooks and "after_fields_bwd" in hooks:
         hooks["after_fields_bwd"]()
@@ -868,5 +923,8 @@
         sums.add(*job)
     if hooks and "before_flush" in hooks:
         hooks["before_flush"]()
-    sums.flush(st, probe)
+    if dense_sumsq is not None and side is not None:
+        raise ValueError("dense_sumsq needs the weight gradients on the main stream (side=None)")
+    partial = sums.flush(st, probe, sumsq=dense_sumsq, grads=g if dense_sumsq is not None else None)
     wg.join()
+    return partial
diff --git a/ctr_recommendation_amd/trainer.py b/ctr_recommendation_amd/trainer.py
--- a/ctr_recommendation_amd/trainer.py
+++ b/ctr_recommendation_amd/trainer.py
@@ -40,6 +40,8 @@
 _OWNER_CLAIM_FUSED = os.environ.get("FBN_OWNER_CLAIM_FUSED", "1") != "0"
 _SHARD_W16_SIDE = os.environ.get("FBN_SHARD_W16_SIDE", "1") != "0"
 _OWNER_FOLD = os.environ.get("FBN_OWNER_FOLD", "1") != "0"
+_GVEC_SLOT = os.environ.get("FBN_GVEC_SLOT", "1") != "0"
+_NORM_IN_SUMS = os.environ.get("FBN_NORM_IN_SUMS", "1") != "0"
 _CHECK_POOL = os.environ.get("FBN_CHECK_POOL", "0") == "1"
 from .schedule import OneCycle, adam_table
 
@@ -307,6 +309,9 @@
         self._fc_seen = 0
         self._fc_steps = 0
         self.ring_cell = torch.zeros(2, dtype=torch.int64, device=dev)
+        self.gvec_slot = _GVEC_SLOT and not sharded and self.deferred
+        self.norm_in_sums = _NORM_IN_SUMS and _DENSE_SUMSQ_FOLD and not sharded and not self.deterministic
+        self._gap_checked = False
         self._fc_grad = None
         self._fc_extra = None
         self._fc_part = None
@@ -534,6 +539,13 @@
                                                                         and not torch.cuda.is_current_stream_capturing()))
                       and not self.deterministic and L > 0
                       and not self._early_grad_xchg())
+        slot = self.gvec_slot and self.xchg is None and L > 0
+        gv, gcell = (self.ring_cell, FBN_GRAD_CELL) if slot else (self.gvec, 0)
+        in_sums = self.norm_in_sums and self.xchg is None and L > 0
+
+        def table_norm(stream):
+            call("fbn_sumsq_sparse_norms", ptr(self.gnorm), ptr(gv), ptr(self.extra), ptr(self.slot_row),
+                 (L + 1) | gcell, B * (L + 1), d, ptr(self.sumsq), None, None, 0, stream)
         if (self.xchg is not None and self.shard_graph and probe is None and masks_out is None
                 and self.table_adam != "eager" and not self._recording):
             sendbuf = self.xchg.make_sendbuf()
@@ -554,8 +566,10 @@
             if fixup_side:
                 def fork_fixup():
                     _lib.wait_stream(self.side, main)
-                    call("fbn_sparse_fixup_dup", ptr(self.dup), B * (L + 1), ptr(self.gvec), ptr(self.extra),
-                         ptr(self.slot_row), L + 1, d, self.side.cuda_stream)
+                    call("fbn_sparse_fixup_dup", ptr(self.dup), B * (L + 1), ptr(gv), ptr(self.extra),
+                         ptr(self.slot_row), (L + 1) | gcell, d, self.side.cuda_stream)
+                    if in_sums:
+                        table_norm(self.side.cuda_stream)
                 bhooks = {"after_fields_bwd": fork_fixup}
                 if _WGRAD_EARLY and cfg.bf16:
                     def early_wgrad(sums):
@@ -563,11 +577,19 @@
                         sums.launch_group(self.side.cuda_stream, probe, tstream=self.side)
                     bhooks["after_bilinear_bwd"] = early_wgrad
                     bhooks["before_flush"] = lambda: _lib.wait_stream(main, self.side)
-            ops.backward(self.p, batch, a, a["gout"], self.g, cfg, gvec=self.gvec if self.xchg is None else None,
+            gaps = ops.backward(self.p, batch, a, a["gout"], self.g, cfg,
+                         dense_sumsq=self.sumsq if in_sums else None,
+                         gvec=self.gvec if self.xchg is None and not slot else None,
+                         gslot=(self.ring, self.ring_n, self._ring_stride(), self.step_dev, self.ring_cell)
+                         if slot else None,
                          gnorm=self.gnorm if self.xchg is None else None,
                          pos=pos, sendbuf=sendbuf, coll=self.bn_coll, ntot=self._bn_n(ntot, B),
                          extra_sums=[(a["loss_terms"], B, 1, self.loss, 1.0 / ntot)], probe=probe,
                          hooks=bhooks)
+            if gaps and not self._gap_checked and not torch.cuda.is_current_stream_capturing():
+                for key, ncols, remap in gaps:
+                    ops.check_unwritten_columns_zero(self.g[key], ncols, remap)
+                self._gap_checked = True
         dense_work = None
         if self.sharded and self._early_grad_xchg() and self.native_comm is None and not self.coll.det:
             dense_work = dist.all_reduce(self.flat_g, group=self.coll.group, async_op=True)
@@ -580,17 +602,19 @@
             if self.deterministic:
                 if L == 0:
                     raise ValueError("deterministic mode needs the item_seq history (L > 0)")
-                gsrc = (self.gvec, self.extra, (L + 1) | FBN_GRAD_FULL)
-                call("fbn_sparse_fold_fx", ptr(self.dup), ptr(self.hasdup), n_ent, ptr(self.gvec), ptr(self.slot_row),
+                gsrc = (gv, self.extra, (L + 1) | FBN_GRAD_FULL | gcell)
+                call("fbn_sparse_fold_fx", ptr(self.dup), ptr(self.hasdup), n_ent, ptr(gv), ptr(self.slot_row),
                      gsrc[2], d, ptr(self.fx), st)
             else:
-                gsrc = (self.gvec, self.extra, L + 1)
+                gsrc = (gv, self.extra, (L + 1) | gcell)
                 if fixup_side:
                     _lib.wait_stream(main, self.side)
                     joined = True
                 else:
-                    call("fbn_sparse_fixup_dup", ptr(self.dup), n_ent, ptr(self.gvec), ptr(self.extra),
-                         ptr(self.slot_row), L + 1, d, st)
+                    call("fbn_sparse_fixup_dup", ptr(self.dup), n_ent, ptr(gv), ptr(self.extra),
+                         ptr(self.slot_row), gsrc[2], d, st)
+                    if in_sums:
+                        table_norm(st)
         else:
             x = self.xchg
             n_ent = x.n_recv
@@ -647,7 +671,9 @@
                      ptr(gsrc[0]), None, ptr(self.slot_row), gsrc[2], d, st)
         tab_acc = self.sumsq_tab if self.sharded else self.sumsq
         dense_done = False
-        if self.xchg is None and L > 0:
+        if in_sums:
+            dense_done = True
+        elif self.xchg is None and L > 0:
             fold = not self.sharded and _DENSE_SUMSQ_FOLD
             call("fbn_sumsq_sparse_norms", ptr(self.gnorm), ptr(gsrc[0]), ptr(gsrc[1]), ptr(self.slot_row), gsrc[2],
                  n_ent, d, ptr(tab_acc), ptr(self.fx), ptr(self.flat_g) if fold else None,
diff --git a/include/fibinet.h b/include/fibinet.h
--- a/include/fibinet.h
+++ b/include/fibinet.h
@@ -74,6 +74,12 @@
                        const float* a, const float* cnt, const float* dV, float* dhmm, void* dhmm_img,
                        float* partials, float* const* param_grads, float* gtab, float* gvec, double* gnorm,
                        long long V, const int* pos, void* sendbuf, int send_bf16, int B, int L, int D, void* stream);
+int fbn_fields_bwd_slot(const int64_t* item_id, const int64_t* item_seq, const int64_t* likes, const int64_t* views,
+                        const float* hmm, const float* ln_g, const float* ln_b, float ln_eps, const float* w1,
+                        const float* b1, const float* w2, int R, int n_cate, const float* cate, const float* X,
+                        const float* a, const float* cnt, const float* dV, float* dhmm, void* dhmm16, int dhmm_is_img,
+                        float* partials, float* const* param_grads, float* ring, int ring_n, long long ring_stride,
+                        const int* step, void* cell, double* gnorm, long long V, int B, int L, int D, void* stream);
 
 int fbn_pairs_fwd(const float* Vc, const short* Vc16, const float* U, void* c, int B, int D, int ldc, int mode,
                   int c_bf16, void* stream);
@@ -135,6 +141,8 @@
 int fbn_colsum_partial(const float* X, int B, int C, int ldx, float* part, void* stream);
 int fbn_sum_jobs(const void* jobs, int n, void* stream);
 int fbn_sum_jobs2(const void* jobs, int n, const void* slabs, int ns, void* stream);
+int fbn_sum_jobs_sq(const void* jobs, int n, const void* slabs, int ns, const void* ranges, int nr, double* sumsq,
+                    void* stream);
 
 int fbn_head_fwd(const float* H, const float* w, const float* bias, int B, int C, float* logits, float* probs,
                  const float* labels, float* loss_terms, float* gout, float denom, void* stream);
```

New measurement: 20.69 million samples/s (median of 6 runs). 1.0% higher.
